# jinhan/tacotron2-vae

Measured on AMD Instinct MI355X. Metric: mel-frames/s (train step, batch=6, 80-mel), higher is better.
Workload: dtype f32; 1 GPU; configs[1]: Tacotron2-VAE fp32 train step (fwd+loss+bwd+clip+Adam), B=6/GPU fixed shape T_in=84 T_out=400, dropout on, random-init seed 1234; step_mode=hip-graph replay, decoder_forward=persistent, decoder_backward=persistent, startup_steps=43, global_batch=6, parallelism=dp1

## Files before the change

include/t2vae.h:

```cpp
#ifndef T2VAE_H
#define T2VAE_H
#include <stdint.h>
#ifdef __cplusplus
extern "C" {
#endif

#define T2V_OK 0
#define T2V_ERR_DIMS -1
#define T2V_ERR_ARG -2
#define T2V_ERR_LAUNCH -3

const char* t2v_version(void);
const char* t2v_last_error(void);

void t2v_set_phase_profile(unsigned long long* dev_buf32);
int t2v_stamp(unsigned long long* dev_buf, int slot, void* stream);
int t2v_debug_spin(int wgs, int microseconds, void* stream);

typedef struct t2v_step_params {
    uint64_t epoch;
    float lr;
    float bc1;
    float bc2s;
    float kl_weight;
// ... 51 lines not shown
    const float* bias_dec;
    const float* wq;
    const float* wcomb;
    const float* v;
} t2v_dec_train_persist_weights;
int t2v_decoder_train_persist_supported(int B, int T_in);
long t2v_decoder_train_persist_scratch_floats(int B, int T_in, int T_out);
int t2v_decoder_train_fwd_persistent(const t2v_dec_train_persist_weights* w, const t2v_dec_train_bufs* s, float* scratch,
                                     int B, int T_in, int T_out, float p_att, float p_dec, uint64_t seed, void* stream);

int t2v_decoder_train_persist16_supported(int B, int T_in);
long t2v_decoder_train_persist16_scratch_floats(int B, int T_in, int T_out);
int t2v_decoder_train_fwd_persistent16(const t2v_dec_train_persist_weights* w, const t2v_dec_train_bufs* s, float* scratch,
                                       int B, int T_in, int T_out, float p_att, float p_dec, uint64_t seed, void* stream);

int t2v_decoder_replay_fwd_kernels(const t2v_dec_weights* w, const t2v_dec_train_bufs* s,
                                   int B, int T_in, int T_out, float p_att, float p_dec,
                                   uint64_t seed, int kernel_mask, void* stream);

typedef struct t2v_dec_bwd_bufs {
    const float* dHC;
    float* DGA;
    float* DGD;
    float* DQ;
    float* DCTX;
    float* YD;
    float* YA;
    float* DCA;
    float* DCD;
    float* GPREV;
    float* GCUM;
    float* DV;
} t2v_dec_bwd_bufs;

int t2v_attn_bwd_slices(int T_in);

int t2v_decoder_train_bwd(const t2v_dec_weights* w, const t2v_dec_train_bufs* s,
                          const t2v_dec_bwd_bufs* g, int B, int T_in, int T_out,
                          float p_att, float p_dec, uint64_t seed, void* stream);

int t2v_decoder_replay_bwd_kernels(const t2v_dec_weights* w, const t2v_dec_train_bufs* s,
                                   const t2v_dec_bwd_bufs* g, int B, int T_in, int T_out,
                                   float p_att, float p_dec, uint64_t seed, int kernel_mask, void* stream);

int t2v_attn_wgrad_scratch_floats(void);
int t2v_attn_wgrad(const float* dpre, const float* al, const float* acum, const float* loc_conv,
                   const float* loc_dense, float* part_scratch, float* d_loc_dense, float* d_loc_conv,
                   int B, int T_in, int T, void* stream);


int t2v_decoder_bwd_persist_supported(int B, int T_in);
long t2v_decoder_bwd_achain_scratch_floats(int B, int T_in, int T_out);
int t2v_decoder_bwd_persist_slices(int T_in);
int t2v_decoder_bwd_achain(const t2v_dec_train_persist_weights* w, const float* reserved, const t2v_dec_train_bufs* s,
                           const float* dHC, float* DGA, float* DGD, float* DCTX, float* DV, float* DQP, float* scratch,
                           uint32_t* err_word, int B, int T_in, int T_out, float p_att, float p_dec, uint64_t seed,
                           void* stream);
int t2v_decoder_bwd_persist16_supported(int B, int T_in);
int t2v_decoder_bwd_persist16_slices(int T_in);
int t2v_decoder_bwd_persist16_fits(int B, int T_in, int T_out);
long t2v_decoder_bwd_persist16_scratch_floats(int B, int T_in, int T_out);
long t2v_decoder_bwd_persist16_dq_offset(int B, int T_in, int T_out);
int t2v_decoder_bwd_persistent16(const t2v_dec_train_persist_weights* w, const t2v_dec_train_bufs* s, const float* dHC,
                                 float* DGA, float* DGD, float* DCTX, float* DV, float* DQP, float* scratch,
                                 uint32_t* err_word, int B, int T_in, int T_out, float p_att, float p_dec, uint64_t seed,
                                 void* stream);
int t2v_decoder_bwd_persistent16_prepare(float* DQP, float* scratch, uint32_t* err_word, int B, int T_in, int T_out, void* stream);
int t2v_decoder_bwd_persistent16_prepared(const t2v_dec_train_persist_weights* w, const t2v_dec_train_bufs* s, const float* dHC,
                                          float* DGA, float* DGD, float* DCTX, float* DV, float* DQP, float* scratch,
                                          uint32_t* err_word, int B, int T_in, int T_out, float p_att, float p_dec, uint64_t seed,
                                          void* stream);

long t2v_decoder_bwd_achain_dq_offset(int B, int T_in, int T_out);
int t2v_decoder_bwd_achain_prepare(const t2v_dec_train_bufs* s, float* DQP, float* scratch, uint32_t* err_word, int B, int T_in,
                                   int T_out, float p_att, float p_dec, uint64_t seed, void* stream);
int t2v_decoder_bwd_achain_prepared(const t2v_dec_train_persist_weights* w, const float* reserved, const t2v_dec_train_bufs* s,
                           const float* dHC, float* DGA, float* DGD, float* DCTX, float* DV, float* DQP, float* scratch,
                           uint32_t* err_word, int B, int T_in, int T_out, float p_att, float p_dec, uint64_t seed,
                           void* stream);

typedef struct t2v_dec_infer_bufs {
    const float* memory;
    const float* pm;
    const int32_t* lengths;
    float* XS; float* CA; float* CD; float* QP; float* AL; float* ACUM;
    float* PRE;
    float* MEL;
    float* GATE;
    int32_t* stop_flag;
    const float* prenet_w1;
    const float* proj_w;
    const float* proj_b;
} t2v_dec_infer_bufs;

int t2v_decoder_infer_steps(const t2v_dec_weights* w, const t2v_dec_infer_bufs* s, int B, int T_in,
                            int t_begin, int t_end, float gate_threshold, float p_prenet,
                            int external_prenet, uint64_t seed, void* stream);

typedef struct t2v_dec_persist_weights {
    const float* w_ih_att; const float* w_hh_att;
    const float* w_ih_dec; const float* w_hh_dec;
    const float* bias_att; const float* bias_dec;
    const float* wq;
    const float* wcomb;
    const float* v;
    const float* proj_w;
    const float* proj_b;
    const float* prenet_w1;
} t2v_dec_persist_weights;
typedef struct t2v_dec_persist_bufs {
    const float* memory;
    const float* pm;
    const int32_t* lengths;
    const float* pre_first;
    float* MEL;
    float* GATE;
    float* AL;
    int32_t* stop_flag;
    void* exchange;
    uint32_t* err_word;
} t2v_dec_persist_bufs;
long t2v_decoder_persist_scratch_floats(int B, int t_end);
int t2v_decoder_persist_supported(int B, int T_in);
int t2v_decoder_infer_persistent(const t2v_dec_persist_weights* w, const t2v_dec_persist_bufs* s, int B, int T_in,
                                 int t_end, float gate_threshold, float p_prenet, uint64_t seed, void* stream);

typedef struct t2v_dec_items {
    int32_t* stop_item;
    const uint64_t* item_seeds;
// ... 32 lines not shown
                   float* dconv_bias, int B, int M, int T, int act, float p_drop, uint64_t seed,
                   uint32_t rng_stream, uint32_t rng_t, void* stream);
int t2v_bn_act_bwd_eval(const float* y, const float* dout, const float* mean, const float* rstd,
                   const float* gamma, const float* beta, float* dy, float* dgamma, float* dbeta,
                   float* dconv_bias, int B, int M, int T, int act, float p_drop, uint64_t seed,
                   uint32_t rng_stream, uint32_t rng_t, void* stream);

int t2v_embedding_fwd(const long long* ids, const float* W, float* out_bct, int B, int T, int C, int n_symbols, void* stream);
int t2v_embedding_bwd(const long long* ids, const float* dy_bct, float* dW, int B, int T, int C, int n_symbols, void* stream);

int t2v_gemm_epilogue_bwd(const float* dy, const float* y, float* out, size_t n, float scale, void* stream);

long t2v_colsum_scratch_floats(long M, long N);
int t2v_colsum(const float* A, long lda, long M, long N, float* scratch, float* out, void* stream);

int t2v_mask_outputs(float* mel, float* mel_post, float* gate, const int* lengths, int B, int C, int T, float gate_fill,
                     void* stream);
int t2v_mask_time(const float* x, float* out, const int32_t* lengths, int B, int C, int T, void* stream);
int t2v_reparam_fwd(const float* eps, const float* mu, const float* logvar, float* z, long n, void* stream);
int t2v_reparam_bwd(const float* dz, const float* eps, const float* logvar, float* dlogvar, long n, void* stream);
int t2v_gather_words(const void* const* src, void* const* dst, int n, void* stream);
int t2v_concat2_rows(const float* a, long lda, int na, const float* b, long ldb, int nb, float* out, long rows, void* stream);

int t2v_bilstm_fwd(const float* gx, const float* whh, const int32_t* lengths, float* y, float* gates,
                   float* cells, float* hx_scratch, uint32_t* sync3, int B, int T, void* stream);
int t2v_bilstm_bwd(const float* whh, const int32_t* lengths, const float* dy, const float* gates,
                   const float* cells, float* dg, float* dgx_scratch, uint32_t* sync3, int B, int T,
                   void* stream);

int t2v_gemm_f32(const float* A, long sAi, long sAk, const float* B, long sBj, long sBk, const float* bias,
                 float* C, int ldc, int M, int N, int K, int relu, int accumulate, float p_drop,
                 uint64_t seed, uint32_t rng_stream, uint32_t rng_t, void* stream);
long t2v_gemm_splitk_scratch_floats(int M, int N, int K);
int t2v_gemm_f32_splitk(const float* A, long sAi, long sAk, const float* B, long sBj, long sBk, const float* bias,
                        float* C, int ldc, int M, int N, int K, int relu, int accumulate, float p_drop,
                        uint64_t seed, uint32_t rng_stream, uint32_t rng_t, float* splitk_scratch, void* stream);

int t2v_gemm_f32_set_mode(int x3);

typedef struct t2v_gemm_group {
    const float* A;
    long sAi;
    long sAk;
    int nb;
    const float* B[3];
    long sBj[3];
    long sBk[3];
    int N[3];
    float* C[3];
    int ldc[3];
} t2v_gemm_group;
long t2v_gemm_f32_grouped_scratch_floats(const t2v_gemm_group* groups, int ngroups, int M, int K);
int t2v_gemm_f32_grouped(const t2v_gemm_group* groups, int ngroups, int M, int K, int accumulate, float* scratch, void* stream);
long t2v_gemm_bf16_grouped_scratch_floats(const t2v_gemm_group* groups, int ngroups, int M, int K);
int t2v_gemm_bf16_grouped(const t2v_gemm_group* groups, int ngroups, int M, int K, int accumulate, float* scratch, void* stream);

int t2v_conv1d_x3_set_mode(int mode);
int t2v_conv1d_takes_x3(int B, int Cin, int T, int Cout, int KS, int bf16);

int t2v_gemm_f32_batched(const float* A, long sAb, long sAi, long sAk, const float* B, long sBb, long sBj, long sBk,
                         float* C, long sCb, int ldc, int nbatch, int M, int N, int K, void* stream);
int t2v_gemm_bf16(const float* A, long sAi, long sAk, const float* B, long sBj, long sBk, const float* bias,
                  float* C, int ldc, int M, int N, int K, int relu, int accumulate, float p_drop,
                  uint64_t seed, uint32_t rng_stream, uint32_t rng_t, void* stream);
long t2v_gemm_bf16_splitk_scratch_floats(int M, int N, int K);
int t2v_gemm_bf16_splitk(const float* A, long sAi, long sAk, const float* B, long sBj, long sBk, const float* bias,
                         float* C, int ldc, int M, int N, int K, int relu, int accumulate, float p_drop,
                         uint64_t seed, uint32_t rng_stream, uint32_t rng_t, float* splitk_scratch, void* stream);


int t2v_conv2d_s2_fwd(const float* x, const float* w, const float* bias, float* y, int B, int Cx, int H, int W,
                      int Cout, int coord, void* stream);
int t2v_conv2d_s2_dw_scratch_floats(int B, int Cx, int H, int W, int Cout, int coord);
int t2v_conv2d_s2_bwd(const float* x, const float* w, const float* dy, float* dx, float* dw, float* dw_scratch,
                      int B, int Cx, int H, int W, int Cout, int coord, void* stream);

long t2v_conv2d_s2_gemm_scratch_floats(int B, int Cx, int H, int W, int Cout, int coord);
int t2v_conv2d_s2_fwd_gemm(const float* x, const float* w, const float* bias, float* y, float* scratch, int B, int Cx, int H, int W,
                           int Cout, int coord, void* stream);
int t2v_conv2d_s2_bwd_gemm(const float* x, const float* w, const float* dy, float* dx, float* dw, float* scratch, int B, int Cx, int H,
                           int W, int Cout, int coord, void* stream);
int t2v_gru_fwd(const float* gi, const float* whh, const float* bhh, float* hs, float* gsave, float* xchg,
                uint32_t* sync2, int B, int T, void* stream);
int t2v_gru_bwd(const float* whh, const float* hs, const float* gsave, const float* dh_last, float* dgi,
                float* dgh, float* xchg, uint32_t* sync2, int B, int T, void* stream);

int t2v_conv2d_s2_fwd_ragged(const float* x, const float* w, const float* bias, float* y, const int32_t* hlen, int B, int Cx,
                             int H, int W, int Cout, int coord, int x_tstride, void* stream);
long t2v_conv2d_s2_gemm_ragged_scratch_floats(int B, int Cx, int H, int W, int Cout, int coord);
int t2v_conv2d_s2_fwd_gemm_ragged(const float* x, const float* w, const float* bias, float* y, float* scratch,
                                  const int32_t* hlen, int B, int Cx, int H, int W, int Cout, int coord, int x_tstride,
                                  void* stream);
int t2v_gru_fwd_len(const float* gi, const float* whh, const float* bhh, float* hs, float* gsave, float* xchg,
                    uint32_t* sync2, const int32_t* steps, float* h_last, int B, int T, void* stream);
int t2v_loss_fwd_bwd(const float* mel, const float* post, const float* mel_t, const float* gate,
                     const float* gate_t, const float* mu, const float* logvar, float* dmel, float* dpost,
                     float* dgate, float* dmu, float* dlogvar, float* part192, float* out4, uint32_t* ticket,
                     uint64_t n_mel, int n_gate, int n_lat, float kl_weight, void* stream);

int t2v_clip_adam_step(float* params, float* grads, float* exp_avg, float* exp_avg_sq, uint64_t n,
                       float lr, float beta1, float beta2, float eps, float weight_decay,
                       float max_norm, float inv_world, float bc1, float bc2, float* partials,
                       float* norm_out, void* stream);
int t2v_clip_adam_step_guarded(float* params, float* grads, float* exp_avg, float* exp_avg_sq, uint64_t n,
                               float lr, float beta1, float beta2, float eps, float weight_decay,
                               float max_norm, float inv_world, float bc1, float bc2, float* partials,
// ... 32 lines not shown
```

tacotron2-vae_amd/csrc/decoder_train_bwd_persist.hip:

```cpp
#include "t2v_common.h"
#include "t2v_kernels.h"
#include "t2v_xchg.h"

#define PB_THREADS 512
#define PB_MAXB 6
#define PB_MAXT 224
#define PB_MAXT_LONG 576
#define PB_SPIN 400000
#define PB_KJ (T2V_G / PB_THREADS)

#define PB_ROW_BYTES(NB) ((NB) > 4 ? 98304u : 65536u)

#define PB_DROW_BYTES(NB) ((NB) > 4 ? 49152u : 32768u)
__device__ __forceinline__ void pb_dma4(const void* g, float* ldsbase, const int aux_sc1) {
    if (aux_sc1)
        __builtin_amdgcn_global_load_lds((const __attribute__((address_space(1))) void*)g, (__attribute__((address_space(3))) void*)ldsbase, 4, 0, T2V_SC1);
    else
        __builtin_amdgcn_global_load_lds((const __attribute__((address_space(1))) void*)g, (__attribute__((address_space(3))) void*)ldsbase, 4, 0, 0);
}

template <int NB>
__device__ __forceinline__ void pb_park_factors(float* ldsX, const float* Frow) {
    const int wave = threadIdx.x >> 6, lane = threadIdx.x & 63;
    constexpr int NCH = PB_ROW_BYTES(NB) / 1024;
#pragma unroll
    for (int i = 0; i < NCH / 8; ++i) {
        const int c = wave + 8 * i;
        __builtin_amdgcn_global_load_lds((const __attribute__((address_space(1))) void*)(Frow + 256 * c + 4 * lane),
                                         (__attribute__((address_space(3))) void*)(ldsX + 256 * c), 16, 0, 0);
    }
}
template <int NB>
__device__ __forceinline__ int pb_build_row(f32x4* X0, f32x2* X1, __amdgpu_buffer_rsrc_t r, unsigned row_off, int B,
                                            int nap, unsigned* err, int* flag) {
    const int tid = threadIdx.x;
    for (int i = 0; i < nap; i += 8) __builtin_amdgcn_s_sleep(8);
    f32x4 dc[2], dh[2], dx[2];
    int rounds = 0;
    const int nw0 = min(B, 4), nw1 = B - 4;
    for (;;) {
#pragma unroll
        for (int h = 0; h < 2; ++h) {
            const unsigned U = (unsigned)(tid + PB_THREADS * h);
            dc[h] = t2v_ld_f32x4(r, row_off + 32u * U);
            dh[h] = t2v_ld_f32x4(r, row_off + 32u * U + 16u);
            if (NB > 4) dx[h] = t2v_ld_f32x4(r, row_off + 32768u + 16u * U);
        }
        bool ok = true;
#pragma unroll
        for (int h = 0; h < 2; ++h) {
            ok = ok && t2v_ok(dc[h][0]) && (nw0 < 2 || t2v_ok(dc[h][1])) && (nw0 < 3 || t2v_ok(dc[h][2])) && (nw0 < 4 || t2v_ok(dc[h][3]));
            ok = ok && t2v_ok(dh[h][0]) && (nw0 < 2 || t2v_ok(dh[h][1])) && (nw0 < 3 || t2v_ok(dh[h][2])) && (nw0 < 4 || t2v_ok(dh[h][3]));
            if (NB > 4) ok = ok && t2v_ok(dx[h][0]) && t2v_ok(dx[h][2]) && (nw1 < 2 || (t2v_ok(dx[h][1]) && t2v_ok(dx[h][3])));
        }
        if (__all(ok)) break;
        __builtin_amdgcn_s_sleep(2);
        if (t2v_give_up(rounds, PB_SPIN, err, flag)) break;
    }
#pragma unroll
    for (int j = 0; j < PB_KJ; ++j) {
        const int h = j & 1;
        const f32x4 d = (j >> 1) == 3 ? dh[h] : dc[h];
// ... 82 lines not shown
                     "v_add_f32_dpp %0, %2, %2 row_half_mirror row_mask:0xf bank_mask:0xa" : "=&v"(t) : "v"(lo), "v"(hi));
    return t;
}
__device__ __forceinline__ void pb_reduce16(float (&v)[16], float* part) {
    const int tid = threadIdx.x, lane = tid & 63;
    const bool b1 = lane & 2, b0 = lane & 1;
    float w8[8], w4[4], w2[2];
#pragma unroll
    for (int i = 0; i < 8; ++i) w8[i] = pb_dpp_pair_add(v[i], v[8 + i], 0);
#pragma unroll
    for (int i = 0; i < 4; ++i) w4[i] = pb_dpp_pair_add(w8[i], w8[4 + i], 1);
#pragma unroll
    for (int i = 0; i < 2; ++i) {
        const float keep = b1 ? w4[2 + i] : w4[i], send = b1 ? w4[i] : w4[2 + i];
        w2[i] = keep + T2V_DPP_F(send, 0x4E);
    }
    const float keep = b0 ? w2[1] : w2[0], send = b0 ? w2[0] : w2[1];
    part[((tid >> 6) * 4 + (lane >> 4)) * 16 + (lane & 15)] = keep + T2V_DPP_F(send, 0xB1);
}
__device__ __forceinline__ float pb_sum16(const float* part, int idx) {
    float s[8];
#pragma unroll
    for (int i = 0; i < 8; ++i) s[i] = (part[(4 * i) * 16 + idx] + part[(4 * i + 1) * 16 + idx]) + (part[(4 * i + 2) * 16 + idx] + part[(4 * i + 3) * 16 + idx]);
    return ((s[0] + s[1]) + (s[2] + s[3])) + ((s[4] + s[5]) + (s[6] + s[7]));
}

static size_t pb_row_bytes(int B) { return B > 4 ? 98304u : 65536u; }

extern "C" int t2v_decoder_bwd_persist_supported(int B, int T_in) {
    if (!(B >= 1 && B <= PB_MAXB && T_in >= 1 && T_in <= PB_MAXT_LONG)) return 0;
    return t2v_persist_cus_ok();
}

struct PBAArgs {
    const float* w_ih_att; const float* w_hh_att; const float* w_ih_dec; const float* w_hh_dec;
    const float* wq;
    const float* wcomb;
    const float* v;
    const float* memory; const float* XS; const float* CA; const float* CD; const float* GA; const float* GD; const float* AL;
    float* S;
    const float* dHC;
    float* DGA; float* DGD; float* DCTX; float* DV;
    float* GXA; float* GXD; float* CX; float* DQX; float* GPX; float* EX;
    float* DQT;
    const float* CPA;
    const float* CPD;
    const float* FA; const float* FD;
    unsigned* err;
    int B, T_in, T, S_sl;
    float p_att, p_dec;
    uint64_t seed;
    const t2v_step_params* step;
    unsigned long long* prof;
};
#define PBA_STAMP(COND, I) do { if (a.prof && (COND) && threadIdx.x == 0) { const unsigned long long now_ = __builtin_readcyclecounter(); \
        lprof_[(I)] += now_ - tprev_; tprev_ = now_; } } while (0)
#define PBA_RT(SLOT) do { if (a.prof && t == a.T / 2 && threadIdx.x == 0) a.prof[64 + blockIdx.x * 8 + (SLOT)] = __builtin_amdgcn_s_memrealtime(); } while (0)
#define PBA_PROF_INIT(FLAGP) unsigned long long* lprof_ = (unsigned long long*)((FLAGP) + 4); \
    if (threadIdx.x < 16) lprof_[threadIdx.x] = 0ull
#define PBA_PROF_FLUSH(COND, I0, N) do { if (a.prof && (COND) && threadIdx.x < (N)) a.prof[(I0) + threadIdx.x] = lprof_[(I0) + threadIdx.x]; } while (0)

#define PB_CX_ROW_BYTES(NB) ((NB) > 4 ? 32768u : 16384u)

__host__ __device__ static inline int pba_na(int NL);
template <int JS, int NWV>
__device__ __forceinline__ void pba_attention_role(const PBAArgs& a, float* lds, const int b, const int s, const int NB) {
    constexpr int NJT = JS / 16;
    constexpr int PW = JS + 30;
    constexpr int GPW = PW <= 64 ? 64 : 128;
    constexpr int NRG = 2 * NWV;
    constexpr int DPS = JS == 96 ? JS + 17 : JS + 1;
    static_assert(JS % NRG == 0 && JS % NWV == 0 && PW <= GPW, "slice geometry");
    const int tid = threadIdx.x, lane = tid & 63, wave = tid >> 6;
    const bool act = tid < 64 * NWV;
    const int g = lane >> 4, c16 = lane & 15;
    const int B = a.B, Tp = a.T_in, T = a.T, S = a.S_sl, j0 = s * JS;
    const int Tcap = (Tp + 15) & ~15;
    const int nown = min(JS, Tp - j0);
    const int NAw = pba_na(T2V_NWG - B * S);
    float* gfull0 = lds;
    float* gfull1 = gfull0 + Tcap;
    float* alf = gfull1 + Tcap;
    float* gcum = alf + Tcap;
    float* dctx = gcum + Tcap;
    float* de = dctx + T2V_E;
    float* red = de + JS;
    float* dpT = red + (1 + JS / NWV) * 4 * NWV;
    float* Tl = dpT + T2V_A * DPS;
    float* rq = Tl + 64 * (JS + 1);
    float* rv = rq + NRG * T2V_A;
    int* flag = (int*)(rv + NRG * T2V_A);
    constexpr bool AREG_LDS = NWV == 8;
    float* wcs = (float*)(flag + 40);
    const __amdgpu_buffer_rsrc_t rC = t2v_rsrc(a.CX), rQ = t2v_rsrc(a.DQX), rP = t2v_rsrc(a.GPX), rQT = t2v_rsrc(a.DQT);
    const int d4 = tid & 31, rg = (tid >> 5) & (NRG - 1);
    float4 m0[JS / NWV], m1[JS / NWV];
    float areg[AREG_LDS ? 1 : 32];
    float4 vd4 = make_float4(0.f, 0.f, 0.f, 0.f);
    if (act) {
#pragma unroll
        for (int r = 0; r < JS / NWV; ++r) {
            const int jl = wave + NWV * r;
            const float* mrow = a.memory + ((size_t)b * Tp + j0 + (jl < nown ? jl : 0)) * T2V_E + lane * 4;
            m0[r] = *(const float4*)mrow;
            m1[r] = *(const float4*)(mrow + 256);
        }
// ... 261 lines not shown
        }
    }
#pragma unroll
    for (int i = 0; i < 16; ++i) v[i] = 0.f;
#pragma unroll
    for (int c = 0; c < NC; ++c)
#pragma unroll
        for (int i = 0; i < 3; ++i) { v[c * 8 + 2 * i] = acc[c][i][0]; v[c * 8 + 2 * i + 1] = acc[c][i][1]; }
}

template <int NCT, int C0, int N, int NB, int R = 0>
__device__ __forceinline__ void pba_rounds16(const f32x2 (&w)[NCT][PB_KJ / 2], const f32x4* X0, const f32x2* X1, float* part) {
    if constexpr (2 * R < N) {
        float v[16];
        pb_gemv_cols16<NCT, C0 + 2 * R, (N - 2 * R >= 2 ? 2 : 1), NB>(w, X0, X1, v);
        pb_reduce16(v, part + 512 * R);
        pba_rounds16<NCT, C0, N, NB, R + 1>(w, X0, X1, part);
    }
}

#define PBA_NUA 13
#define PBA_NCA 7
#define PBA_NUD 8
#define PBA_NCD 4
__host__ __device__ static inline int pba_na(int NL) {
    if (NL - 128 >= 86) return NL - 128;
    const int n = (3 * NL + 4) / 8;
    return n < 79 ? 79 : n;
}

__device__ __forceinline__ float pba_wait_word(__amdgpu_buffer_rsrc_t r, unsigned off, unsigned* err, int* flag) {
    unsigned x;
    int spins = 0;
    for (;;) {
        x = t2v_ld_b32(r, off);
        if (x != T2V_SENT) break;
        __builtin_amdgcn_s_sleep(1);
        if (t2v_give_up(spins, PB_SPIN, err, flag)) break;
    }
    return __uint_as_float(x);
}

template <int NB>
__device__ __forceinline__ void pba_publish_rows(__amdgpu_buffer_rsrc_t r, unsigned row_off, const float* stage, int u0, int nu) {
    const int tid = threadIdx.x;
    if (tid < 2 * nu) {
        const int u = tid >> 1, q = tid & 1;
        const float* sp = stage + (u * 2 + q) * 8;
        t2v_st(r, row_off + 32u * (unsigned)(u0 + u) + 16u * (unsigned)q, f32x4{sp[0], sp[1], sp[2], sp[3]});
        if (NB > 4) t2v_st(r, row_off + 32768u + 16u * (unsigned)(u0 + u) + 8u * (unsigned)q, f32x2{sp[4], sp[5]});
    }
}

template <int NB>
__device__ __forceinline__ void pba_decoder_role(const PBAArgs& a, float* lds, const int jd, const int ND) {
    const int B = a.B, T = a.T;
    f32x4* X0 = (f32x4*)lds;
    f32x2* X1 = (f32x2*)(lds + 4 * T2V_G);
    float* part = lds + (NB > 4 ? 6 : 4) * T2V_G;
    float* stage = part + 10 * 512;
    float* cpd = stage + 256;
    float* dhcs = cpd + 1024;
    int* flag = (int*)(dhcs + 128);
    const int u0 = (jd * T2V_H) / ND, nu = ((jd + 1) * T2V_H) / ND - u0;
    const int c0 = (jd * T2V_E) / ND, nc = ((jd + 1) * T2V_E) / ND - c0;
    const __amdgpu_buffer_rsrc_t rD = t2v_rsrc(a.GXD), rE = t2v_rsrc(a.EX), rDG = t2v_rsrc(a.DGD);
    f32x2 w[20][PB_KJ / 2];
    {
        const int tid = threadIdx.x;
#pragma unroll
        for (int jj = 0; jj < PB_KJ; ++jj) {
            const size_t k = (size_t)(tid + PB_THREADS * jj);
#pragma unroll
            for (int u = 0; u < PBA_NUD; ++u) {
                const bool on = u < nu;
                const int U = u0 + (on ? u : 0);
                w[u][jj / 2][jj & 1] = on ? a.w_hh_dec[k * T2V_H + U] : 0.f;
                w[8 + u][jj / 2][jj & 1] = on ? a.w_ih_dec[k * T2V_KATT + U] : 0.f;
            }
#pragma unroll
            for (int c = 0; c < PBA_NCD; ++c) {
                const bool on = c < nc;
                w[16 + c][jj / 2][jj & 1] = on ? a.w_ih_dec[k * T2V_KATT + T2V_H + c0 + (on ? c : 0)] : 0.f;
            }
        }
        if (tid == 0) flag[0] = 1;
    }
    float dcd = 0.f;
    int nap = 0;
    const int ncp4 = 2 * nu * NB;
    const float* cpd0 = a.CPD + (size_t)u0 * NB * 8;
    constexpr size_t CPSTEP = (size_t)T2V_H * NB * 8;
    {
        const int tid = threadIdx.x;
        if (tid < ncp4) *(float4*)(cpd + ((T - 1) & 1) * 512 + 4 * tid) = *(const float4*)(cpd0 + (size_t)(T - 1) * CPSTEP + 4 * tid);
        const int cu = tid >> 3, cb = tid & 7;
        if (tid < 64 && cu < nu && cb < B) dhcs[((T - 1) & 1) * 64 + tid] = a.dHC[((size_t)(T - 1) * B + cb) * (T2V_H + T2V_E) + u0 + cu];
    }
    pb_park_factors<NB>(lds, a.FD + (size_t)(T - 1) * (PB_ROW_BYTES(NB) / 4));
    __syncthreads();

    if (a.prof && jd == 0 && threadIdx.x == 0) a.prof[40] = __builtin_amdgcn_s_memrealtime();
    for (int t = T; t >= 0; --t) {
        int tid_op = threadIdx.x;
        asm volatile("" : "+v"(tid_op));
        const int tid = tid_op;
// ... 2 lines not shown
        const int U = u0 + (cu < nu ? cu : 0);
        if (t < T) {
            const int rounds = pb_build_row<NB>(X0, X1, rD, (unsigned)t * PB_DROW_BYTES(NB), B, nap, a.err, flag);
            nap = t2v_adapt_nap(nap, rounds);
            pba_rounds16<20, 0, 8, NB>(w, X0, X1, part);
        }
        if (t >= 2) {
            if (tid < ncp4)
                __builtin_amdgcn_global_load_lds((const __attribute__((address_space(1))) void*)(cpd0 + (size_t)(t - 2) * CPSTEP + 4 * tid),
                                                 (__attribute__((address_space(3))) void*)(cpd + ((t - 2) & 1) * 512 + 256 * (tid >> 6)), 16, 0, 0);
            if (cell_thr) pb_dma4(a.dHC + ((size_t)(t - 2) * B + cb) * (T2V_H + T2V_E) + U, dhcs + ((t - 2) & 1) * 64, 0);
        }
        __syncthreads();
        if (flag[0] != 1) return;
        f32x4 dg4 = {0.f, 0.f, 0.f, 0.f};
        if (t >= 1) {
            const int td = t - 1;
            if (cell_thr) {
                const float dh = dhcs[(td & 1) * 64 + tid] + (t < T ? pb_sum16(part + (cu >> 1) * 512, (cu & 1) * 8 + cb) : 0.f);
                const float* cp = cpd + (td & 1) * 512 + (cu * NB + cb) * 8;
                const float4 c0v = *(const float4*)cp, c1v = *(const float4*)(cp + 4);
                const float dht = dh * c0v.x;
                const float dct = dcd * c0v.y + dht * c0v.z;
                dg4 = f32x4{dct * c1v.x, dct * c1v.y, dct * c1v.z, dht * c1v.w};
                dcd = dct * c0v.w;
                float* sp = stage + (cu * 2) * 8 + cb;
                sp[0] = dct; sp[8] = dht;
            }
            if (tid < 64) pba_publish_rows<NB>(rD, (unsigned)td * PB_DROW_BYTES(NB), stage, u0, nu);
            if (cell_thr) {
                const unsigned o = (unsigned)((td * B + cb) * T2V_G + U) * 4u;
                __builtin_amdgcn_raw_buffer_store_b32(__float_as_uint(dg4[0]), rDG, (int)o, 0, 0);
                __builtin_amdgcn_raw_buffer_store_b32(__float_as_uint(dg4[1]), rDG, (int)(o + 4u * T2V_H), 0, 0);
                __builtin_amdgcn_raw_buffer_store_b32(__float_as_uint(dg4[2]), rDG, (int)(o + 8u * T2V_H), 0, 0);
                __builtin_amdgcn_raw_buffer_store_b32(__float_as_uint(dg4[3]), rDG, (int)(o + 12u * T2V_H), 0, 0);
            }
        }
        if (t < T) {
            pba_rounds16<20, 8, 12, NB>(w, X0, X1, part + 4 * 512);
            __syncthreads();
            if (t > 0) pb_park_factors<NB>(lds, a.FD + (size_t)(t - 1) * (PB_ROW_BYTES(NB) / 4));
            if (tid >= 64 && tid < 64 + 96) {
                const int i = tid - 64, col = i >> 3, b = i & 7;
                if (b < B) {
                    const float val = pb_sum16(part + (4 + (col >> 1)) * 512, (col & 1) * 8 + b);
                    if (col < 8) { if (col < nu) t2v_st(rE, (unsigned)(((t * B + b) * T2V_KATT) + u0 + col) * 4u, val); }
                    else if (col - 8 < nc) t2v_st(rE, (unsigned)(((t * B + b) * T2V_KATT) + T2V_H + c0 + col - 8) * 4u, val);
                }
            }
        }
        __syncthreads();
    }
    if (a.prof && jd == 0 && threadIdx.x == 0) a.prof[41] = __builtin_amdgcn_s_memrealtime();
}

struct PBACellIn { float gi, gf, gg, go, cac, cprev; };
__device__ __forceinline__ PBACellIn pba_cell_pre_load(const PBAArgs& a, bool cell_thr, int t, int cb, int U) {
    PBACellIn r = {0.f, 0.f, 0.f, 0.f, 0.f, 0.f};
    if (!cell_thr) return r;
    const int B = a.B;
    const float* gp = a.GA + ((size_t)t * B + cb) * T2V_G + U;
    r.gi = gp[0]; r.gf = gp[T2V_H]; r.gg = gp[2 * T2V_H]; r.go = gp[3 * T2V_H];
    r.cac = a.CA[((size_t)(t + 1) * B + cb) * T2V_H + U];
    r.cprev = a.CA[((size_t)t * B + cb) * T2V_H + U];
    return r;
}
__device__ __forceinline__ void pba_cell_pre_finish(const PBAArgs& a, float* cpre, uint64_t seed, bool cell_thr, int rowi, int t, uint32_t idx,
                                                    const PBACellIn& r) {
    if (!cell_thr) return;
    const float gi = r.gi, gf = r.gf, gg = r.gg, go = r.go;
    float cprev = r.cprev;
    const float fh = t2v_drop_scale(seed, T2V_RNG_ATT_H, t, idx, a.p_att);
    const float fc = t2v_drop_scale(seed, T2V_RNG_ATT_C, t, idx, a.p_att);
    if (t > 0) cprev *= t2v_drop_scale(seed, T2V_RNG_ATT_C, t - 1, idx, a.p_att);
    const float tc = tanhf_(r.cac);
    *(float4*)(cpre + rowi * 8) = make_float4(fh, fc, go * (1.0f - tc * tc), gf);
    *(float4*)(cpre + rowi * 8 + 4) = make_float4(gg * gi * (1.0f - gi), cprev * gf * (1.0f - gf), gi * (1.0f - gg * gg), tc * go * (1.0f - go));
}
__device__ __forceinline__ void pba_cell_pre(const PBAArgs& a, float* cpre, uint64_t seed, bool cell_thr, int rowi, int t, int cb, int U,
                                             uint32_t idx) {
    const PBACellIn r = pba_cell_pre_load(a, cell_thr, t, cb, U);
    pba_cell_pre_finish(a, cpre, seed, cell_thr, rowi, t, idx, r);
}

template <int NB, int NUA, int NCA>
__device__ __forceinline__ void pba_attention_rnn_role(const PBAArgs& a, float* lds, const int ja, const int NA) {
    constexpr int NCT = NUA + NCA;
    static_assert(NCA > 4 && NCA <= 8 && NUA > 8 && NUA <= 16, "two context rounds, three or four recurrent rounds");
    constexpr int NCR = (NCA + 1) / 2;
    const uint64_t seed = t2v_step_seed(a.seed, a.step);
    const int tid = threadIdx.x;
    const int B = a.B, T = a.T, S = a.S_sl;
    f32x4* X0 = (f32x4*)lds;
    f32x2* X1 = (f32x2*)(lds + 4 * T2V_G);
    float* part = lds + (NB > 4 ? 6 : 4) * T2V_G;
    float* ysum = part + 6 * 1024;
    float* dhA = ysum + 192;
    float* stage = dhA + 128;
    float* wqs = stage + 512;
    float* dqs = wqs + 16 * T2V_A;
    float* cpre = dqs + 8 * T2V_A;
    float* eps = cpre + 2048;
    int* flag = (int*)(eps + 256);
    float* dump = eps + 256 + 64;
    const int u0 = (ja * T2V_H) / NA, nu = ((ja + 1) * T2V_H) / NA - u0;
    const int c0 = (ja * T2V_E) / NA, nc = ((ja + 1) * T2V_E) / NA - c0;
// ... 187 lines not shown
        }
        __syncthreads();
        if (t > 0) pba_publish_rows<NB>(rA, (unsigned)t * PB_DROW_BYTES(NB), stage, u0, nu);
        if (cell_thr) {
            const unsigned o = (unsigned)((t * B + cb) * T2V_G + U) * 4u;
            __builtin_amdgcn_raw_buffer_store_b32(__float_as_uint(dg4[0]), rDG, (int)o, 0, 0);
            __builtin_amdgcn_raw_buffer_store_b32(__float_as_uint(dg4[1]), rDG, (int)(o + 4u * T2V_H), 0, 0);
            __builtin_amdgcn_raw_buffer_store_b32(__float_as_uint(dg4[2]), rDG, (int)(o + 8u * T2V_H), 0, 0);
            __builtin_amdgcn_raw_buffer_store_b32(__float_as_uint(dg4[3]), rDG, (int)(o + 12u * T2V_H), 0, 0);
        }
        PBA_STAMP(ja == 0, 6);
        PBA_RT(5);
        __syncthreads();
        PBA_STAMP(ja == 0, 7);
    }
    if (a.prof && ja == 0 && tid == 0) a.prof[43] = __builtin_amdgcn_s_memrealtime();
    PBA_PROF_FLUSH(ja == 0, 0, 8);
    PBA_PROF_FLUSH(ja == 0, 12, 4);
}

template <int NB, bool LONG>
__global__ __launch_bounds__(PB_THREADS) void k_achain_bwd(PBAArgs a) {
    extern __shared__ __attribute__((aligned(16))) float lds[];
    const int wg = blockIdx.x;
    const int S = a.S_sl, NT = a.B * S, NL = T2V_NWG - NT, NA = pba_na(NL), ND = NL - NA;
#if defined(PBA_ONLY) && PBA_ONLY == 1
    pba_attention_role<16, 4>(a, lds, wg / S, wg % S, NB);
#elif defined(PBA_ONLY) && PBA_ONLY == 2
    pba_attention_rnn_role<NB, 12, 6>(a, lds, wg - NT, NA);
#elif defined(PBA_ONLY) && PBA_ONLY == 3
    pba_attention_rnn_role<NB, PBA_NUA, PBA_NCA>(a, lds, wg - NT, NA);
#elif defined(PBA_ONLY) && PBA_ONLY == 4
    pba_decoder_role<NB>(a, lds, wg - NT - NA, ND);
#else
    if (wg < NT) {
        if (LONG) pba_attention_role<96, 8>(a, lds, wg / S, wg % S, NB);
        else if (a.T_in <= 128) pba_attention_role<16, 4>(a, lds, wg / S, wg % S, NB);
        else pba_attention_role<32, 4>(a, lds, wg / S, wg % S, NB);
    } else if (wg < NT + NA) {
        if (NA >= 114) pba_attention_rnn_role<NB, 9, 5>(a, lds, wg - NT, NA);
        else if (NA >= 86) pba_attention_rnn_role<NB, 12, 6>(a, lds, wg - NT, NA);
        else pba_attention_rnn_role<NB, PBA_NUA, PBA_NCA>(a, lds, wg - NT, NA);
    } else {
        pba_decoder_role<NB>(a, lds, wg - NT - NA, ND);
    }
#endif
}

static inline int pba_js(int T_in) { return T_in > PB_MAXT ? 96 : t2v_attn_bwd_js(T_in); }
static inline int pba_slices(int T_in) { const int js = pba_js(T_in); return (T_in + js - 1) / js; }
extern "C" int t2v_decoder_bwd_persist_slices(int T_in) { return T_in < 1 ? 0 : pba_slices(T_in); }

static size_t pba_lds_bytes(int B, int T_in) {
    const size_t lrole = (B > 4 ? 6 : 4) * T2V_G + 6 * 1024 + 192 + 128 + 512 + 16 * T2V_A + 8 * T2V_A + 2048 + 256 + 64 + 512;
    const size_t Tcap = (size_t)((T_in + 15) / 16) * 16, JS = (size_t)pba_js(T_in), NWV = JS == 96 ? 8 : 4;
    const size_t trole = 4 * Tcap + T2V_E + JS + (1 + JS / NWV) * 4 * NWV + T2V_A * (JS == 96 ? JS + 17 : JS + 1) + 64 * (JS + 1) +
                         2 * 2 * NWV * T2V_A + 40 + (NWV == 8 ? 64 * 132 : 0);
    return sizeof(float) * (lrole > trole ? lrole : trole);
}

struct PBALayout {
    size_t n_gx, n_cx, n_gp, n_ex, n_dqt, n_f, n_cp, n_dq;
    size_t dqt_off() const { return 2 * n_gx + n_cx + n_gp + n_ex; }
    size_t n_exchange() const { return dqt_off() + n_dqt; }
    size_t total() const { return n_exchange() + 2 * n_f + 2 * n_cp; }
};
static PBALayout pba_layout(int B, int T_in, int T_out) {
    const size_t T = (size_t)T_out, S = (size_t)pba_slices(T_in), gpw = pba_js(T_in) + 30 <= 64 ? 64 : 128;
    const size_t rowf = pb_row_bytes(B) / 4, cxf = (size_t)(B > 4 ? 32768 : 16384) / 4;
    PBALayout l;
    l.n_gx = T * rowf / 2;
    l.n_cx = T * cxf;
    l.n_gp = T * B * S * 2 * gpw;
    l.n_ex = T * B * T2V_KATT;
    l.n_dqt = T * 8 * T2V_A;
    l.n_f = T * rowf;
    l.n_cp = T * T2V_H * (B > 4 ? 6 : 4) * 8;
    l.n_dq = T * B * S * 128;
    return l;
}

extern "C" long t2v_decoder_bwd_achain_scratch_floats(int B, int T_in, int T_out) {
    if (B < 1 || B > PB_MAXB || T_in < 1 || T_in > PB_MAXT_LONG || T_out < 1) return 0;
    return (long)pba_layout(B, T_in, T_out).total();
}

extern "C" long t2v_decoder_bwd_achain_dq_offset(int B, int T_in, int T_out) {
    if (!t2v_decoder_bwd_persist_supported(B, T_in) || T_out < 1) return -1;
    return (long)pba_layout(B, T_in, T_out).dqt_off();
}

static int pba_launch(const t2v_dec_train_persist_weights* w, const t2v_dec_train_bufs* s,
                      const float* dHC, float* DGA, float* DGD, float* DCTX, float* DV, float* DQP, float* scratch,
                      uint32_t* err_word, int B, int T_in, int T_out, float p_att, float p_dec, uint64_t seed,
                      void* stream_, bool do_prepare, bool do_run) {
    hipStream_t stream = (hipStream_t)stream_;
    if (!s || !DQP || !scratch || !err_word) return T2V_ERR_ARG;
    if (do_run && (!w || !dHC || !DGA || !DGD || !DCTX || !DV)) return T2V_ERR_ARG;
    if (!t2v_decoder_bwd_persist_supported(B, T_in) || T_out < 1) return T2V_ERR_ARG;
    if (do_run && (!w->w_ih_att || !w->w_hh_att || !w->w_ih_dec || !w->w_hh_dec || !w->wq || !w->wcomb || !w->v)) return T2V_ERR_ARG;
    if (!s->memory || !s->XS || !s->CA || !s->CD || !s->GA || !s->GD || !s->AL || !s->S) return T2V_ERR_ARG;
    const PBALayout l = pba_layout(B, T_in, T_out);
    if (((uintptr_t)scratch & 15) || ((uintptr_t)DQP & 15) || l.n_gx * 4 >= 0x7fffffffull || l.n_dq * 4 >= 0x7fffffffull) return T2V_ERR_ARG;
    if (pba_lds_bytes(B, T_in) > T2V_LDS_MAX) return T2V_ERR_ARG;
    static bool raised = false;
    if (!t2v_persist_raise_lds({(const void*)k_achain_bwd<4, false>, (const void*)k_achain_bwd<6, false>,
                                (const void*)k_achain_bwd<4, true>, (const void*)k_achain_bwd<6, true>}, raised))
        return t2v_check_launch();
    if (do_prepare) {
        (void)hipMemsetAsync(err_word, 0, sizeof(uint32_t), stream);
        t2v_fill_sentinel(scratch, l.n_exchange() / 4, 1024, stream);
        t2v_fill_sentinel(DQP, l.n_dq / 4, 256, stream);
    }
    PBAArgs a;
    if (do_run) {
        a.w_ih_att = w->w_ih_att; a.w_hh_att = w->w_hh_att; a.w_ih_dec = w->w_ih_dec; a.w_hh_dec = w->w_hh_dec;
        a.wq = w->wq; a.wcomb = w->wcomb; a.v = w->v;
    }
    a.memory = s->memory; a.XS = s->XS; a.CA = s->CA; a.CD = s->CD; a.GA = s->GA; a.GD = s->GD; a.AL = s->AL; a.S = s->S;
    a.dHC = dHC; a.DGA = DGA; a.DGD = DGD; a.DCTX = DCTX; a.DV = DV; a.DQX = DQP;
    a.GXA = scratch;
    a.GXD = a.GXA + l.n_gx;
    a.CX = a.GXD + l.n_gx;
    a.GPX = a.CX + l.n_cx;
    a.EX = a.GPX + l.n_gp;
    a.DQT = a.EX + l.n_ex;
    float* FA = a.DQT + l.n_dqt;
    float* FD = FA + l.n_f;
    float* CPA = FD + l.n_f;
    float* CPD = CPA + l.n_cp;
    a.FA = FA; a.FD = FD; a.CPA = CPA; a.CPD = CPD;
    a.err = err_word;
    a.B = B; a.T_in = T_in; a.T = T_out; a.S_sl = pba_slices(T_in); a.p_att = p_att; a.p_dec = p_dec; a.seed = seed;
    a.step = t2v_step_for(stream);
    a.prof = g_t2v_prof;
    if (do_prepare) {
        const unsigned nblk = (unsigned)(((size_t)T_out * T2V_G + 255) / 256);
        k_pb_factors<<<nblk, 256, 0, stream>>>(s->GA, s->CA, FA, B, T_out, B, p_att, T2V_RNG_ATT_C, seed, a.step);
        k_pb_factors<<<nblk, 256, 0, stream>>>(s->GD, s->CD, FD, B, T_out, B, p_dec, T2V_RNG_DEC_C, seed, a.step);
        const int nbs = B > 4 ? 6 : 4;
        const unsigned ncp = (unsigned)(((size_t)T_out * T2V_H * nbs + 255) / 256);
        k_pb_cellpre<<<ncp, 256, 0, stream>>>(s->GA, s->CA, CPA, B, T_out, nbs, p_att, T2V_RNG_ATT_H, T2V_RNG_ATT_C, seed, a.step);
        k_pb_cellpre<<<ncp, 256, 0, stream>>>(s->GD, s->CD, CPD, B, T_out, nbs, p_dec, T2V_RNG_DEC_H, T2V_RNG_DEC_C, seed, a.step);
    }
    if (!do_run) return t2v_check_launch();
    const size_t lds = pba_lds_bytes(B, T_in);
    if (T_in > PB_MAXT) {
        if (B > 4) k_achain_bwd<6, true><<<T2V_NWG, PB_THREADS, lds, stream>>>(a);
        else k_achain_bwd<4, true><<<T2V_NWG, PB_THREADS, lds, stream>>>(a);
    } else {
        if (B > 4) k_achain_bwd<6, false><<<T2V_NWG, PB_THREADS, lds, stream>>>(a);
        else k_achain_bwd<4, false><<<T2V_NWG, PB_THREADS, lds, stream>>>(a);
    }
    return t2v_check_launch();
}

extern "C" int t2v_decoder_bwd_achain(const t2v_dec_train_persist_weights* w, const float* w_unused, const t2v_dec_train_bufs* s,
                                      const float* dHC, float* DGA, float* DGD, float* DCTX, float* DV, float* DQP, float* scratch,
                                      uint32_t* err_word, int B, int T_in, int T_out, float p_att, float p_dec, uint64_t seed,
                                      void* stream_) {
    (void)w_unused;
    return pba_launch(w, s, dHC, DGA, DGD, DCTX, DV, DQP, scratch, err_word, B, T_in, T_out, p_att, p_dec, seed, stream_, true, true);
}

extern "C" int t2v_decoder_bwd_achain_prepare(const t2v_dec_train_bufs* s, float* DQP, float* scratch, uint32_t* err_word, int B, int T_in,
                                              int T_out, float p_att, float p_dec, uint64_t seed, void* stream_) {
    return pba_launch(nullptr, s, nullptr, nullptr, nullptr, nullptr, nullptr, DQP, scratch, err_word, B, T_in, T_out, p_att, p_dec, seed,
                      stream_, true, false);
}
extern "C" int t2v_decoder_bwd_achain_prepared(const t2v_dec_train_persist_weights* w, const float* w_unused, const t2v_dec_train_bufs* s,
                                               const float* dHC, float* DGA, float* DGD, float* DCTX, float* DV, float* DQP, float* scratch,
                                               uint32_t* err_word, int B, int T_in, int T_out, float p_att, float p_dec, uint64_t seed,
                                               void* stream_) {
    (void)w_unused;
    return pba_launch(w, s, dHC, DGA, DGD, DCTX, DV, DQP, scratch, err_word, B, T_in, T_out, p_att, p_dec, seed, stream_, false, true);
}
```

tacotron2-vae_amd/csrc/gemm.hip:

```cpp
#include <stdlib.h>
#include <string.h>
#include "t2v_common.h"
#include "t2v_kernels.h"
#include "t2v_coop.h"
#include "t2v_x3.h"
#include "t2v_xchg.h"

#define GM_BM 64
#define GM_BN 64
#define GM_BK 32

struct GemmArgs {
    const float* A; const float* B; const float* bias; float* C;
    long sAi, sAk, sBj, sBk;
    int M, N, K, ldc;
    int relu, accumulate;
    float p_drop; uint64_t seed; uint32_t rng_stream, rng_t;
    const t2v_step_params* step;
    int kz_chunk;
    float* part;
    int nbatch;
    long sAb, sBb, sCb;
    int nsub;
    long sAs, sBs;
    int bias_row;
    unsigned* tile_ctr;
};

__device__ __forceinline__ void gemm64_epilogue(const GemmArgs& a, f32x16& acc, int i0, int j0, int wm, int wn, int lane, int tid) {
    const int j = j0 + 32 * wn + (lane & 31);
    if (a.part) {
        if (j < a.N) {
#pragma unroll
            for (int r = 0; r < 16; ++r) {
                const int i = i0 + 32 * wm + (r & 3) + 8 * (r >> 2) + 4 * (lane >> 5);
                if (i < a.M) st_sc1(a.part + ((size_t)blockIdx.z * a.M + i) * a.N + j, acc[r]);
            }
        }
        __shared__ unsigned last_;
        asm volatile("s_waitcnt vmcnt(0)" ::: "memory");
        __syncthreads();
        unsigned* ctr = a.tile_ctr + blockIdx.y * gridDim.x + blockIdx.x;
        if (tid == 0) last_ = __hip_atomic_fetch_add(ctr, 1u, __ATOMIC_RELAXED, __HIP_MEMORY_SCOPE_AGENT) == gridDim.z - 1 ? 1u : 0u;
        __syncthreads();
        if (!last_) return;
        if (tid == 0) __hip_atomic_store(ctr, 0u, __ATOMIC_RELAXED, __HIP_MEMORY_SCOPE_AGENT);
        const int nz = (int)gridDim.z;
#pragma unroll
        for (int r = 0; r < 16; ++r) acc[r] = 0.f;
        if (j < a.N) {
            for (int z0 = 0; z0 < nz; z0 += 4) {
                float v[4][16];
#pragma unroll
                for (int u = 0; u < 4; ++u) {
                    const int z = min(z0 + u, nz - 1);
#pragma unroll
                    for (int r = 0; r < 16; ++r) {
                        const int i = min(i0 + 32 * wm + (r & 3) + 8 * (r >> 2) + 4 * (lane >> 5), a.M - 1);
                        v[u][r] = ld_sc1(a.part + ((size_t)z * a.M + i) * a.N + j);
// ... 524 lines not shown
            if (j < a.N) {
                const float bvs = a.bias ? a.bias[j] : 0.f;
#pragma unroll
                for (int r = 0; r < 16; ++r) {
                    const int i = i0 + 64 * wm + 32 * x + (r & 3) + 8 * (r >> 2) + 4 * (lane >> 5);
                    if (i < a.M) {
                        const size_t idx = (size_t)i * a.ldc + j;
                        float v = acc[x][y][r] + bvs;
                        if (a.accumulate) v += a.C[idx];
                        a.C[idx] = v;
                    }
                }
            }
        }
}
static bool gemm_bf16_big_operand_ok(long s_row, long s_k, int K, bool* kc) {
    if (s_row == 1 && !(s_k & 3)) { *kc = false; return true; }
    if (s_k == 1 && !(s_row & 3) && !(K % GBB_BK)) { *kc = true; return true; }
    return false;
}
static bool gemm_bf16_big_ok(const GemmArgs& a, bool* akc, bool* bkc) {
    if (a.relu || a.p_drop > 0.f) return false;
    if (!gemm_bf16_big_operand_ok(a.sAi, a.sAk, a.K, akc) || !gemm_bf16_big_operand_ok(a.sBj, a.sBk, a.K, bkc)) return false;
    if (a.M < GBB_BM || a.N < GBB_BN || (a.M & 3) || (a.N & 3)) return false;
    if (((uintptr_t)a.A | (uintptr_t)a.B) & 15) return false;
    return (long)((a.M + GBB_BM - 1) / GBB_BM) * ((a.N + GBB_BN - 1) / GBB_BN) >= 64;
}
static int gemm_bf16_big_splits(int M, int N, int K) {
    const long tiles = (long)((M + GBB_BM - 1) / GBB_BM) * ((N + GBB_BN - 1) / GBB_BN);
    const int nkt = (K + GBB_BK - 1) / GBB_BK;
    if (tiles < 64 || tiles >= 512 || nkt < 32) return 1;
    static const int forced = getenv("T2V_GEMM_BF16_SPLITS") ? atoi(getenv("T2V_GEMM_BF16_SPLITS")) : 0;
    long ns = forced > 0 ? forced : (768 + tiles - 1) / tiles;
    if (ns > nkt / 16) ns = nkt / 16;
    if (ns > 8) ns = 8;
    return ns < 2 ? 1 : (int)ns;
}
static bool gemm_bf16_planes_ok(int M, int N, int K);
static long gemm_x3_scratch_floats(int M, int N, int K, int np);
extern "C" long t2v_gemm_bf16_splitk_scratch_floats(int M, int N, int K) {
    if (M < 1 || N < 1 || K < 1) return 0;
    if (gemm_bf16_planes_ok(M, N, K)) return gemm_x3_scratch_floats(M, N, K, 1);
    long big = 0;
    if (M >= GBB_BM && N >= GBB_BN && !(M & 3) && !(N & 3)) {
        const int ns = gemm_bf16_big_splits(M, N, K);
        const long tiles = (long)((M + GBB_BM - 1) / GBB_BM) * ((N + GBB_BN - 1) / GBB_BN);
        big = ns > 1 ? (long)ns * tiles * GBB_BM * GBB_BN : 0;
    }
    const int ns64 = gemm_splits(M, N, K);
    const long small = ns64 > 1 ? (long)ns64 * M * N : 0;
    return big > small ? big : small;
}

#define GX_BM 128
#define GX_BN 128
#define GX_SK 16
static inline long gx_rp(int rows) { return ((long)rows + 127) / 128 * 128; }
static inline long gx_groups(int K, int np = 3) { return np == 3 ? ((long)K + 31) / 32 * 4 : ((long)K + 63) / 64 * 8; }
static inline long gx_plane_slots(int rows, int K, int np = 3) { return np * gx_groups(K, np) * gx_rp(rows); }
template <bool KC, int NP>
__global__ __launch_bounds__(256) void k_x3_split(const float* __restrict__ src, long s_row, long s_k, int rows, int K, uint4* __restrict__ dst,
                                                  long Rp, long G) {
    __shared__ uint4 sm[NP][4][64];
    const int tid = threadIdx.x;
    const int row0 = blockIdx.x * 64, g0 = blockIdx.y * 4;
    const int r = KC ? tid >> 2 : tid & 63, g = KC ? tid & 3 : tid >> 6;
    const int row = row0 + r, k0 = 8 * (g0 + g);
    float v[8];
    const bool rin = row < rows;
    const float* base = src + (long)min(row, rows - 1) * s_row;
    if (KC && s_k == 1 && !(s_row & 3) && !((uintptr_t)src & 15) && k0 + 8 <= K) {
        const float4 lo = *(const float4*)(base + k0), hi = *(const float4*)(base + k0 + 4);
        v[0] = lo.x; v[1] = lo.y; v[2] = lo.z; v[3] = lo.w; v[4] = hi.x; v[5] = hi.y; v[6] = hi.z; v[7] = hi.w;
#pragma unroll
        for (int u = 0; u < 8; ++u) v[u] = rin ? v[u] : 0.f;
    } else {
#pragma unroll
        for (int u = 0; u < 8; ++u) {
            const float x = base[(long)min(k0 + u, K - 1) * s_k];
            v[u] = (rin && k0 + u < K) ? x : 0.f;
        }
    }
    if (NP == 3) {
        uint4 p0, p1, p2;
        t2v_split8(v, p0, p1, p2);
        sm[0][g][r] = p0; sm[NP > 1 ? 1 : 0][g][r] = p1; sm[NP > 2 ? 2 : 0][g][r] = p2;
    } else {
        sm[0][g][r] = make_uint4(t2v_pack_bf16x2(v[0], v[1]), t2v_pack_bf16x2(v[2], v[3]), t2v_pack_bf16x2(v[4], v[5]), t2v_pack_bf16x2(v[6], v[7]));
    }
    __syncthreads();
    const int g2 = tid >> 6, r2 = tid & 63;
    if (row0 + r2 < Rp && g0 + g2 < G) {
#pragma unroll
        for (int p = 0; p < NP; ++p) dst[(p * G + g0 + g2) * Rp + row0 + r2] = sm[p][g2][r2];
    }
}
struct GemmX3Prod {
    const uint4* Ap; const uint4* Bp;
    long RpA, RpB;
    int N, tiles_x, tile0, nseg;
    int seg_col[3]; float* segC[3]; int seg_ldc[3];
};
struct GemmX3Args {
    GemmX3Prod pr[2];
    int nprod, ntiles;
    long G;
    const float* bias;
    int M, relu, accumulate;
    float p_drop; uint64_t seed; uint32_t rng_stream, rng_t;
    const t2v_step_params* step;
    int st_chunk;
    float* part; unsigned* tile_ctr;
};
#ifndef GX_NB
#define GX_NB 2
#endif
#ifndef GX_LDS_PAD
#define GX_LDS_PAD 0
#endif
#ifndef GX_NG1
#define GX_NG1 4
#endif
template <int NP, int NG>
__global__ __launch_bounds__(256, 2) void k_gemm_x3p(GemmX3Args a) {
    __shared__ uint4 lds_[GX_NB * 2 * NP * NG * GX_BM + GX_LDS_PAD];
    uint4 (*Ls)[2][NP][NG][GX_BM] = (uint4 (*)[2][NP][NG][GX_BM])&lds_[0];
    const unsigned lds0 = (unsigned)(unsigned long)(__attribute__((address_space(3))) void*)&lds_[0];
    const int tid = threadIdx.x, wave = __builtin_amdgcn_readfirstlane(tid >> 6), lane = tid & 63;
    const int wm = wave >> 1, wn = wave & 1;
    int lin;
    {
        const int nb = a.ntiles, bid = blockIdx.x;
        const int q = nb >> 3, r = nb & 7, xcd = bid & 7, idx = bid >> 3;
        lin = (xcd < r ? xcd * (q + 1) : r * (q + 1) + (xcd - r) * q) + idx;
    }
    const GemmX3Prod& P = a.pr[(a.nprod > 1 && lin >= a.pr[1].tile0) ? 1 : 0];
    const int by_ = (lin - P.tile0) / P.tiles_x, bx_ = (lin - P.tile0) - by_ * P.tiles_x;
    const int i0 = by_ * GX_BM, j0 = bx_ * GX_BN;
    const int nst_all = (int)(a.G / NG);
    const int st0 = a.st_chunk ? blockIdx.z * a.st_chunk : 0, st1 = a.st_chunk ? min(nst_all, st0 + a.st_chunk) : nst_all;
    constexpr int NPIECE = NP * NG;
    auto stage_dma = [&](int st, int buf) {
        st = min(st, st1 - 1);
#pragma unroll
        for (int i = 0; i < NPIECE; ++i) {
            const int q = wave + 4 * i;
            const int op = q / (2 * NP * NG), rem = q - (2 * NP * NG) * op, p = rem / (2 * NG), g = (rem >> 1) % NG, half = rem & 1;
            const uint4* src = op ? P.Bp + (p * a.G + NG * st + g) * P.RpB + j0 + 64 * half + lane
                                  : P.Ap + (p * a.G + NG * st + g) * P.RpA + i0 + 64 * half + lane;
            t2v_dma16(src, lds0 + 16u * (unsigned)(((((buf * 2 + op) * NP + p) * NG + g) * GX_BM) + 64 * half));
        }
    };
    f32x16 acc[2][2];
#pragma unroll
    for (int x = 0; x < 2; ++x)
#pragma unroll
        for (int y = 0; y < 2; ++y)
#pragma unroll
            for (int r = 0; r < 16; ++r) acc[x][y][r] = 0.f;
    const int am = 64 * wm + (lane & 31), bn = 64 * wn + (lane & 31), kq = lane >> 5;
#define GX_MFMA(A_, B_, C_) C_ = __builtin_amdgcn_mfma_f32_32x32x16_bf16(*(const t2v_bf16x8*)&(A_), *(const t2v_bf16x8*)&(B_), C_, 0, 0, 0)
#pragma unroll
    for (int d = 0; d < GX_NB - 1; ++d) stage_dma(st0 + d, d);
    t2v_wait_vmcnt<NPIECE * (GX_NB - 2)>();
    __syncthreads();
    int buf = 0;
    for (int st = st0; st < st1; ++st) {
        const int nb2 = buf == 0 ? GX_NB - 1 : buf - 1;
        stage_dma(st + GX_NB - 1, nb2);
#define GX_ALL(PA, PB)                                      \
        GX_MFMA(av[PA][0], bv[PB][0], acc[0][0]); GX_MFMA(av[PA][0], bv[PB][1], acc[0][1]); \
        GX_MFMA(av[PA][1], bv[PB][0], acc[1][0]); GX_MFMA(av[PA][1], bv[PB][1], acc[1][1])
#pragma unroll
        for (int ks = 0; ks < NG / 2; ++ks) {
            uint4 av[NP][2], bv[NP][2];
#pragma unroll
            for (int p = 0; p < NP; ++p) {
                av[p][0] = Ls[buf][0][p][2 * ks + kq][am];
                av[p][1] = Ls[buf][0][p][2 * ks + kq][am + 32];
                bv[p][0] = Ls[buf][1][p][2 * ks + kq][bn];
                bv[p][1] = Ls[buf][1][p][2 * ks + kq][bn + 32];
            }
            if constexpr (NP == 3) {
                GX_ALL(2, 0); GX_ALL(0, 2); GX_ALL(1, 1); GX_ALL(1, 0); GX_ALL(0, 1); GX_ALL(0, 0);
            } else {
                GX_ALL(0, 0);
            }
        }
#undef GX_ALL
        t2v_wait_vmcnt<NPIECE * (GX_NB - 2)>();
        __syncthreads();
        buf = buf == GX_NB - 1 ? 0 : buf + 1;
    }
#undef GX_MFMA
    asm volatile("s_waitcnt vmcnt(0)" ::: "memory");
    if (a.part) {
        const size_t tiles = (size_t)a.ntiles, tile = (size_t)lin;
        {
            __amdgpu_buffer_rsrc_t rs = t2v_rsrc(a.part + (blockIdx.z * tiles + tile) * (GX_BM * GX_BN));
#pragma unroll
            for (int x = 0; x < 2; ++x)
#pragma unroll
                for (int y = 0; y < 2; ++y)
#pragma unroll
                    for (int q = 0; q < 4; ++q) {
                        u32x4 v;
                        v.x = __float_as_uint(acc[x][y][4 * q]); v.y = __float_as_uint(acc[x][y][4 * q + 1]);
                        v.z = __float_as_uint(acc[x][y][4 * q + 2]); v.w = __float_as_uint(acc[x][y][4 * q + 3]);
                        __builtin_amdgcn_raw_buffer_store_b128(v, rs, ((((x * 2 + y) * 4 + q) * 256) + tid) * 16, 0, 16);
                    }
        }
        __shared__ unsigned last_;
        asm volatile("s_waitcnt vmcnt(0)" ::: "memory");
        __syncthreads();
        unsigned* ctr = a.tile_ctr + tile;
        if (tid == 0) last_ = __hip_atomic_fetch_add(ctr, 1u, __ATOMIC_RELAXED, __HIP_MEMORY_SCOPE_AGENT) == gridDim.z - 1 ? 1u : 0u;
        __syncthreads();
        if (!last_) return;
        if (tid == 0) __hip_atomic_store(ctr, 0u, __ATOMIC_RELAXED, __HIP_MEMORY_SCOPE_AGENT);
        const int nz = (int)gridDim.z;
#pragma unroll
        for (int x = 0; x < 2; ++x)
#pragma unroll
            for (int y = 0; y < 2; ++y)
#pragma unroll
                for (int r = 0; r < 16; ++r) acc[x][y][r] = 0.f;
        for (int z0 = 0; z0 < nz; z0 += 2) {
            u32x4 v[2][16];
#pragma unroll
            for (int u = 0; u < 2; ++u) {
                const int z = min(z0 + u, nz - 1);
                __amdgpu_buffer_rsrc_t rs = t2v_rsrc(a.part + (z * tiles + tile) * (GX_BM * GX_BN));
#pragma unroll
                for (int g = 0; g < 16; ++g) v[u][g] = __builtin_amdgcn_raw_buffer_load_b128(rs, (g * 256 + tid) * 16, 0, 16);
            }
#pragma unroll
            for (int u = 0; u < 2; ++u)
                if (z0 + u < nz) {
#pragma unroll
                    for (int g = 0; g < 16; ++g) {
                        acc[g >> 3][(g >> 2) & 1][4 * (g & 3)] += __uint_as_float(v[u][g].x);
                        acc[g >> 3][(g >> 2) & 1][4 * (g & 3) + 1] += __uint_as_float(v[u][g].y);
                        acc[g >> 3][(g >> 2) & 1][4 * (g & 3) + 2] += __uint_as_float(v[u][g].z);
                        acc[g >> 3][(g >> 2) & 1][4 * (g & 3) + 3] += __uint_as_float(v[u][g].w);
                    }
                }
        }
    }
    const uint64_t seed = t2v_step_seed(a.seed, a.step);
    int sg = 0;
    if (P.nseg > 1 && j0 >= P.seg_col[1]) sg = 1;
    if (P.nseg > 2 && j0 >= P.seg_col[2]) sg = 2;
    float* const Cd = P.segC[sg];
    const int ldc = P.seg_ldc[sg], jc0 = j0 - P.seg_col[sg];
#pragma unroll
    for (int x = 0; x < 2; ++x)
#pragma unroll
        for (int y = 0; y < 2; ++y) {
            const int jl = 64 * wn + 32 * y + (lane & 31), j = j0 + jl;
            if (j < P.N) {
                const float bvs = a.bias ? a.bias[j] : 0.f;
#pragma unroll
                for (int r = 0; r < 16; ++r) {
                    const int i = i0 + 64 * wm + 32 * x + (r & 3) + 8 * (r >> 2) + 4 * (lane >> 5);
                    if (i < a.M) {
                        const size_t idx = (size_t)i * ldc + jc0 + jl;
                        float v = acc[x][y][r] + bvs;
                        if (a.accumulate) v += Cd[idx];
                        if (a.relu) v = fmaxf(v, 0.f);
                        if (a.p_drop > 0.f) v *= t2v_drop_scale(seed, a.rng_stream, a.rng_t, (uint32_t)idx, a.p_drop);
                        Cd[idx] = v;
                    }
                }
            }
        }
}
static int g_f32_gemm_x3 = -1;
static int gemm_x3_mode() {
    if (g_f32_gemm_x3 < 0) {
        const char* e = getenv("T2V_F32_GEMM");
        g_f32_gemm_x3 = (e && (!strcmp(e, "native") || !strcmp(e, "0"))) ? 0 : 1;
    }
    return g_f32_gemm_x3;
}
extern "C" int t2v_gemm_f32_set_mode(int x3) {
    const int prev = gemm_x3_mode();
    if (x3 >= 0) g_f32_gemm_x3 = x3 ? 1 : 0;
    return prev;
}
static bool gemm_x3_shape_ok(int M, int N, int K) {
    if (M < GX_BM || N < GX_BN || K < 32) return false;
    static const int min_tiles = getenv("T2V_X3_MIN_TILES") ? atoi(getenv("T2V_X3_MIN_TILES")) : 64;
    return (long)((M + GX_BM - 1) / GX_BM) * ((N + GX_BN - 1) / GX_BN) >= min_tiles;
}
static int gemm_x3_splits(int M, int N, int K, int np = 3) {
    const long tiles = (long)((M + GX_BM - 1) / GX_BM) * ((N + GX_BN - 1) / GX_BN);
    const int nst = (int)(gx_groups(K, np) / (np == 3 ? 2 : GX_NG1));
    static const int forced = getenv("T2V_GEMM_X3_SPLITS") ? atoi(getenv("T2V_GEMM_X3_SPLITS")) : 0;
    if (forced > 0) return forced > nst ? nst : forced;
    int best = 1;
    double best_w = 1e30;
    for (int ns = 1; ns <= 6 && (ns == 1 || nst / ns >= 16); ++ns) {
        const double rounds = (double)((tiles * ns + 767) / 768);
        const double w = rounds * (1.0 / ns + 0.08) + 0.03 * (ns - 1);
        if (w < best_w - 1e-9) { best_w = w; best = ns; }
    }
    return best;
}
static long gemm_x3_plane_floats(int M, int N, int K, int np = 3) { return 4 * (gx_plane_slots(M, K, np) + gx_plane_slots(N, K, np)); }
static long gemm_x3_scratch_floats(int M, int N, int K, int np) {
    const int ns = gemm_x3_splits(M, N, K, np);
    const long tiles = (long)((M + GX_BM - 1) / GX_BM) * ((N + GX_BN - 1) / GX_BN);
    return gemm_x3_plane_floats(M, N, K, np) + (ns > 1 ? (long)ns * tiles * GX_BM * GX_BN : 0);
}
static bool gemm_bf16_planes_ok(int M, int N, int K) {
    static const int on = getenv("T2V_BF16_GEMM_PLANES") ? atoi(getenv("T2V_BF16_GEMM_PLANES")) : 1;
    return on && K >= 64 && gemm_x3_shape_ok(M, N, K);
}
static void gx_split_launch(const float* src, long s_row, long s_k, int rows, int K, uint4* planes, long Rp, long G, long row_off, hipStream_t stream,
                            int np = 3) {
    const unsigned gx = (unsigned)((rows + 127) / 128 * 2);
    const dim3 grid(gx, (unsigned)(G / 4));
    if (np == 3) {
        if (s_k == 1) k_x3_split<true, 3><<<grid, 256, 0, stream>>>(src, s_row, s_k, rows, K, planes + row_off, Rp, G);
        else k_x3_split<false, 3><<<grid, 256, 0, stream>>>(src, s_row, s_k, rows, K, planes + row_off, Rp, G);
    } else {
        if (s_k == 1) k_x3_split<true, 1><<<grid, 256, 0, stream>>>(src, s_row, s_k, rows, K, planes + row_off, Rp, G);
        else k_x3_split<false, 1><<<grid, 256, 0, stream>>>(src, s_row, s_k, rows, K, planes + row_off, Rp, G);
    }
}
static int gemm_x3_run(const GemmArgs& g, float* scratch, hipStream_t stream, int np = 3) {
    const int M = g.M, N = g.N, K = g.K;
    uint4* Ap = (uint4*)scratch;
    uint4* Bp = Ap + gx_plane_slots(M, K, np);
    const long G = gx_groups(K, np), RpA = gx_rp(M), RpB = gx_rp(N);
    gx_split_launch(g.A, g.sAi, g.sAk, M, K, Ap, RpA, G, 0, stream, np);
    gx_split_launch(g.B, g.sBj, g.sBk, N, K, Bp, RpB, G, 0, stream, np);
    GemmX3Args a;
    a.nprod = 1;
    GemmX3Prod& P = a.pr[0];
    P.Ap = Ap; P.Bp = Bp; P.RpA = RpA; P.RpB = RpB; P.N = N; P.tiles_x = (N + GX_BN - 1) / GX_BN; P.tile0 = 0; P.nseg = 1;
    P.seg_col[0] = 0; P.segC[0] = g.C; P.seg_ldc[0] = g.ldc;
    a.pr[1] = a.pr[0];
    a.ntiles = P.tiles_x * ((M + GX_BM - 1) / GX_BM);
    a.G = G; a.bias = g.bias; a.M = M; a.relu = g.relu; a.accumulate = g.accumulate;
    a.p_drop = g.p_drop; a.seed = g.seed; a.rng_stream = g.rng_stream; a.rng_t = g.rng_t; a.step = g.step;
    a.st_chunk = 0; a.part = nullptr; a.tile_ctr = nullptr;
    dim3 gb(a.ntiles, 1, 1);
    const int ns = gemm_x3_splits(M, N, K, np);
    if (ns > 1) {
        const int nst = (int)(G / (np == 3 ? 2 : GX_NG1));
        a.st_chunk = (nst + ns - 1) / ns;
        gb.z = (unsigned)((nst + a.st_chunk - 1) / a.st_chunk);
        a.part = scratch + gemm_x3_plane_floats(M, N, K, np);
        a.tile_ctr = t2v_arrival_counters(a.ntiles);
        if (!a.tile_ctr) return T2V_ERR_LAUNCH;
        if (gb.z < 2) { a.st_chunk = 0; a.part = nullptr; a.tile_ctr = nullptr; gb.z = 1; }
    }
    if (np == 3) k_gemm_x3p<3, 2><<<gb, 256, 0, stream>>>(a);
    else k_gemm_x3p<1, GX_NG1><<<gb, 256, 0, stream>>>(a);
    return t2v_check_launch();
}

static long gemm_grouped_scratch(const t2v_gemm_group* gr, int ngroups, int M, int K, int np) {
    if (!gr || ngroups < 1 || ngroups > 2 || M < 1 || K < 1) return 0;
    long slots = 0;
    for (int g = 0; g < ngroups; ++g) {
        long n = 0;
        for (int p = 0; p < gr[g].nb; ++p) n += gx_rp(gr[g].N[p]);
        slots += gx_plane_slots(M, K, np) + np * gx_groups(K, np) * n;
    }
    return 4 * slots;
}
extern "C" long t2v_gemm_f32_grouped_scratch_floats(const t2v_gemm_group* gr, int ngroups, int M, int K) {
    return gemm_grouped_scratch(gr, ngroups, M, K, 3);
}
extern "C" long t2v_gemm_bf16_grouped_scratch_floats(const t2v_gemm_group* gr, int ngroups, int M, int K) {
    return gemm_grouped_scratch(gr, ngroups, M, K, 1);
}
static bool gemm_grouped_x3_ok(const t2v_gemm_group* gr, int ngroups, int M, int K, int np) {
    if ((np == 3 && !gemm_x3_mode()) || M < GX_BM || K < 32) return false;
    long tiles = 0;
    for (int g = 0; g < ngroups; ++g)
        for (int p = 0; p < gr[g].nb; ++p) {
            if (gr[g].N[p] < GX_BN || (gr[g].N[p] % GX_BN)) return false;
            tiles += (long)(gr[g].N[p] / GX_BN) * ((M + GX_BM - 1) / GX_BM);
        }
    return tiles >= 64;
}
static int gemm_grouped_impl(const t2v_gemm_group* gr, int ngroups, int M, int K, int accumulate, float* scratch, void* stream_, int np) {
    hipStream_t stream = (hipStream_t)stream_;
    if (!gr || ngroups < 1 || ngroups > 2 || M < 1 || K < 1) return T2V_ERR_ARG;
    for (int g = 0; g < ngroups; ++g) {
        if (!gr[g].A || gr[g].nb < 1 || gr[g].nb > 3) return T2V_ERR_ARG;
        for (int p = 0; p < gr[g].nb; ++p)
            if (!gr[g].B[p] || !gr[g].C[p] || gr[g].N[p] < 1 || gr[g].ldc[p] < gr[g].N[p]) return T2V_ERR_ARG;
    }
    if (!scratch || ((uintptr_t)scratch & 15) || !gemm_grouped_x3_ok(gr, ngroups, M, K, np)) {
        for (int g = 0; g < ngroups; ++g)
            for (int p = 0; p < gr[g].nb; ++p) {
                const int rc = (np == 3 ? t2v_gemm_f32 : t2v_gemm_bf16)(gr[g].A, gr[g].sAi, gr[g].sAk, gr[g].B[p], gr[g].sBj[p], gr[g].sBk[p], nullptr, gr[g].C[p], gr[g].ldc[p],
                                            M, gr[g].N[p], K, 0, accumulate, 0.f, 0, 0, 0, stream_);
                if (rc != T2V_OK) return rc;
            }
        return T2V_OK;
    }
    const long G = gx_groups(K, np), RpA = gx_rp(M);
    GemmX3Args a;
    a.nprod = ngroups;
    uint4* at = (uint4*)scratch;
    int tile0 = 0;
    for (int g = 0; g < ngroups; ++g) {
        GemmX3Prod& P = a.pr[g];
        long n = 0;
        for (int p = 0; p < gr[g].nb; ++p) n += gr[g].N[p];
        P.Ap = at; at += gx_plane_slots(M, K, np);
        P.Bp = at; at += np * G * n;
        P.RpA = RpA; P.RpB = n; P.N = (int)n; P.tiles_x = (int)(n / GX_BN); P.tile0 = tile0; P.nseg = gr[g].nb;
        gx_split_launch(gr[g].A, gr[g].sAi, gr[g].sAk, M, K, (uint4*)P.Ap, RpA, G, 0, stream, np);
        long col = 0;
        for (int p = 0; p < 3; ++p) {
            const int q = p < gr[g].nb ? p : gr[g].nb - 1;
            P.seg_col[p] = p < gr[g].nb ? (int)col : 0x7fffffff; P.segC[p] = gr[g].C[q]; P.seg_ldc[p] = gr[g].ldc[q];
            if (p < gr[g].nb) {
                gx_split_launch(gr[g].B[p], gr[g].sBj[p], gr[g].sBk[p], gr[g].N[p], K, (uint4*)P.Bp, n, G, col, stream, np);
                col += gr[g].N[p];
            }
        }
        tile0 += P.tiles_x * (int)((M + GX_BM - 1) / GX_BM);
    }
    if (ngroups == 1) a.pr[1] = a.pr[0];
    a.ntiles = tile0;
    a.G = G; a.bias = nullptr; a.M = M; a.relu = 0; a.accumulate = accumulate;
    a.p_drop = 0.f; a.seed = 0; a.rng_stream = 0; a.rng_t = 0; a.step = t2v_step_for(stream);
    a.st_chunk = 0; a.part = nullptr; a.tile_ctr = nullptr;
    if (np == 3) k_gemm_x3p<3, 2><<<dim3(a.ntiles, 1, 1), 256, 0, stream>>>(a);
    else k_gemm_x3p<1, GX_NG1><<<dim3(a.ntiles, 1, 1), 256, 0, stream>>>(a);
    return t2v_check_launch();
}
extern "C" int t2v_gemm_f32_grouped(const t2v_gemm_group* gr, int ngroups, int M, int K, int accumulate, float* scratch, void* stream_) {
    return gemm_grouped_impl(gr, ngroups, M, K, accumulate, scratch, stream_, 3);
}
extern "C" int t2v_gemm_bf16_grouped(const t2v_gemm_group* gr, int ngroups, int M, int K, int accumulate, float* scratch, void* stream_) {
    return gemm_grouped_impl(gr, ngroups, M, K, accumulate, scratch, stream_, 1);
}

__global__ __launch_bounds__(256) void k_epilogue_bwd(const float4* __restrict__ dy, const float4* __restrict__ y,
                                                      float4* __restrict__ out, size_t n4, float scale) {
    const size_t i = (size_t)blockIdx.x * 256 + threadIdx.x;
    if (i >= n4) return;
    const float4 g = dy[i], v = y[i];
    float4 o;
    o.x = v.x != 0.f ? g.x * scale : 0.f; o.y = v.y != 0.f ? g.y * scale : 0.f;
    o.z = v.z != 0.f ? g.z * scale : 0.f; o.w = v.w != 0.f ? g.w * scale : 0.f;
    out[i] = o;
}
__global__ __launch_bounds__(256) void k_epilogue_bwd_tail(const float* __restrict__ dy, const float* __restrict__ y,
                                                           float* __restrict__ out, size_t lo, size_t n, float scale) {
    const size_t i = lo + threadIdx.x;
    if (i < n) out[i] = y[i] != 0.f ? dy[i] * scale : 0.f;
}

extern "C" int t2v_gemm_epilogue_bwd(const float* dy, const float* y, float* out, size_t n, float scale, void* stream_) {
    hipStream_t stream = (hipStream_t)stream_;
    if (!dy || !y || !out || n < 1) return T2V_ERR_ARG;
    if (((uintptr_t)dy | (uintptr_t)y | (uintptr_t)out) & 15) return T2V_ERR_ARG;
    const size_t n4 = n / 4;
    if (n4) k_epilogue_bwd<<<(unsigned)((n4 + 255) / 256), 256, 0, stream>>>((const float4*)dy, (const float4*)y, (float4*)out, n4, scale);
    if (n & 3) k_epilogue_bwd_tail<<<1, 256, 0, stream>>>(dy, y, out, 4 * n4, n, scale);
    return t2v_check_launch();
}

extern "C" int t2v_gemm_f32(const float* A, long sAi, long sAk, const float* B, long sBj, long sBk, const float* bias,
                            float* C, int ldc, int M, int N, int K, int relu, int accumulate, float p_drop,
                            uint64_t seed, uint32_t rng_stream, uint32_t rng_t, void* stream_);
static int gemm_bf16_impl(const float* A, long sAi, long sAk, const float* B, long sBj, long sBk, const float* bias,
                          float* C, int ldc, int M, int N, int K, int relu, int accumulate, float p_drop,
                          uint64_t seed, uint32_t rng_stream, uint32_t rng_t, float* splitk_scratch, void* stream_);
extern "C" int t2v_gemm_bf16(const float* A, long sAi, long sAk, const float* B, long sBj, long sBk, const float* bias,
                             float* C, int ldc, int M, int N, int K, int relu, int accumulate, float p_drop,
                             uint64_t seed, uint32_t rng_stream, uint32_t rng_t, void* stream_) {
    return gemm_bf16_impl(A, sAi, sAk, B, sBj, sBk, bias, C, ldc, M, N, K, relu, accumulate, p_drop, seed, rng_stream, rng_t, nullptr, stream_);
}
extern "C" int t2v_gemm_bf16_splitk(const float* A, long sAi, long sAk, const float* B, long sBj, long sBk, const float* bias,
                                    float* C, int ldc, int M, int N, int K, int relu, int accumulate, float p_drop,
                                    uint64_t seed, uint32_t rng_stream, uint32_t rng_t, float* splitk_scratch, void* stream_) {
    return gemm_bf16_impl(A, sAi, sAk, B, sBj, sBk, bias, C, ldc, M, N, K, relu, accumulate, p_drop, seed, rng_stream, rng_t, splitk_scratch, stream_);
}
static int gemm_bf16_impl(const float* A, long sAi, long sAk, const float* B, long sBj, long sBk, const float* bias,
                          float* C, int ldc, int M, int N, int K, int relu, int accumulate, float p_drop,
                          uint64_t seed, uint32_t rng_stream, uint32_t rng_t, float* splitk_scratch, void* stream_) {
    hipStream_t stream = (hipStream_t)stream_;
    if (!A || !B || !C || M < 1 || N < 1 || K < 1 || ldc < N) return T2V_ERR_ARG;
    GemmArgs a;
// ... 127 lines not shown
```

tacotron2-vae_amd/t2v_hip.py:

```python
import collections
import ctypes as C
import os

import torch

_HERE = os.path.dirname(os.path.abspath(__file__))
_LIB_PATH = os.environ.get('T2V_LIB') or os.path.join(_HERE, 'libt2vae_hip.so')
_lib = None

H, E, PRE, A, F_LOC, KS, XW, KATT, KATT_INF, G4 = 1024, 512, 256, 128, 32, 31, 2560, 1536, 1792, 4096


class T2VHipError(RuntimeError):
    pass


class _DecWeights(C.Structure):
    _fields_ = [(n, C.c_void_p) for n in (
        'packF_att', 'packF_dec', 'packB_att', 'packB_dec', 'bias_att', 'bias_dec', 'wqT', 'wcomb', 'v')] + [
        ('packs_bf16', C.c_int32)]


class _DecTrainBufs(C.Structure):
    _fields_ = [(n, C.c_void_p) for n in (
        'gpre', 'memory', 'pm', 'lengths', 'XS', 'CA', 'CD', 'GA', 'GD', 'QP', 'AL', 'ACUM', 'S')]


class _DecBwdBufs(C.Structure):
    _fields_ = [(n, C.c_void_p) for n in (
        'dHC', 'DGA', 'DGD', 'DQ', 'DCTX', 'YD', 'YA', 'DCA', 'DCD', 'GPREV', 'GCUM', 'DV')]


class _DecPersistWeights(C.Structure):
    _fields_ = [(n, C.c_void_p) for n in (
        'w_ih_att', 'w_hh_att', 'w_ih_dec', 'w_hh_dec', 'bias_att', 'bias_dec', 'wq', 'wcomb', 'v', 'proj_w', 'proj_b',
        'prenet_w1')]


class _DecPersistBufs(C.Structure):
    _fields_ = [(n, C.c_void_p) for n in (
        'memory', 'pm', 'lengths', 'pre_first', 'MEL', 'GATE', 'AL', 'stop_flag', 'exchange', 'err_word')]


class _DecTrainPersistWeights(C.Structure):
    C_NAME = 't2v_dec_train_persist_weights'
    _fields_ = [(n, C.c_void_p) for n in (
        'w_ih_att', 'w_hh_att', 'w_ih_dec', 'w_hh_dec', 'bias_dec', 'wq', 'wcomb', 'v')]


class _GemmGroup(C.Structure):
    C_NAME = 't2v_gemm_group'
    _fields_ = [('A', C.c_void_p), ('sAi', C.c_long), ('sAk', C.c_long), ('nb', C.c_int), ('B', C.c_void_p * 3), ('sBj', C.c_long * 3),
                ('sBk', C.c_long * 3), ('N', C.c_int * 3), ('C', C.c_void_p * 3), ('ldc', C.c_int * 3)]


class _DecInferBufs(C.Structure):
    _fields_ = [(n, C.c_void_p) for n in (
        'memory', 'pm', 'lengths', 'XS', 'CA', 'CD', 'QP', 'AL', 'ACUM', 'PRE', 'MEL', 'GATE', 'stop_flag',
        'prenet_w1', 'proj_w', 'proj_b')]


class _DecItems(C.Structure):
    C_NAME = 't2v_dec_items'
    _fields_ = [(n, C.c_void_p) for n in ('stop_item', 'item_seeds')]


EXPORTS = ('t2v_version', 't2v_last_error', 't2v_stamp', 't2v_debug_spin', 't2v_pack_lstm_weights', 't2v_pack_lstm_weights_bf16', 't2v_decoder_train_fwd',
           't2v_decoder_train_bwd', 't2v_clip_adam_step', 't2v_clip_adam_step_guarded', 't2v_decoder_replay_fwd_kernels', 't2v_mel_frontend', 't2v_set_phase_profile', 't2v_decoder_infer_steps', 't2v_conv1d_stat_blocks', 't2v_conv1d_stat_blocks_bf16', 't2v_conv1d_fwd', 't2v_conv1d_bwd', 't2v_conv1d_fwd_bf16', 't2v_conv1d_bwd_bf16', 't2v_conv1d_dw_scratch_floats', 't2v_conv1d_flip_weights', 't2v_gemm_bf16', 't2v_gemm_bf16_splitk', 't2v_gemm_bf16_splitk_scratch_floats', 't2v_attn_wgrad', 't2v_attn_wgrad_scratch_floats',
           't2v_bn_act_fwd', 't2v_bn_act_bwd', 't2v_bn_act_bwd_eval', 't2v_bilstm_fwd', 't2v_bilstm_bwd', 't2v_gemm_f32', 't2v_conv2d_s2_fwd', 't2v_conv2d_s2_bwd', 't2v_conv2d_s2_dw_scratch_floats', 't2v_conv2d_s2_fwd_gemm', 't2v_conv2d_s2_bwd_gemm',
           't2v_conv2d_s2_gemm_scratch_floats',
           't2v_gru_fwd', 't2v_gru_bwd', 't2v_loss_fwd_bwd', 't2v_fuse_location_weights', 't2v_decoder_qp_floats',
           't2v_set_step_params', 't2v_set_step_params_stream', 't2v_decoder_replay_bwd_kernels', 't2v_embedding_fwd', 't2v_embedding_bwd', 't2v_gemm_f32_splitk', 't2v_gemm_splitk_scratch_floats', 't2v_gemm_f32_batched',
           't2v_decoder_infer_persistent', 't2v_decoder_persist_supported', 't2v_decoder_persist_scratch_floats',
           't2v_attn_bwd_slices', 't2v_colsum', 't2v_colsum_scratch_floats', 't2v_gemm_epilogue_bwd',
           't2v_decoder_train_fwd_persistent', 't2v_decoder_train_persist_supported',
           't2v_decoder_train_persist_scratch_floats', 't2v_decoder_bwd_persist_supported',
           't2v_decoder_bwd_achain_scratch_floats', 't2v_decoder_bwd_achain', 't2v_decoder_bwd_achain_prepare',
           't2v_decoder_bwd_achain_prepared', 't2v_decoder_bwd_persist_slices', 't2v_decoder_bwd_achain_dq_offset', 't2v_mask_outputs', 't2v_reparam_fwd',
           't2v_reparam_bwd', 't2v_gather_words', 't2v_concat2_rows',
           't2v_decoder_train_fwd_persistent16', 't2v_decoder_train_persist16_supported',
           't2v_decoder_train_persist16_scratch_floats', 't2v_decoder_bwd_persistent16', 't2v_decoder_bwd_persist16_supported',
           't2v_decoder_bwd_persist16_scratch_floats', 't2v_decoder_bwd_persist16_dq_offset', 't2v_decoder_bwd_persist16_slices',
           't2v_decoder_bwd_persist16_fits', 't2v_gemm_f32_set_mode', 't2v_conv1d_x3_set_mode', 't2v_gemm_f32_grouped',
           't2v_gemm_f32_grouped_scratch_floats', 't2v_gemm_bf16_grouped', 't2v_gemm_bf16_grouped_scratch_floats',
           't2v_decoder_bwd_persistent16_prepare', 't2v_decoder_bwd_persistent16_prepared',
           't2v_stft_polar', 't2v_istft', 't2v_istft_scratch_bytes', 't2v_griffin_lim', 't2v_griffin_lim_scratch_bytes',
           't2v_mel_to_magnitude', 't2v_decoder_infer_steps_items', 't2v_decoder_infer_persistent_items', 't2v_bn_act_fwd_len',
           't2v_mask_time', 't2v_conv2d_s2_fwd_ragged', 't2v_conv2d_s2_fwd_gemm_ragged', 't2v_conv2d_s2_gemm_ragged_scratch_floats',
           't2v_gru_fwd_len', 't2v_mel_dtw', 't2v_mel_dtw_scratch_bytes')


def lib_path():
    return _LIB_PATH


def load_library():
    global _lib
    if _lib is not None:
        return _lib
    if not os.path.isfile(_LIB_PATH):
        raise T2VHipError("libt2vae_hip.so not built: run `python -c 'import __graft_entry__ as g; g.build()'` "
                          "(or make -C tacotron2-vae_amd/csrc)")
    lib = C.CDLL(_LIB_PATH)
    lib.t2v_version.restype = C.c_char_p
    lib.t2v_last_error.restype = C.c_char_p
    lib.t2v_pack_lstm_weights.argtypes = [C.c_void_p, C.c_void_p, C.c_void_p, C.c_void_p, C.c_int, C.c_void_p,
                                          C.c_void_p, C.c_void_p, C.c_void_p, C.c_void_p]
    lib.t2v_pack_lstm_weights_bf16.argtypes = [C.c_void_p, C.c_void_p, C.c_void_p, C.c_void_p, C.c_int, C.c_void_p,
                                          C.c_void_p, C.c_void_p, C.c_void_p, C.c_void_p]
    lib.t2v_fuse_location_weights.argtypes = [C.c_void_p, C.c_void_p, C.c_void_p, C.c_void_p]
    lib.t2v_decoder_qp_floats.argtypes = [C.c_int, C.c_int]
    lib.t2v_decoder_qp_floats.restype = C.c_long
    lib.t2v_attn_bwd_slices.argtypes = [C.c_int]
    lib.t2v_decoder_train_fwd.argtypes = [C.POINTER(_DecWeights), C.POINTER(_DecTrainBufs), C.c_int, C.c_int,
                                          C.c_int, C.c_float, C.c_float, C.c_uint64, C.c_void_p]
    lib.t2v_decoder_train_bwd.argtypes = [C.POINTER(_DecWeights), C.POINTER(_DecTrainBufs),
                                          C.POINTER(_DecBwdBufs), C.c_int, C.c_int, C.c_int, C.c_float,
                                          C.c_float, C.c_uint64, C.c_void_p]
    lib.t2v_decoder_train_fwd_persistent.argtypes = [C.POINTER(_DecTrainPersistWeights), C.POINTER(_DecTrainBufs), C.c_void_p,
                                                     C.c_int, C.c_int, C.c_int, C.c_float, C.c_float, C.c_uint64, C.c_void_p]
    lib.t2v_decoder_train_persist_supported.argtypes = [C.c_int, C.c_int]
    lib.t2v_decoder_train_fwd_persistent16.argtypes = lib.t2v_decoder_train_fwd_persistent.argtypes
    lib.t2v_decoder_train_persist16_supported.argtypes = [C.c_int, C.c_int]
    lib.t2v_decoder_train_persist16_scratch_floats.argtypes = [C.c_int, C.c_int, C.c_int]
    lib.t2v_decoder_train_persist16_scratch_floats.restype = C.c_long
    lib.t2v_decoder_bwd_persistent16.argtypes = [C.POINTER(_DecTrainPersistWeights), C.POINTER(_DecTrainBufs)] + [C.c_void_p] * 8 + [
        C.c_int, C.c_int, C.c_int, C.c_float, C.c_float, C.c_uint64, C.c_void_p]
    lib.t2v_decoder_bwd_persistent16_prepared.argtypes = lib.t2v_decoder_bwd_persistent16.argtypes
    lib.t2v_decoder_bwd_persistent16_prepare.argtypes = [C.c_void_p, C.c_void_p, C.c_void_p, C.c_int, C.c_int, C.c_int, C.c_void_p]
    lib.t2v_decoder_bwd_persist16_supported.argtypes = [C.c_int, C.c_int]
    lib.t2v_decoder_bwd_persist16_scratch_floats.argtypes = [C.c_int, C.c_int, C.c_int]
    lib.t2v_decoder_bwd_persist16_scratch_floats.restype = C.c_long
    lib.t2v_decoder_bwd_persist16_dq_offset.argtypes = [C.c_int, C.c_int, C.c_int]
    lib.t2v_decoder_bwd_persist16_dq_offset.restype = C.c_long
    lib.t2v_decoder_bwd_persist16_slices.argtypes = [C.c_int]
    lib.t2v_decoder_bwd_persist16_fits.argtypes = [C.c_int, C.c_int, C.c_int]
    lib.t2v_gemm_f32_set_mode.argtypes = [C.c_int]
    lib.t2v_conv1d_x3_set_mode.argtypes = [C.c_int]
    lib.t2v_gemm_f32_grouped_scratch_floats.argtypes = [C.POINTER(_GemmGroup), C.c_int, C.c_int, C.c_int]
    lib.t2v_gemm_f32_grouped_scratch_floats.restype = C.c_long
    lib.t2v_gemm_f32_grouped.argtypes = [C.POINTER(_GemmGroup), C.c_int, C.c_int, C.c_int, C.c_int, C.c_void_p, C.c_void_p]
    lib.t2v_gemm_bf16_grouped_scratch_floats.argtypes = lib.t2v_gemm_f32_grouped_scratch_floats.argtypes
    lib.t2v_gemm_bf16_grouped_scratch_floats.restype = C.c_long
    lib.t2v_gemm_bf16_grouped.argtypes = lib.t2v_gemm_f32_grouped.argtypes
    lib.t2v_decoder_train_persist_scratch_floats.argtypes = [C.c_int, C.c_int, C.c_int]
    lib.t2v_decoder_train_persist_scratch_floats.restype = C.c_long
    lib.t2v_decoder_bwd_persist_supported.argtypes = [C.c_int, C.c_int]
    lib.t2v_decoder_bwd_achain_scratch_floats.argtypes = [C.c_int, C.c_int, C.c_int]
    lib.t2v_decoder_bwd_achain_scratch_floats.restype = C.c_long
    lib.t2v_decoder_bwd_achain.argtypes = [C.POINTER(_DecTrainPersistWeights), C.c_void_p, C.POINTER(_DecTrainBufs)] + [C.c_void_p] * 8 + [
        C.c_int, C.c_int, C.c_int, C.c_float, C.c_float, C.c_uint64, C.c_void_p]
    lib.t2v_decoder_bwd_persist_slices.argtypes = [C.c_int]
    lib.t2v_decoder_bwd_achain_dq_offset.argtypes = [C.c_int, C.c_int, C.c_int]
    lib.t2v_decoder_bwd_achain_dq_offset.restype = C.c_long
    lib.t2v_decoder_bwd_achain_prepared.argtypes = lib.t2v_decoder_bwd_achain.argtypes
    lib.t2v_decoder_bwd_achain_prepare.argtypes = [C.POINTER(_DecTrainBufs), C.c_void_p, C.c_void_p, C.c_void_p, C.c_int, C.c_int, C.c_int,
                                                   C.c_float, C.c_float, C.c_uint64, C.c_void_p]
    lib.t2v_decoder_replay_fwd_kernels.argtypes = [C.POINTER(_DecWeights), C.POINTER(_DecTrainBufs), C.c_int,
                                                   C.c_int, C.c_int, C.c_float, C.c_float, C.c_uint64, C.c_int,
                                                   C.c_void_p]
    lib.t2v_decoder_replay_bwd_kernels.argtypes = [C.POINTER(_DecWeights), C.POINTER(_DecTrainBufs),
                                                   C.POINTER(_DecBwdBufs), C.c_int, C.c_int, C.c_int, C.c_float,
                                                   C.c_float, C.c_uint64, C.c_int, C.c_void_p]
    lib.t2v_clip_adam_step.argtypes = [C.c_void_p, C.c_void_p, C.c_void_p, C.c_void_p, C.c_uint64, C.c_float,
                                       C.c_float, C.c_float, C.c_float, C.c_float, C.c_float, C.c_float,
                                       C.c_float, C.c_float, C.c_void_p, C.c_void_p, C.c_void_p]
    lib.t2v_clip_adam_step_guarded.argtypes = lib.t2v_clip_adam_step.argtypes[:-1] + [C.c_void_p, C.c_int, C.c_void_p]
    lib.t2v_mask_outputs.argtypes = [C.c_void_p] * 4 + [C.c_int, C.c_int, C.c_int, C.c_float, C.c_void_p]
    lib.t2v_reparam_fwd.argtypes = [C.c_void_p] * 4 + [C.c_long, C.c_void_p]
    lib.t2v_reparam_bwd.argtypes = [C.c_void_p] * 4 + [C.c_long, C.c_void_p]
    lib.t2v_concat2_rows.argtypes = [C.c_void_p, C.c_long, C.c_int, C.c_void_p, C.c_long, C.c_int, C.c_void_p, C.c_long, C.c_void_p]
    lib.t2v_gather_words.argtypes = [C.POINTER(C.c_void_p), C.POINTER(C.c_void_p), C.c_int, C.c_void_p]
    lib.t2v_embedding_fwd.argtypes = [C.c_void_p, C.c_void_p, C.c_void_p, C.c_int, C.c_int, C.c_int, C.c_int, C.c_void_p]
    lib.t2v_embedding_bwd.argtypes = [C.c_void_p, C.c_void_p, C.c_void_p, C.c_int, C.c_int, C.c_int, C.c_int, C.c_void_p]
    lib.t2v_gemm_epilogue_bwd.argtypes = [C.c_void_p, C.c_void_p, C.c_void_p, C.c_size_t, C.c_float, C.c_void_p]
    lib.t2v_colsum.argtypes = [C.c_void_p, C.c_long, C.c_long, C.c_long, C.c_void_p, C.c_void_p, C.c_void_p]
    lib.t2v_colsum_scratch_floats.argtypes = [C.c_long, C.c_long]
    lib.t2v_colsum_scratch_floats.restype = C.c_long
    lib.t2v_set_step_params.argtypes = [C.c_void_p]
    lib.t2v_set_step_params.restype = None
    lib.t2v_set_step_params_stream.argtypes = [C.c_void_p, C.c_void_p]
    lib.t2v_mel_frontend.argtypes = [C.c_void_p, C.c_void_p, C.c_void_p, C.c_int, C.c_int, C.c_float, C.c_int,
                                     C.c_int, C.c_int, C.c_void_p, C.c_void_p, C.c_void_p, C.c_void_p, C.c_void_p,
                                     C.c_void_p, C.c_int, C.c_void_p, C.c_int, C.c_void_p]
    lib.t2v_set_phase_profile.argtypes = [C.c_void_p]
    lib.t2v_stamp.argtypes = [C.c_void_p, C.c_int, C.c_void_p]
    lib.t2v_debug_spin.argtypes = [C.c_int, C.c_int, C.c_void_p]
    lib.t2v_decoder_infer_persistent.argtypes = [C.POINTER(_DecPersistWeights), C.POINTER(_DecPersistBufs), C.c_int, C.c_int,
                                                 C.c_int, C.c_float, C.c_float, C.c_uint64, C.c_void_p]
    lib.t2v_decoder_infer_persistent_items.argtypes = lib.t2v_decoder_infer_persistent.argtypes[:-1] + [C.POINTER(_DecItems),
                                                                                                        C.c_void_p]
    lib.t2v_decoder_persist_supported.argtypes = [C.c_int, C.c_int]
    lib.t2v_decoder_persist_scratch_floats.argtypes = [C.c_int, C.c_int]
    lib.t2v_decoder_persist_scratch_floats.restype = C.c_long
    lib.t2v_decoder_infer_steps.argtypes = [C.POINTER(_DecWeights), C.POINTER(_DecInferBufs), C.c_int, C.c_int, C.c_int,
                                            C.c_int, C.c_float, C.c_float, C.c_int, C.c_uint64, C.c_void_p]
    lib.t2v_decoder_infer_steps_items.argtypes = lib.t2v_decoder_infer_steps.argtypes[:-1] + [C.POINTER(_DecItems), C.c_void_p]
    vp = C.c_void_p
    lib.t2v_stft_polar.argtypes = [vp, vp, C.c_int, C.c_int, C.c_int, C.c_int, vp, vp, vp, vp, vp, C.c_int, vp]
    lib.t2v_istft_scratch_bytes.argtypes = [C.c_int, C.c_int]
    lib.t2v_istft_scratch_bytes.restype = C.c_size_t
    lib.t2v_istft.argtypes = [vp, vp, vp, C.c_int, C.c_int, C.c_int, C.c_int, vp, vp, vp, vp, vp, C.c_int, vp]
    lib.t2v_griffin_lim_scratch_bytes.argtypes = [C.c_int, C.c_int]
# ... 503 lines not shown
    if bad:
        e = T2VHipError("cooperative kernel barrier timed out (results of that step are invalid): %s"
                        % ", ".join(sorted(set(bad))))
        e.labels = sorted(set(bad))
        raise e


def _require_gpu(*tensors):
    lib = load_library()
    for t in tensors:
        if t is not None and not t.is_cuda:
            raise T2VHipError("HIP op called with a CPU tensor; this path has no CPU fallback")
    return lib


def _check(rc, what):
    if rc != 0:
        raise T2VHipError("%s failed: rc=%d (%s)" % (what, rc, load_library().t2v_last_error().decode()))


def _p(t):
    return None if t is None else C.c_void_p(t.data_ptr())


def _stream():
    return C.c_void_p(torch.cuda.current_stream().cuda_stream)


def _f32c(t):
    assert t.dtype == torch.float32
    return t.contiguous()


MAX_DEC_B = 16

_FwdEngine = collections.namedtuple('_FwdEngine', 'kernel scratch run')
_FWD_ENGINES = {
    'persist': _FwdEngine('k_dec_train_persist', 't2v_decoder_train_persist_scratch_floats', 't2v_decoder_train_fwd_persistent'),
    'persist16': _FwdEngine('k_dec_train_persist16', 't2v_decoder_train_persist16_scratch_floats',
                            't2v_decoder_train_fwd_persistent16'),
}
_BwdEngine = collections.namedtuple('_BwdEngine', 'kernel slices scratch dq_offset dq_rows prepare prepared run arena_prepare '
                                                  'reserved keep')
_BWD_ENGINES = {
    'achain': _BwdEngine('k_achain_bwd', 't2v_decoder_bwd_persist_slices', 't2v_decoder_bwd_achain_scratch_floats',
                         't2v_decoder_bwd_achain_dq_offset', None, 't2v_decoder_bwd_achain_prepare',
                         't2v_decoder_bwd_achain_prepared', 't2v_decoder_bwd_achain', True, True, ('XS', 'CA', 'CD', 'GA', 'GD')),
    'persist16': _BwdEngine('k_bwd_persist16', 't2v_decoder_bwd_persist16_slices', 't2v_decoder_bwd_persist16_scratch_floats',
                            't2v_decoder_bwd_persist16_dq_offset', 16, 't2v_decoder_bwd_persistent16_prepare',
                            't2v_decoder_bwd_persistent16_prepared', 't2v_decoder_bwd_persistent16', False, False, ('XS',)),
}
_STEPS_KERNELS = {'fwd': 'k_lstm_fwd256 + k_attn_fwd', 'bwd': 'k_lstm_bwd256 + k_attn_cell_bwd'}
_ARENA = tuple(n for n, _ in _DecTrainBufs._fields_)
ChunkPlan = collections.namedtuple('ChunkPlan', 'b0 b1 fwd bwd prepare')


def _chunk_seed(seed, b0):
    return (int(seed) + 7919 * b0) & 0x7FFFFFFFFFFFFFFF


def _persist_weights(raw, bias_dec, wcomb, vv):
    w_ih_att, w_hh_att, w_ih_dec, w_hh_dec, wq = raw
    return _DecTrainPersistWeights(_p(w_ih_att), _p(w_hh_att), _p(w_ih_dec), _p(w_hh_dec), _p(bias_dec), _p(wq), _p(wcomb), _p(vv))


def _bwd_launch(lib, eng, prepared, PW, Sb, bufs, dims):
    name = eng.prepared if prepared else eng.run
    head = (C.byref(PW), None, C.byref(Sb)) if eng.reserved else (C.byref(PW), C.byref(Sb))
    _check(getattr(lib, name)(*(head + tuple(_p(t) for t in bufs) + tuple(dims) + (_stream(),))), name)


def replay_fwd_kernels(kernel_mask):
    if DecoderCore.last_call is None:
        raise T2VHipError("replay_fwd_kernels: set DecoderCore.keep_last = True before the forward pass")
    W, Sb, (B, T_in, T, p_att, p_dec, seed), _keep = DecoderCore.last_call
    _check(load_library().t2v_decoder_replay_fwd_kernels(C.byref(W), C.byref(Sb), B, T_in, T, p_att, p_dec,
                                                         seed, int(kernel_mask), _stream()),
           't2v_decoder_replay_fwd_kernels')
    return T + 1 if kernel_mask == 1 else T


def replay_persistent_forward():
    if DecoderCore.last_persist is None:
        raise T2VHipError("replay_persistent_forward: the last forward pass did not run on the persistent kernel (or "
                          "DecoderCore.keep_last was off)")
    PW, Sb, scratch, dims, _keep = DecoderCore.last_persist
    eng = _FWD_ENGINES['persist16' if DecoderCore.last_kernel == _FWD_ENGINES['persist16'].kernel else 'persist']
    _check(getattr(load_library(), eng.run)(C.byref(PW), C.byref(Sb), _p(scratch), *(tuple(dims) + (_stream(),))), eng.run)
    return 1


def replay_persistent_backward():
    if DecoderCore.last_bwd_persist is None:
        raise T2VHipError("replay_persistent_backward: the last backward pass did not run on the persistent kernel (or "
                          "DecoderCore.keep_last was off)")
    PW, Sb, bufs, dims, _keep = DecoderCore.last_bwd_persist
    eng = _BWD_ENGINES['persist16' if DecoderCore.last_bwd_kernel == _BWD_ENGINES['persist16'].kernel else 'achain']
    _bwd_launch(load_library(), eng, False, PW, Sb, bufs, dims)
    return 1


def replay_bwd_kernels(kernel_mask):
    if DecoderCore.last_bwd is None:
        raise T2VHipError("replay_bwd_kernels: no backward pass was kept (DecoderCore.keep_last = True before the step)")
    W, Sb, Gb, (B, T_in, T, p_att, p_dec, seed), _keep = DecoderCore.last_bwd
    _check(load_library().t2v_decoder_replay_bwd_kernels(C.byref(W), C.byref(Sb), C.byref(Gb), B, T_in, T, p_att, p_dec,
                                                         seed, int(kernel_mask), _stream()),
           't2v_decoder_replay_bwd_kernels')
    return T if kernel_mask == 1 else T + 1


def pack_decoder_weights(w_ih_att, w_hh_att, w_ih_dec, w_hh_dec, k_att, need_bwd, bf16=False, need_fwd=True):
    lib = load_library()
    dev = w_ih_att.device
    f32 = dict(device=dev, dtype=torch.float32)
    w_ih_att, w_hh_att, w_ih_dec, w_hh_dec = (_f32c(t.detach()) for t in (w_ih_att, w_hh_att, w_ih_dec, w_hh_dec))
    need_fwd = need_fwd or not need_bwd
    packF_att = torch.empty(G4 * k_att, **f32) if need_fwd else None
    packF_dec = torch.empty(G4 * XW, **f32) if need_fwd else None
    packB_att = torch.empty(G4 * KATT, **f32) if need_bwd else None
    packB_dec = torch.empty(G4 * XW, **f32) if need_bwd else None
    fn = lib.t2v_pack_lstm_weights_bf16 if bf16 else lib.t2v_pack_lstm_weights
    _check(fn(_p(w_ih_att), _p(w_hh_att), _p(w_ih_dec), _p(w_hh_dec), int(k_att),
              _p(packF_att), _p(packF_dec), _p(packB_att), _p(packB_dec), _stream()), 't2v_pack_lstm_weights')
    return packF_att, packF_dec, packB_att, packB_dec


def fuse_location_weights(loc_conv, loc_dense):
    lib = load_library()
    wcomb = torch.empty(2, A, 64, device=loc_conv.device, dtype=torch.float32)
    _check(lib.t2v_fuse_location_weights(_p(loc_conv), _p(loc_dense), _p(wcomb), _stream()), 't2v_fuse_location_weights')
    return wcomb


class DecoderCore(torch.autograd.Function):
    persistent = None
    persistent_bwd = None
    persistent16 = None
    keep_last = False
    last_call = None
    last_persist = None
    last_bwd = None
    last_bwd_persist = None
    last_mode = None
    last_bwd_mode = None
    last_kernel = None
    last_bwd_kernel = None
    chunk_kernels = []
    chunk_bwd_kernels = []

    @staticmethod
    def plan(lib, B, T_in, T, need_grad):
        D = DecoderCore
        env = os.environ.get
        fwd_on = D.persistent if D.persistent is not None else env('T2V_TRAIN_PERSISTENT', '1') != '0'
        bwd_on = D.persistent_bwd if D.persistent_bwd is not None else env('T2V_BWD_PERSISTENT', env('T2V_TRAIN_PERSISTENT', '1')) != '0'
        on16 = D.persistent16 if D.persistent16 is not None else env('T2V_PERSIST16', '1') != '0'
        force = on16 == 'force'
        on16 = bool(on16) and bool(_BF16)
        small = lambda floats: 4 * floats < 2 ** 31 - 1
        chunks = [(b0, min(B, b0 + MAX_DEC_B)) for b0 in range(0, B, MAX_DEC_B)]
        fwd, bwd = [], []
        for b0, b1 in chunks:
            b = b1 - b0
            p32 = bool(fwd_on) and bool(lib.t2v_decoder_train_persist_supported(b, T_in)) and \
                small(lib.t2v_decoder_train_persist_scratch_floats(b, T_in, T))
            f16 = on16 and bool(fwd_on) and bool(lib.t2v_decoder_train_persist16_supported(b, T_in)) and (force or not p32) and \
                small(lib.t2v_decoder_train_persist16_scratch_floats(b, T_in, T))
            fwd.append('persist16' if f16 else 'persist' if p32 else 'steps')
            if need_grad:
                r32 = bool(bwd_on) and bool(lib.t2v_decoder_bwd_persist_supported(b, T_in)) and \
                    small(lib.t2v_decoder_bwd_achain_scratch_floats(b, T_in, T))
                r16 = on16 and env('T2V_PERSIST16_BWD', '1') != '0' and bool(bwd_on) and \
                    bool(lib.t2v_decoder_bwd_persist16_fits(b, T_in, T)) and (force or not r32)
                bwd.append('persist16' if r16 else 'achain' if r32 else 'steps')
            else:
                bwd.append(None)
        if 'steps' in bwd:
            bwd = ['steps'] * len(bwd)
        return [ChunkPlan(b0, b1, f, r, f != 'steps' and r in _BWD_ENGINES) for (b0, b1), f, r in zip(chunks, fwd, bwd)]

    @staticmethod
    def _note(fwd=None, bwd=None, **kept):
        D = DecoderCore
        if fwd is not None:
            D.last_mode = 'launch-per-step' if fwd == 'steps' else 'persistent'
            D.last_kernel = _STEPS_KERNELS['fwd'] if fwd == 'steps' else _FWD_ENGINES[fwd].kernel
            D.chunk_kernels.append(D.last_kernel)
        if bwd is not None:
            D.last_bwd_mode = 'launch-per-step' if bwd == 'steps' else 'persistent'
            D.last_bwd_kernel = _STEPS_KERNELS['bwd'] if bwd == 'steps' else _BWD_ENGINES[bwd].kernel
            D.chunk_bwd_kernels.append(D.last_bwd_kernel)
        for name, value in kept.items():
            setattr(D, name, value)

    @staticmethod
    def _bwd_buffers(lib, eng, B, T_in, T, dev):
        f32 = dict(device=dev, dtype=torch.float32)
        DQP = torch.empty(T, B, getattr(lib, eng.slices)(T_in), A, **f32)
        scratch = torch.empty(getattr(lib, eng.scratch)(B, T_in, T), **f32)
        return DQP, scratch, torch.zeros(1, device=dev, dtype=torch.int32)

    @staticmethod
    def _fwd_chunk(lib, plan, gpre, memory, pm, lengths, packs, bias_dec, wqT, wcomb, vv, need_grad, p_att, p_dec, seed, wbf, raw):
        T, B, _ = gpre.shape
        T_in = memory.shape[1]
        f32 = dict(device=gpre.device, dtype=torch.float32)
        XS = torch.empty(T + 2, B, XW, **f32)
        CA = torch.empty(T + 1, B, H, **f32)
        CD = torch.empty(T + 1, B, H, **f32)
        GA = torch.empty(T, B, G4, **f32) if need_grad else None
        GD = torch.empty(T, B, G4, **f32) if need_grad else None
        QP = torch.empty(lib.t2v_decoder_qp_floats(B, T_in), **f32)
        AL = torch.empty(T + 1, B, T_in, **f32)
        ACUM = torch.empty(T + 1, B, T_in, **f32)
        S = torch.empty(T, B, T_in, A, **f32) if need_grad else None
        keep = (gpre, memory, pm, lengths, XS, CA, CD, GA, GD, QP, AL, ACUM, S)
        packF_att, packF_dec, packB_att, packB_dec = packs
        W = _DecWeights(_p(packF_att), _p(packF_dec), _p(packB_att), _p(packB_dec), None, _p(bias_dec),
                        _p(wqT), _p(wcomb), _p(vv), int(bool(wbf)))
        Sb = _DecTrainBufs(*(_p(t) for t in keep))
        dims = (B, T_in, T, float(p_att), float(p_dec), int(seed))
        if plan.fwd == 'steps':
            _check(lib.t2v_decoder_train_fwd(C.byref(W), C.byref(Sb), *(dims + (_stream(),))), 't2v_decoder_train_fwd')
            _err_note('decoder forward (attention exchange)', QP.view(torch.int32)[B * 256 * A + 31:][:1])
            DecoderCore._note(fwd='steps')
            return W, Sb, keep, None
        eng = _FWD_ENGINES[plan.fwd]
        scratch = torch.empty(getattr(lib, eng.scratch)(B, T_in, T), **f32)
        PW = _persist_weights(raw, bias_dec, wcomb, vv)
        _check(getattr(lib, eng.run)(C.byref(PW), C.byref(Sb), _p(scratch), *(dims + (_stream(),))), eng.run)
        _err_note('decoder forward (persistent kernel hand-off)', QP.view(torch.int32)[B * 256 * A + 31:][:1])
        DecoderCore._note(fwd=plan.fwd)
        if DecoderCore.keep_last:
            DecoderCore._note(last_persist=(PW, Sb, scratch, dims, raw))
        if not plan.prepare:
            return W, Sb, keep, None
        beng = _BWD_ENGINES[plan.bwd]
        DQP, bscr, errw = DecoderCore._bwd_buffers(lib, beng, B, T_in, T, gpre.device)
        with side('w', keep=tuple(keep[_ARENA.index(n)] for n in beng.keep)):
            args = (_p(DQP), _p(bscr), _p(errw), B, T_in, T)
            if beng.arena_prepare:
                args = (C.byref(Sb),) + args + dims[3:]
            _check(getattr(lib, beng.prepare)(*(args + (_stream(),))), beng.prepare)
            ev = torch.cuda.Event()
            ev.record()
        return W, Sb, keep, (DQP, bscr, errw, ev)
# ... 31 lines not shown
        wcomb = fuse_location_weights(loc_conv, loc_dense)
        chunks = []
        DecoderCore._note(chunk_kernels=[])
        for p in plans:
            if p.b0 == 0 and p.b1 == B:
                g_c, m_c, pm_c, l_c = gpre, memory, pm, lengths
            else:
                g_c, m_c, pm_c = gpre[:, p.b0:p.b1].contiguous(), memory[p.b0:p.b1].contiguous(), pm[p.b0:p.b1].contiguous()
                l_c = None if lengths is None else lengths[p.b0:p.b1].contiguous()
            chunks.append(DecoderCore._fwd_chunk(lib, p, g_c, m_c, pm_c, l_c, packs, bias_dec, wqT, wcomb, vv, need_grad,
                                                 p_att, p_dec, _chunk_seed(seed, p.b0), wbf, raw))
        hcs = []
        for _w, _s, k, _prep in chunks:
            XSc = k[4]
            Bc, XWc = XSc.size(1), XSc.size(2)
            hc_c = torch.empty(T, Bc, XWc - H, device=XSc.device, dtype=torch.float32)
            _check(lib.t2v_concat2_rows(_p(XSc[2:, :, KATT:]), XWc, XWc - KATT, _p(XSc[1:, :, H:KATT]), XWc, KATT - H, _p(hc_c),
                                        T * Bc, _stream()), 't2v_concat2_rows')
            hcs.append(hc_c)
        als = [k[10][1:].permute(1, 0, 2) for _, _, k, _ in chunks]
        HC = hcs[0] if len(hcs) == 1 else torch.cat(hcs, 1)
        align = als[0] if len(als) == 1 else torch.cat(als, 0)
        ctx.dims = (B, T_in, T, float(p_att), float(p_dec), int(seed))
        ctx.consts = (packs, bias_dec, wqT, wcomb, vv, loc_conv, loc_dense)
        ctx.wbf = wbf
        ctx.wrefs = (w_ih_att, w_hh_att, w_ih_dec, w_hh_dec)
        ctx.raw = raw
        ctx.pre2 = pre2
        ctx.pre_on_side = gpre_ready is not None
        ctx.plans = plans
        ctx.chunks = [k for _, _, k, _ in chunks] if need_grad else None
        ctx.prepared = [pr for _, _, _, pr in chunks] if need_grad else None
        ctx.mark_non_differentiable(align)
        if DecoderCore.keep_last:
            W0, S0, k0, _ = chunks[0]
            DecoderCore._note(last_call=(W0, S0, (k0[0].shape[1], T_in, T, float(p_att), float(p_dec), int(seed)),
                                         k0 + (packs, bias_dec, wqT, wcomb, vv)))
        return HC, align

    @staticmethod
    def backward(ctx, dHC, _dalign):
        lib = load_library()
        Bt, T_in, T, p_att, p_dec, seed = ctx.dims
        packs, bias_dec, wqT, wcomb, vv, loc_conv, loc_dense = ctx.consts
        packF_att, packF_dec, packB_att, packB_dec = packs
        if ctx.chunks is None:
            raise T2VHipError("DecoderCore.backward without a saved arena (forward ran under no_grad)")
        dev = dHC.device
        f32 = dict(device=dev, dtype=torch.float32)
        dHC = _f32c(dHC)
        tcap = (T_in + 15) // 16 * 16
        acc = bacc = None
        wg = None
        dga_l, dmem_l, dpm_l, dpre_l = [], [], [], []
        DecoderCore._note(chunk_bwd_kernels=[])
        for ci, (plan, keep) in enumerate(zip(ctx.plans, ctx.chunks)):
            gpre, memory, pm, lengths, XS, CA, CD, GA, GD, QP, AL, ACUM, S = keep
            b0, B = plan.b0, plan.b1 - plan.b0
            kept = DecoderCore.keep_last and b0 == 0
            dhc_c = dHC if B == Bt else dHC[:, b0:b0 + B].contiguous()
            DGA = torch.empty(T, B, G4, **f32)
            DGD = torch.empty(T, B, G4, **f32)
            DCTX = torch.empty(T, B, E, **f32)
            eng = _BWD_ENGINES.get(plan.bwd)
            NS = lib.t2v_attn_bwd_slices(T_in) if eng is None else getattr(lib, eng.slices)(T_in)
            DV = torch.empty(B, NS, A, **f32)
            Sb = _DecTrainBufs(*(_p(t) for t in keep))
            if eng is not None:
                PW = _persist_weights(ctx.raw, bias_dec, wcomb, vv)
                prep, ctx.prepared[ci] = ctx.prepared[ci], None
                if prep is not None:
                    DQP, scratch, errw, pev = prep
                    torch.cuda.current_stream().wait_event(pev)
                else:
                    DQP, scratch, errw = DecoderCore._bwd_buffers(lib, eng, B, T_in, T, dev)
                stamp('dec_bwd_begin')
                bufs = (dhc_c, DGA, DGD, DCTX, DV, DQP, scratch, errw)
                _bwd_launch(lib, eng, prep is not None, PW, Sb, bufs, (B, T_in, T, p_att, p_dec, _chunk_seed(seed, b0)))
                _err_note('decoder backward (persistent kernel hand-off)', errw)
                dq_off = getattr(lib, eng.dq_offset)(B, T_in, T)
                rows = eng.dq_rows or B
                dq_sum = scratch[dq_off:dq_off + T * rows * A].view(T, rows, A)[:, :B].reshape(T * B, A)
                DecoderCore._note(bwd=plan.bwd)
                if kept:
                    DecoderCore._note(last_bwd_persist=(PW, Sb, bufs, (B, T_in, T, p_att, p_dec, seed), keep + (ctx.raw, wcomb, vv, bias_dec)))
            else:
                W = _DecWeights(_p(packF_att), _p(packF_dec), _p(packB_att), _p(packB_dec), None, _p(bias_dec),
                                _p(wqT), _p(wcomb), _p(vv), int(bool(ctx.wbf)))
                DQ = torch.empty(T, B, NS, A, 2, **f32)
                YD = torch.empty(B, XW, **f32); YA = torch.empty(B, KATT, **f32)
                DCA = torch.empty(B, H, **f32); DCD = torch.empty(B, H, **f32)
                GPREV = torch.empty(2, B, NS, 2, 64, **f32); GCUM = torch.empty(B * NS * tcap + 64, **f32)
                Gb = _DecBwdBufs(_p(dhc_c), _p(DGA), _p(DGD), _p(DQ), _p(DCTX), _p(YD), _p(YA), _p(DCA),
                                 _p(DCD), _p(GPREV), _p(GCUM), _p(DV))
                _check(lib.t2v_decoder_train_bwd(C.byref(W), C.byref(Sb), C.byref(Gb), B, T_in, T, p_att, p_dec,
                                                 _chunk_seed(seed, b0), _stream()), 't2v_decoder_train_bwd')
                _err_note('decoder backward (dq hand-off)', GCUM.view(torch.int32)[B * NS * tcap + 1:][:1])
                dq_sum = DQ[..., 0].sum(2).view(T * B, A)
                DecoderCore._note(bwd='steps')
                if kept:
                    DecoderCore._note(last_bwd=(W, Sb, Gb, (B, T_in, T, p_att, p_dec, seed),
                                                keep + (dhc_c, DGA, DGD, DQ, DCTX, YD, YA, DCA, DCD, GPREV, GCUM, DV, packs, bias_dec,
                                                        wqT, wcomb, vv)))
            TB = T * B
            stamp('dec_bwd_end')
            fork = mark()
            d_memory = torch.empty(B, T_in, E, **f32)
            _check(lib.t2v_gemm_f32_batched(_p(AL[1:]), T_in, 1, B * T_in, _p(DCTX), E, 1, B * E, _p(d_memory), T_in * E, E, B,
                                            T_in, E, T, _stream()), 't2v_gemm_f32_batched')
            dpre = S
            d_pm = colsum(dpre.view(T, B * T_in * A)).view(B, T_in, A)
            dmem_l.append(d_memory); dpm_l.append(d_pm)
            if ctx.pre2 is not None and ctx.needs_input_grad[17] and not ctx.pre_on_side:
                dpre_l.append(gemm(DGA.view(TB, G4), ctx.wrefs[0].detach()[:, :PRE].t()).view(T, B, PRE))
            with side('w', keep=(DGA, DGD, DCTX, DV, dq_sum, dhc_c) + tuple(keep), after=fork):
                dga2, dgd2 = DGA.view(TB, G4), DGD.view(TB, G4)
                x_prev = XS[0:T].reshape(TB, XW)
                x_cur = XS[1:T + 1].reshape(TB, XW)
                first = wg is None
                if first:
                    wg = [grad_slot(w) for w in ctx.wrefs]
                    wg = [torch.empty(w.shape, **f32) if g is None else g for g, w in zip(wg, ctx.wrefs)]
                    if ctx.pre2 is None:
                        wg[0][:, :PRE].zero_()
                d_w_ih_att, d_w_hh_att, d_w_ih_dec, d_w_hh_dec = wg
                grouped = os.environ.get('T2V_DW_GROUPED', '1') != '0'
                if ctx.pre2 is not None:
                    pre_c = ctx.pre2 if B == Bt else ctx.pre2.view(T, Bt, PRE)[:, b0:b0 + B].reshape(TB, PRE)
                    if ctx.needs_input_grad[17] and ctx.pre_on_side:
                        dpre_l.append(gemm(dga2, ctx.wrefs[0].detach()[:, :PRE].t()).view(T, B, PRE))
                    if not grouped:
                        gemm(dga2.t(), pre_c.t(), out=d_w_ih_att[:, :PRE], accumulate=not first)
                with side('g', after=fork):
                    if grouped:
                        att = [(x_prev[:, :H].t(), d_w_hh_att), (x_prev[:, H:KATT].t(), d_w_ih_att[:, PRE:])]
                        if ctx.pre2 is not None:
                            att.insert(0, (pre_c.t(), d_w_ih_att[:, :PRE]))
                        gemm_grouped([(dga2.t(), att),
                                      (dgd2.t(), [(x_cur[:, :KATT].t(), d_w_ih_dec), (x_cur[:, KATT:].t(), d_w_hh_dec)])], accumulate=not first)
                    else:
                        gemm(dga2.t(), x_prev[:, :H].t(), out=d_w_hh_att, accumulate=not first)
                        gemm(dga2.t(), x_prev[:, H:KATT].t(), out=d_w_ih_att[:, PRE:], accumulate=not first)
                        gemm(dgd2.t(), x_cur[:, :KATT].t(), out=d_w_ih_dec, accumulate=not first)
                        gemm(dgd2.t(), x_cur[:, KATT:].t(), out=d_w_hh_dec, accumulate=not first)
                d_wq = gemm(dq_sum.t(), x_cur[:, :H].t())
                d_v = DV.sum((0, 1)).view(1, A)
                d_loc_dense, d_loc_conv = attn_wgrad(dpre, AL, ACUM, loc_conv, loc_dense, B, T_in, T)
                parts = [d_wq, d_loc_conv, d_loc_dense, d_v]
                acc = parts if acc is None else [x + y for x, y in zip(acc, parts)]
            bparts = [colsum(DGD.view(TB, G4))] + ([colsum(DGA.view(TB, G4))] if ctx.pre2 is not None else [])
            bacc = bparts if bacc is None else [x + y for x, y in zip(bacc, bparts)]
            dga_l.append(DGA)
        ctx.chunks = ctx.prepared = None
        d_wq, d_loc_conv, d_loc_dense, d_v = acc
        d_bias_dec = bacc[0]
        d_w_ih_att, d_w_hh_att, d_w_ih_dec, d_w_hh_dec = wg
        d_memory = dmem_l[0] if len(dmem_l) == 1 else torch.cat(dmem_l, 0)
        d_pm = dpm_l[0] if len(dpm_l) == 1 else torch.cat(dpm_l, 0)
        d_pre = d_b_att = None
        if ctx.pre2 is not None:
            DGA = None
            d_b_att = bacc[1]
            if dpre_l and ctx.pre_on_side:
                with side('w'):
                    d_pre = dpre_l[0] if len(dpre_l) == 1 else torch.cat(dpre_l, 1)
            elif dpre_l:
                d_pre = dpre_l[0] if len(dpre_l) == 1 else torch.cat(dpre_l, 1)
        else:
            DGA = dga_l[0] if len(dga_l) == 1 else torch.cat(dga_l, 1)
        return (DGA, d_memory, d_pm, None, d_w_ih_att, d_w_hh_att, d_w_ih_dec, d_w_hh_dec, d_bias_dec,
                d_wq, d_loc_conv, d_loc_dense, d_v, None, None, None, None, d_pre, d_b_att, d_b_att, None)


def attn_wgrad(dpre, AL, ACUM, loc_conv, loc_dense, B, T_in, T):
    lib = _require_gpu(dpre, AL, ACUM, loc_conv, loc_dense)
    f32 = dict(device=dpre.device, dtype=torch.float32)
    part = torch.empty(lib.t2v_attn_wgrad_scratch_floats(), **f32)
    d_dense, d_conv = torch.empty(A, F_LOC, **f32), torch.empty(F_LOC, 2, KS, **f32)
    _check(lib.t2v_attn_wgrad(_p(dpre), _p(AL), _p(ACUM), _p(_f32c(loc_conv)), _p(_f32c(loc_dense)), _p(part),
                              _p(d_dense), _p(d_conv), B, T_in, T, _stream()), 't2v_attn_wgrad')
    return d_dense, d_conv


def mel_frontend(wav, n_samples, tables, scale=1.0, t_stride=None):
    lib = _require_gpu(wav)
    B, N = wav.shape
    wav = wav.contiguous()
# ... 528 lines not shown
            hp0 = torch.cat((z, y[:, :-1, :256]), 1).reshape(BT, 256)
            hp1 = torch.cat((y[:, 1:, 256:], z), 1).reshape(BT, 256)
            g = (gemm(d0.t(), x2.t(), out=grad_slot(w_ih)), gemm(d0.t(), hp0.t()),
                 gemm(d1.t(), x2.t(), out=grad_slot(w_ih_r)), gemm(d1.t(), hp1.t()))
        return (dx, None, g[0], g[1], db0, db0, g[2], g[3], db1, db1, None)


def bilstm_check(sync):
    if int(sync[2].item()) != 0:
        raise T2VHipError("BiLSTM cooperative kernel timed out on its inter-workgroup barrier")


def colsum(x):
    lib = _require_gpu(x)
    assert x.dim() == 2 and x.dtype == torch.float32
    if x.stride(1) != 1 and x.shape[1] > 1:
        x = x.contiguous()
    M, N = x.shape
    out = torch.empty(N, device=x.device, dtype=torch.float32)
    nscr = lib.t2v_colsum_scratch_floats(M, N)
    scr = torch.empty(nscr, device=x.device, dtype=torch.float32) if nscr else None
    _check(lib.t2v_colsum(_p(x), x.stride(0) if M > 1 else N, M, N, _p(scr), _p(out), _stream()), 't2v_colsum')
    return out


_GRAD_SLOTS = {}


def register_grad_slots(slots):
    _GRAD_SLOTS.clear()
    _GRAD_SLOTS.update(slots)


def grad_slot(weight):
    if not weight.is_leaf or weight.grad is not None:
        return None
    ent = _GRAD_SLOTS.get(weight.data_ptr())
    if ent is None:
        return None
    flat, off, shape = ent
    if tuple(shape) != tuple(weight.shape) or flat.device != weight.device:
        return None
    return flat[off:off + weight.numel()].view(shape)


def _small_grads(params, n, f32):
    out = []
    for p in params:
        g = grad_slot(p) if p is not None else None
        out.append(torch.empty(n, **f32) if g is None else g)
    return out


def gemm_grouped(groups, accumulate=False):
    lib = _require_gpu(groups[0][0])
    M, K = groups[0][0].shape
    ok = 1 <= len(groups) <= 2
    for A, parts in groups:
        ok = ok and A.shape == (M, K) and A.dtype == torch.float32 and 1 <= len(parts) <= 3
        for Bp, out in parts:
            ok = ok and Bp.shape[1] == K and Bp.dtype == torch.float32 and out.shape == (M, Bp.shape[0]) and out.stride(1) == 1 and Bp.shape[0] % 128 == 0
    if not ok:
        for A, parts in groups:
            for Bp, out in parts:
                gemm(A, Bp, out=out, accumulate=accumulate)
        return
    arr = (_GemmGroup * len(groups))()
    for g, (A, parts) in zip(arr, groups):
        g.A, g.sAi, g.sAk, g.nb = A.data_ptr(), A.stride(0), A.stride(1), len(parts)
        for p, (Bp, out) in enumerate(parts):
            g.B[p], g.sBj[p], g.sBk[p], g.N[p] = Bp.data_ptr(), Bp.stride(0), Bp.stride(1), Bp.shape[0]
            g.C[p], g.ldc[p] = out.data_ptr(), out.stride(0)
    size_fn, run_fn = ((lib.t2v_gemm_bf16_grouped_scratch_floats, lib.t2v_gemm_bf16_grouped) if _BF16 else
                       (lib.t2v_gemm_f32_grouped_scratch_floats, lib.t2v_gemm_f32_grouped))
    nscr = size_fn(arr, len(groups), M, K)
    scr = torch.empty(max(nscr, 4), device=groups[0][0].device, dtype=torch.float32)
    _check(run_fn(arr, len(groups), M, K, int(bool(accumulate)), _p(scr), _stream()), 't2v_gemm_grouped')


def set_f32_gemm_mode(x3):
    return bool(load_library().t2v_gemm_f32_set_mode(-1 if x3 is None else int(bool(x3))))


def gemm(A, B, bias=None, out=None, relu=False, accumulate=False, p_drop=0.0, seed=0, rng_stream=0, rng_t=0):
    lib = _require_gpu(A, B)
    M, K = A.shape
    N, K2 = B.shape
    assert K == K2 and A.dtype == torch.float32 and B.dtype == torch.float32
    if out is None:
        out = torch.empty(M, N, device=A.device, dtype=torch.float32)
    assert out.shape == (M, N) and out.dtype == torch.float32 and (N == 1 or out.stride(1) == 1)
    ldc = out.stride(0) if M > 1 else max(N, out.stride(0))
    assert ldc >= N and (ldc == N or p_drop == 0.0)
    if True:
        nscr = lib.t2v_gemm_splitk_scratch_floats(M, N, K)
        if nscr and _BF16 and ((M + 63) // 64) * ((N + 63) // 64) >= 64:
            nscr = 0
        if nscr:
            scr = torch.empty(nscr, device=A.device, dtype=torch.float32)
            _check(lib.t2v_gemm_f32_splitk(_p(A), A.stride(0), A.stride(1), _p(B), B.stride(0), B.stride(1), _p(bias), _p(out),
                                           ldc, M, N, K, int(relu), int(accumulate), float(p_drop), int(seed), int(rng_stream),
                                           int(rng_t), _p(scr), _stream()), 't2v_gemm_f32_splitk')
            return out
    if _BF16:
        nscr = lib.t2v_gemm_bf16_splitk_scratch_floats(M, N, K)
        if nscr:
            scr = torch.empty(nscr, device=A.device, dtype=torch.float32)
            _check(lib.t2v_gemm_bf16_splitk(_p(A), A.stride(0), A.stride(1), _p(B), B.stride(0), B.stride(1), _p(bias), _p(out),
                                            ldc, M, N, K, int(relu), int(accumulate), float(p_drop), int(seed), int(rng_stream),
                                            int(rng_t), _p(scr), _stream()), 't2v_gemm_bf16_splitk')
            return out
    fn = lib.t2v_gemm_bf16 if _BF16 else lib.t2v_gemm_f32
    _check(fn(_p(A), A.stride(0), A.stride(1), _p(B), B.stride(0), B.stride(1), _p(bias), _p(out), ldc,
              M, N, K, int(relu), int(accumulate), float(p_drop), int(seed), int(rng_stream),
              int(rng_t), _stream()), 't2v_gemm_bf16' if _BF16 else 't2v_gemm_f32')
    return out


class LinearHIP(torch.autograd.Function):

    @staticmethod
    def forward(ctx, x, weight, bias, relu, p_drop, seed, rng_stream, rng_t):
        _require_gpu(x, weight)
        x2 = x.reshape(-1, x.shape[-1])
        x2 = x2 if x2.dtype == torch.float32 else x2.float()
# ... 220 lines not shown
```

Measured before the change: 222,000 mel-frames/s.

## Fuse decoder-LSTM weight-gradient GEMM into the persistent backward kernel epilogue

```diff
diff --git a/include/t2vae.h b/include/t2vae.h
--- a/include/t2vae.h
+++ b/include/t2vae.h
@@ -127,7 +127,15 @@
 int t2v_decoder_bwd_persist_supported(int B, int T_in);
 long t2v_decoder_bwd_achain_scratch_floats(int B, int T_in, int T_out);
 int t2v_decoder_bwd_persist_slices(int T_in);
-int t2v_decoder_bwd_achain(const t2v_dec_train_persist_weights* w, const float* reserved, const t2v_dec_train_bufs* s,
+typedef struct t2v_achain_dw {
+    float* planes;
+    float* d_w_ih; int ld_ih;
+    float* d_w_hh; int ld_hh;
+    int accumulate;
+    int tile_cap;
+} t2v_achain_dw;
+long t2v_decoder_bwd_achain_dw_offset(int B, int T_in, int T_out);
+int t2v_decoder_bwd_achain(const t2v_dec_train_persist_weights* w, const t2v_achain_dw* dw, const t2v_dec_train_bufs* s,
                            const float* dHC, float* DGA, float* DGD, float* DCTX, float* DV, float* DQP, float* scratch,
                            uint32_t* err_word, int B, int T_in, int T_out, float p_att, float p_dec, uint64_t seed,
                            void* stream);
@@ -149,7 +157,7 @@
 long t2v_decoder_bwd_achain_dq_offset(int B, int T_in, int T_out);
 int t2v_decoder_bwd_achain_prepare(const t2v_dec_train_bufs* s, float* DQP, float* scratch, uint32_t* err_word, int B, int T_in,
                                    int T_out, float p_att, float p_dec, uint64_t seed, void* stream);
-int t2v_decoder_bwd_achain_prepared(const t2v_dec_train_persist_weights* w, const float* reserved, const t2v_dec_train_bufs* s,
+int t2v_decoder_bwd_achain_prepared(const t2v_dec_train_persist_weights* w, const t2v_achain_dw* dw, const t2v_dec_train_bufs* s,
                            const float* dHC, float* DGA, float* DGD, float* DCTX, float* DV, float* DQP, float* scratch,
                            uint32_t* err_word, int B, int T_in, int T_out, float p_att, float p_dec, uint64_t seed,
                            void* stream);
@@ -288,6 +296,9 @@
 } t2v_gemm_group;
 long t2v_gemm_f32_grouped_scratch_floats(const t2v_gemm_group* groups, int ngroups, int M, int K);
 int t2v_gemm_f32_grouped(const t2v_gemm_group* groups, int ngroups, int M, int K, int accumulate, float* scratch, void* stream);
+long t2v_gemm_f32_grouped_group_offset(const t2v_gemm_group* groups, int ngroups, int M, int K, int g);
+int t2v_gemm_f32_grouped_handed(const t2v_gemm_group* groups, int ngroups, int M, int K, int accumulate, float* scratch, int handed,
+                                const uint32_t* done_ctr, int done_cap, void* stream);
 long t2v_gemm_bf16_grouped_scratch_floats(const t2v_gemm_group* groups, int ngroups, int M, int K);
 int t2v_gemm_bf16_grouped(const t2v_gemm_group* groups, int ngroups, int M, int K, int accumulate, float* scratch, void* stream);
 
diff --git a/tacotron2-vae_amd/csrc/decoder_train_bwd_persist.hip b/tacotron2-vae_amd/csrc/decoder_train_bwd_persist.hip
--- a/tacotron2-vae_amd/csrc/decoder_train_bwd_persist.hip
+++ b/tacotron2-vae_amd/csrc/decoder_train_bwd_persist.hip
@@ -1,6 +1,7 @@
 #include "t2v_common.h"
 #include "t2v_kernels.h"
 #include "t2v_xchg.h"
+#include "gemm_x3_tile.h"
 
 #define PB_THREADS 512
 #define PB_MAXB 6
@@ -8,6 +9,7 @@
 #define PB_MAXT_LONG 576
 #define PB_SPIN 400000
 #define PB_KJ (T2V_G / PB_THREADS)
+#define PBA_LROLE_FLOATS(NBS) ((NBS) * T2V_G + 6 * 1024 + 192 + 128 + 512 + 16 * T2V_A + 8 * T2V_A + 2048 + 256 + 64 + 512)
 
 #define PB_ROW_BYTES(NB) ((NB) > 4 ? 98304u : 65536u)
 
@@ -196,6 +198,8 @@
     uint64_t seed;
     const t2v_step_params* step;
     unsigned long long* prof;
+    uint4* dw_planes; float* dw_ih; float* dw_hh; unsigned* dw_ctr;
+    int dw_ld_ih, dw_ld_hh, dw_accumulate, dw_cap, dw_margin;
 };
 #define PBA_STAMP(COND, I) do { if (a.prof && (COND) && threadIdx.x == 0) { const unsigned long long now_ = __builtin_readcyclecounter(); \
         lprof_[(I)] += now_ - tprev_; tprev_ = now_; } } while (0)
@@ -563,6 +567,94 @@
     }
 }
 
+
+struct PBADw {
+    const float* DGD; const float* XC; uint4* planes; float* c_ih; float* c_hh; unsigned* ctr; const float* GXA; unsigned* err;
+    unsigned long long* prof;
+    int K, ld_ih, ld_hh, accumulate, cap, margin_off, jd, ND;
+};
+#define PBA_DW_CTL_SLOT (2 * GX_TILE_SLOTS(3, 2))
+static_assert(16 * (PBA_DW_CTL_SLOT + 1) <= 4 * PBA_LROLE_FLOATS(4), "the epilogue's LDS fits the LSTM roles' allocation");
+
+__device__ __forceinline__ bool pba_dw_barrier(unsigned* ctr, int n, unsigned* err, int* flag) {
+    asm volatile("s_waitcnt vmcnt(0)" ::: "memory");
+    __syncthreads();
+    if (threadIdx.x == 0) {
+        __hip_atomic_fetch_add(ctr, 1u, __ATOMIC_RELEASE, __HIP_MEMORY_SCOPE_AGENT);
+        int rounds = 0;
+        while (__hip_atomic_load(ctr, __ATOMIC_RELAXED, __HIP_MEMORY_SCOPE_AGENT) < (unsigned)n) {
+            __builtin_amdgcn_s_sleep(8);
+            if (t2v_give_up(rounds, PB_SPIN, err, flag)) break;
+        }
+        __builtin_amdgcn_fence(__ATOMIC_ACQUIRE, "agent");
+    }
+    __syncthreads();
+    return flag[0] == 1;
+}
+
+__device__ __noinline__ void pba_dw_epilogue(const PBADw d, float* lds) {
+    const int tid = threadIdx.x, half = tid >> 8, t2 = tid & 255;
+    uint4* const slots = (uint4*)lds;
+    int* const flag = (int*)(slots + PBA_DW_CTL_SLOT);
+    const bool prof = d.prof && d.jd == 0 && tid == 0;
+    if (prof) d.prof[44] = __builtin_amdgcn_s_memrealtime();
+    __syncthreads();
+    if (tid == 0) flag[0] = 1;
+    if (!pba_dw_barrier(d.ctr + 1, d.ND, d.err, flag)) return;
+    if (prof) d.prof[45] = __builtin_amdgcn_s_memrealtime();
+    const long G = gx_groups(d.K);
+    uint4* const Ap = d.planes;
+    uint4* const Bp = Ap + gx_plane_slots(T2V_G, d.K);
+    {
+        uint4 (*sm)[4][64] = (uint4 (*)[4][64])(slots + half * (3 * 4 * 64));
+        const int gy = (int)(G / 4), nA = (T2V_G / 64) * gy, total = nA + (T2V_XW / 64) * gy;
+        const int W = 2 * d.ND, w = 2 * d.jd + half;
+        for (int i0 = 0; i0 < total; i0 += W) {
+            const bool on = i0 + w < total;
+            const int i = on ? i0 + w : 0;
+            const bool isA = i < nA;
+            const int rows = isA ? T2V_G : T2V_XW, j = isA ? i : i - nA, nbx = rows / 64;
+            gx_split_block<false, 3>(isA ? d.DGD : d.XC, 1, rows, rows, d.K, isA ? Ap : Bp, rows, G, j % nbx, j / nbx, t2, sm, on);
+            __syncthreads();
+        }
+    }
+    if (!pba_dw_barrier(d.ctr + 2, d.ND, d.err, flag)) return;
+    if (prof) d.prof[46] = __builtin_amdgcn_s_memrealtime();
+    GemmX3Args ga;
+    {
+        GemmX3Prod& P = ga.pr[0];
+        P.Ap = Ap; P.Bp = Bp; P.RpA = T2V_G; P.RpB = T2V_XW; P.N = T2V_XW; P.tiles_x = T2V_XW / GX_BN; P.tile0 = 0; P.nseg = 2;
+        P.seg_col[0] = 0; P.seg_col[1] = T2V_KATT; P.seg_col[2] = 0x7fffffff;
+        P.segC[0] = d.c_ih; P.segC[1] = d.c_hh; P.segC[2] = d.c_hh;
+        P.seg_ldc[0] = d.ld_ih; P.seg_ldc[1] = d.ld_hh; P.seg_ldc[2] = d.ld_hh;
+        ga.pr[1] = P;
+        ga.nprod = 1; ga.ntiles = (T2V_G / GX_BM) * (T2V_XW / GX_BN); ga.G = G; ga.bias = nullptr; ga.M = T2V_G; ga.relu = 0;
+        ga.accumulate = d.accumulate; ga.p_drop = 0.f; ga.seed = 0; ga.rng_stream = 0; ga.rng_t = 0; ga.step = nullptr;
+        ga.st_chunk = 0; ga.part = nullptr; ga.tile_ctr = nullptr; ga.done_ctr = nullptr; ga.done_prod = 0; ga.done_cap = 0;
+    }
+    const int limit = min(ga.ntiles, d.cap);
+    const __amdgpu_buffer_rsrc_t rA = t2v_rsrc(d.GXA);
+    unsigned npair = 0;
+    for (;;) {
+        if (tid == 0) {
+            int take = -1;
+            if (limit > 0 && d.margin_off >= 0 && t2v_ld_b32(rA, (unsigned)d.margin_off) == T2V_SENT) {
+                const unsigned t = __hip_atomic_fetch_add(d.ctr, 2u, __ATOMIC_RELAXED, __HIP_MEMORY_SCOPE_AGENT);
+                if (t < (unsigned)limit) take = (int)t;
+            }
+            flag[1] = take;
+        }
+        __syncthreads();
+        const int take = flag[1];
+        __syncthreads();
+        if (take < 0) break;
+        const int lin = take + half;
+        gx_tile<3, 2, false>(ga, ga.pr[0], min(lin, limit - 1), t2, slots + half * GX_TILE_SLOTS(3, 2), 0, 1, lin < limit);
+        ++npair;
+    }
+    if (prof) { d.prof[47] = __builtin_amdgcn_s_memrealtime(); d.prof[48] = npair; }
+}
+
 template <int NB>
 __device__ __forceinline__ void pba_decoder_role(const PBAArgs& a, float* lds, const int jd, const int ND) {
     const int B = a.B, T = a.T;
@@ -671,6 +763,15 @@
         __syncthreads();
     }
     if (a.prof && jd == 0 && threadIdx.x == 0) a.prof[41] = __builtin_amdgcn_s_memrealtime();
+    if (a.dw_planes) {
+        PBADw d;
+        d.DGD = a.DGD; d.XC = a.XS + (size_t)B * T2V_XW; d.planes = a.dw_planes; d.c_ih = a.dw_ih; d.c_hh = a.dw_hh; d.ctr = a.dw_ctr;
+        d.GXA = a.GXA; d.err = a.err; d.prof = a.prof;
+        d.K = T * B; d.ld_ih = a.dw_ld_ih; d.ld_hh = a.dw_ld_hh; d.accumulate = a.dw_accumulate; d.cap = a.dw_cap;
+        d.margin_off = a.dw_margin >= 1 && a.dw_margin < T ? (int)((unsigned)a.dw_margin * PB_DROW_BYTES(NB)) : -1;
+        d.jd = jd; d.ND = ND;
+        pba_dw_epilogue(d, lds);
+    }
 }
 
 struct PBACellIn { float gi, gf, gg, go, cac, cprev; };
@@ -964,7 +1065,7 @@
 extern "C" int t2v_decoder_bwd_persist_slices(int T_in) { return T_in < 1 ? 0 : pba_slices(T_in); }
 
 static size_t pba_lds_bytes(int B, int T_in) {
-    const size_t lrole = (B > 4 ? 6 : 4) * T2V_G + 6 * 1024 + 192 + 128 + 512 + 16 * T2V_A + 8 * T2V_A + 2048 + 256 + 64 + 512;
+    const size_t lrole = PBA_LROLE_FLOATS(B > 4 ? 6 : 4);
     const size_t Tcap = (size_t)((T_in + 15) / 16) * 16, JS = (size_t)pba_js(T_in), NWV = JS == 96 ? 8 : 4;
     const size_t trole = 4 * Tcap + T2V_E + JS + (1 + JS / NWV) * 4 * NWV + T2V_A * (JS == 96 ? JS + 17 : JS + 1) + 64 * (JS + 1) +
                          2 * 2 * NWV * T2V_A + 40 + (NWV == 8 ? 64 * 132 : 0);
@@ -972,10 +1073,11 @@
 }
 
 struct PBALayout {
-    size_t n_gx, n_cx, n_gp, n_ex, n_dqt, n_f, n_cp, n_dq;
+    size_t n_gx, n_cx, n_gp, n_ex, n_dqt, n_f, n_cp, n_dwc, n_dq;
     size_t dqt_off() const { return 2 * n_gx + n_cx + n_gp + n_ex; }
     size_t n_exchange() const { return dqt_off() + n_dqt; }
-    size_t total() const { return n_exchange() + 2 * n_f + 2 * n_cp; }
+    size_t dwc_off() const { return n_exchange() + 2 * n_f + 2 * n_cp; }
+    size_t total() const { return dwc_off() + n_dwc; }
 };
 static PBALayout pba_layout(int B, int T_in, int T_out) {
     const size_t T = (size_t)T_out, S = (size_t)pba_slices(T_in), gpw = pba_js(T_in) + 30 <= 64 ? 64 : 128;
@@ -988,6 +1090,7 @@
     l.n_dqt = T * 8 * T2V_A;
     l.n_f = T * rowf;
     l.n_cp = T * T2V_H * (B > 4 ? 6 : 4) * 8;
+    l.n_dwc = 16;
     l.n_dq = T * B * S * 128;
     return l;
 }
@@ -1002,10 +1105,20 @@
     return (long)pba_layout(B, T_in, T_out).dqt_off();
 }
 
+extern "C" long t2v_decoder_bwd_achain_dw_offset(int B, int T_in, int T_out) {
+    if (!t2v_decoder_bwd_persist_supported(B, T_in) || T_out < 1) return -1;
+    return (long)pba_layout(B, T_in, T_out).dwc_off();
+}
+
+static int pba_dw_margin(int B, int T_out) {
+    const double pair_us = 20.0 + 0.09 * (double)T_out * B;
+    return (int)(1.25 * pair_us / 10.58) + 1;
+}
+
 static int pba_launch(const t2v_dec_train_persist_weights* w, const t2v_dec_train_bufs* s,
                       const float* dHC, float* DGA, float* DGD, float* DCTX, float* DV, float* DQP, float* scratch,
                       uint32_t* err_word, int B, int T_in, int T_out, float p_att, float p_dec, uint64_t seed,
-                      void* stream_, bool do_prepare, bool do_run) {
+                      void* stream_, bool do_prepare, bool do_run, const t2v_achain_dw* dw = nullptr) {
     hipStream_t stream = (hipStream_t)stream_;
     if (!s || !DQP || !scratch || !err_word) return T2V_ERR_ARG;
     if (do_run && (!w || !dHC || !DGA || !DGD || !DCTX || !DV)) return T2V_ERR_ARG;
@@ -1015,6 +1128,9 @@
     const PBALayout l = pba_layout(B, T_in, T_out);
     if (((uintptr_t)scratch & 15) || ((uintptr_t)DQP & 15) || l.n_gx * 4 >= 0x7fffffffull || l.n_dq * 4 >= 0x7fffffffull) return T2V_ERR_ARG;
     if (pba_lds_bytes(B, T_in) > T2V_LDS_MAX) return T2V_ERR_ARG;
+    if (do_run && dw && (!dw->planes || ((uintptr_t)dw->planes & 15) || !dw->d_w_ih || !dw->d_w_hh || dw->ld_ih < T2V_KATT || dw->ld_hh < T2V_H ||
+                         (long)T_out * B < 32))
+        return T2V_ERR_ARG;
     static bool raised = false;
     if (!t2v_persist_raise_lds({(const void*)k_achain_bwd<4, false>, (const void*)k_achain_bwd<6, false>,
                                 (const void*)k_achain_bwd<4, true>, (const void*)k_achain_bwd<6, true>}, raised))
@@ -1023,6 +1139,7 @@
         (void)hipMemsetAsync(err_word, 0, sizeof(uint32_t), stream);
         t2v_fill_sentinel(scratch, l.n_exchange() / 4, 1024, stream);
         t2v_fill_sentinel(DQP, l.n_dq / 4, 256, stream);
+        (void)hipMemsetAsync(scratch + l.dwc_off(), 0, l.n_dwc * sizeof(float), stream);
     }
     PBAArgs a;
     if (do_run) {
@@ -1046,6 +1163,14 @@
     a.B = B; a.T_in = T_in; a.T = T_out; a.S_sl = pba_slices(T_in); a.p_att = p_att; a.p_dec = p_dec; a.seed = seed;
     a.step = t2v_step_for(stream);
     a.prof = g_t2v_prof;
+    a.dw_planes = nullptr; a.dw_ih = a.dw_hh = nullptr; a.dw_ctr = (unsigned*)(scratch + l.dwc_off());
+    a.dw_ld_ih = a.dw_ld_hh = a.dw_accumulate = a.dw_cap = a.dw_margin = 0;
+    if (do_run && dw) {
+        a.dw_planes = (uint4*)dw->planes; a.dw_ih = dw->d_w_ih; a.dw_hh = dw->d_w_hh; a.dw_ld_ih = dw->ld_ih; a.dw_ld_hh = dw->ld_hh;
+        a.dw_accumulate = dw->accumulate ? 1 : 0;
+        a.dw_cap = dw->tile_cap < 0 ? 0x7fffffff : dw->tile_cap;
+        a.dw_margin = pba_dw_margin(B, T_out);
+    }
     if (do_prepare) {
         const unsigned nblk = (unsigned)(((size_t)T_out * T2V_G + 255) / 256);
         k_pb_factors<<<nblk, 256, 0, stream>>>(s->GA, s->CA, FA, B, T_out, B, p_att, T2V_RNG_ATT_C, seed, a.step);
@@ -1067,12 +1192,11 @@
     return t2v_check_launch();
 }
 
-extern "C" int t2v_decoder_bwd_achain(const t2v_dec_train_persist_weights* w, const float* w_unused, const t2v_dec_train_bufs* s,
+extern "C" int t2v_decoder_bwd_achain(const t2v_dec_train_persist_weights* w, const t2v_achain_dw* dw, const t2v_dec_train_bufs* s,
                                       const float* dHC, float* DGA, float* DGD, float* DCTX, float* DV, float* DQP, float* scratch,
                                       uint32_t* err_word, int B, int T_in, int T_out, float p_att, float p_dec, uint64_t seed,
                                       void* stream_) {
-    (void)w_unused;
-    return pba_launch(w, s, dHC, DGA, DGD, DCTX, DV, DQP, scratch, err_word, B, T_in, T_out, p_att, p_dec, seed, stream_, true, true);
+    return pba_launch(w, s, dHC, DGA, DGD, DCTX, DV, DQP, scratch, err_word, B, T_in, T_out, p_att, p_dec, seed, stream_, true, true, dw);
 }
 
 extern "C" int t2v_decoder_bwd_achain_prepare(const t2v_dec_train_bufs* s, float* DQP, float* scratch, uint32_t* err_word, int B, int T_in,
@@ -1080,10 +1204,9 @@
     return pba_launch(nullptr, s, nullptr, nullptr, nullptr, nullptr, nullptr, DQP, scratch, err_word, B, T_in, T_out, p_att, p_dec, seed,
                       stream_, true, false);
 }
-extern "C" int t2v_decoder_bwd_achain_prepared(const t2v_dec_train_persist_weights* w, const float* w_unused, const t2v_dec_train_bufs* s,
+extern "C" int t2v_decoder_bwd_achain_prepared(const t2v_dec_train_persist_weights* w, const t2v_achain_dw* dw, const t2v_dec_train_bufs* s,
                                                const float* dHC, float* DGA, float* DGD, float* DCTX, float* DV, float* DQP, float* scratch,
                                                uint32_t* err_word, int B, int T_in, int T_out, float p_att, float p_dec, uint64_t seed,
                                                void* stream_) {
-    (void)w_unused;
-    return pba_launch(w, s, dHC, DGA, DGD, DCTX, DV, DQP, scratch, err_word, B, T_in, T_out, p_att, p_dec, seed, stream_, false, true);
-}
+    return pba_launch(w, s, dHC, DGA, DGD, DCTX, DV, DQP, scratch, err_word, B, T_in, T_out, p_att, p_dec, seed, stream_, false, true, dw);
+}
diff --git a/tacotron2-vae_amd/csrc/gemm.hip b/tacotron2-vae_amd/csrc/gemm.hip
--- a/tacotron2-vae_amd/csrc/gemm.hip
+++ b/tacotron2-vae_amd/csrc/gemm.hip
@@ -5,6 +5,7 @@
 #include "t2v_coop.h"
 #include "t2v_x3.h"
 #include "t2v_xchg.h"
+#include "gemm_x3_tile.h"
 
 #define GM_BM 64
 #define GM_BN 64
@@ -635,228 +636,31 @@
     return big > small ? big : small;
 }
 
-#define GX_BM 128
-#define GX_BN 128
-#define GX_SK 16
-static inline long gx_rp(int rows) { return ((long)rows + 127) / 128 * 128; }
-static inline long gx_groups(int K, int np = 3) { return np == 3 ? ((long)K + 31) / 32 * 4 : ((long)K + 63) / 64 * 8; }
-static inline long gx_plane_slots(int rows, int K, int np = 3) { return np * gx_groups(K, np) * gx_rp(rows); }
 template <bool KC, int NP>
 __global__ __launch_bounds__(256) void k_x3_split(const float* __restrict__ src, long s_row, long s_k, int rows, int K, uint4* __restrict__ dst,
                                                   long Rp, long G) {
     __shared__ uint4 sm[NP][4][64];
-    const int tid = threadIdx.x;
-    const int row0 = blockIdx.x * 64, g0 = blockIdx.y * 4;
-    const int r = KC ? tid >> 2 : tid & 63, g = KC ? tid & 3 : tid >> 6;
-    const int row = row0 + r, k0 = 8 * (g0 + g);
-    float v[8];
-    const bool rin = row < rows;
-    const float* base = src + (long)min(row, rows - 1) * s_row;
-    if (KC && s_k == 1 && !(s_row & 3) && !((uintptr_t)src & 15) && k0 + 8 <= K) {
-        const float4 lo = *(const float4*)(base + k0), hi = *(const float4*)(base + k0 + 4);
-        v[0] = lo.x; v[1] = lo.y; v[2] = lo.z; v[3] = lo.w; v[4] = hi.x; v[5] = hi.y; v[6] = hi.z; v[7] = hi.w;
-#pragma unroll
-        for (int u = 0; u < 8; ++u) v[u] = rin ? v[u] : 0.f;
-    } else {
-#pragma unroll
-        for (int u = 0; u < 8; ++u) {
-            const float x = base[(long)min(k0 + u, K - 1) * s_k];
-            v[u] = (rin && k0 + u < K) ? x : 0.f;
-        }
-    }
-    if (NP == 3) {
-        uint4 p0, p1, p2;
-        t2v_split8(v, p0, p1, p2);
-        sm[0][g][r] = p0; sm[NP > 1 ? 1 : 0][g][r] = p1; sm[NP > 2 ? 2 : 0][g][r] = p2;
-    } else {
-        sm[0][g][r] = make_uint4(t2v_pack_bf16x2(v[0], v[1]), t2v_pack_bf16x2(v[2], v[3]), t2v_pack_bf16x2(v[4], v[5]), t2v_pack_bf16x2(v[6], v[7]));
-    }
-    __syncthreads();
-    const int g2 = tid >> 6, r2 = tid & 63;
-    if (row0 + r2 < Rp && g0 + g2 < G) {
-#pragma unroll
-        for (int p = 0; p < NP; ++p) dst[(p * G + g0 + g2) * Rp + row0 + r2] = sm[p][g2][r2];
-    }
-}
-struct GemmX3Prod {
-    const uint4* Ap; const uint4* Bp;
-    long RpA, RpB;
-    int N, tiles_x, tile0, nseg;
-    int seg_col[3]; float* segC[3]; int seg_ldc[3];
-};
-struct GemmX3Args {
-    GemmX3Prod pr[2];
-    int nprod, ntiles;
-    long G;
-    const float* bias;
-    int M, relu, accumulate;
-    float p_drop; uint64_t seed; uint32_t rng_stream, rng_t;
-    const t2v_step_params* step;
-    int st_chunk;
-    float* part; unsigned* tile_ctr;
-};
-#ifndef GX_NB
-#define GX_NB 2
-#endif
-#ifndef GX_LDS_PAD
-#define GX_LDS_PAD 0
-#endif
-#ifndef GX_NG1
-#define GX_NG1 4
-#endif
+    gx_split_block<KC, NP>(src, s_row, s_k, rows, K, dst, Rp, G, blockIdx.x, blockIdx.y, threadIdx.x, sm);
+}
 template <int NP, int NG>
 __global__ __launch_bounds__(256, 2) void k_gemm_x3p(GemmX3Args a) {
-    __shared__ uint4 lds_[GX_NB * 2 * NP * NG * GX_BM + GX_LDS_PAD];
-    uint4 (*Ls)[2][NP][NG][GX_BM] = (uint4 (*)[2][NP][NG][GX_BM])&lds_[0];
-    const unsigned lds0 = (unsigned)(unsigned long)(__attribute__((address_space(3))) void*)&lds_[0];
-    const int tid = threadIdx.x, wave = __builtin_amdgcn_readfirstlane(tid >> 6), lane = tid & 63;
-    const int wm = wave >> 1, wn = wave & 1;
+    __shared__ uint4 lds_[GX_TILE_SLOTS(NP, NG)];
+    int nb = a.ntiles, d0 = 0, ndone = 0;
+    if (a.done_ctr) {
+        const GemmX3Prod& D = a.pr[a.done_prod];
+        ndone = (int)min(min(*a.done_ctr, a.done_cap), (unsigned)(D.tiles_x * ((a.M + GX_BM - 1) / GX_BM)));
+        nb -= ndone; d0 = D.tile0;
+        if ((int)blockIdx.x >= nb) return;
+    }
     int lin;
     {
-        const int nb = a.ntiles, bid = blockIdx.x;
+        const int bid = blockIdx.x;
         const int q = nb >> 3, r = nb & 7, xcd = bid & 7, idx = bid >> 3;
         lin = (xcd < r ? xcd * (q + 1) : r * (q + 1) + (xcd - r) * q) + idx;
+        if (lin >= d0) lin += ndone;
     }
     const GemmX3Prod& P = a.pr[(a.nprod > 1 && lin >= a.pr[1].tile0) ? 1 : 0];
-    const int by_ = (lin - P.tile0) / P.tiles_x, bx_ = (lin - P.tile0) - by_ * P.tiles_x;
-    const int i0 = by_ * GX_BM, j0 = bx_ * GX_BN;
-    const int nst_all = (int)(a.G / NG);
-    const int st0 = a.st_chunk ? blockIdx.z * a.st_chunk : 0, st1 = a.st_chunk ? min(nst_all, st0 + a.st_chunk) : nst_all;
-    constexpr int NPIECE = NP * NG;
-    auto stage_dma = [&](int st, int buf) {
-        st = min(st, st1 - 1);
-#pragma unroll
-        for (int i = 0; i < NPIECE; ++i) {
-            const int q = wave + 4 * i;
-            const int op = q / (2 * NP * NG), rem = q - (2 * NP * NG) * op, p = rem / (2 * NG), g = (rem >> 1) % NG, half = rem & 1;
-            const uint4* src = op ? P.Bp + (p * a.G + NG * st + g) * P.RpB + j0 + 64 * half + lane
-                                  : P.Ap + (p * a.G + NG * st + g) * P.RpA + i0 + 64 * half + lane;
-            t2v_dma16(src, lds0 + 16u * (unsigned)(((((buf * 2 + op) * NP + p) * NG + g) * GX_BM) + 64 * half));
-        }
-    };
-    f32x16 acc[2][2];
-#pragma unroll
-    for (int x = 0; x < 2; ++x)
-#pragma unroll
-        for (int y = 0; y < 2; ++y)
-#pragma unroll
-            for (int r = 0; r < 16; ++r) acc[x][y][r] = 0.f;
-    const int am = 64 * wm + (lane & 31), bn = 64 * wn + (lane & 31), kq = lane >> 5;
-#define GX_MFMA(A_, B_, C_) C_ = __builtin_amdgcn_mfma_f32_32x32x16_bf16(*(const t2v_bf16x8*)&(A_), *(const t2v_bf16x8*)&(B_), C_, 0, 0, 0)
-#pragma unroll
-    for (int d = 0; d < GX_NB - 1; ++d) stage_dma(st0 + d, d);
-    t2v_wait_vmcnt<NPIECE * (GX_NB - 2)>();
-    __syncthreads();
-    int buf = 0;
-    for (int st = st0; st < st1; ++st) {
-        const int nb2 = buf == 0 ? GX_NB - 1 : buf - 1;
-        stage_dma(st + GX_NB - 1, nb2);
-#define GX_ALL(PA, PB)                                      \
-        GX_MFMA(av[PA][0], bv[PB][0], acc[0][0]); GX_MFMA(av[PA][0], bv[PB][1], acc[0][1]); \
-        GX_MFMA(av[PA][1], bv[PB][0], acc[1][0]); GX_MFMA(av[PA][1], bv[PB][1], acc[1][1])
-#pragma unroll
-        for (int ks = 0; ks < NG / 2; ++ks) {
-            uint4 av[NP][2], bv[NP][2];
-#pragma unroll
-            for (int p = 0; p < NP; ++p) {
-                av[p][0] = Ls[buf][0][p][2 * ks + kq][am];
-                av[p][1] = Ls[buf][0][p][2 * ks + kq][am + 32];
-                bv[p][0] = Ls[buf][1][p][2 * ks + kq][bn];
-                bv[p][1] = Ls[buf][1][p][2 * ks + kq][bn + 32];
-            }
-            if constexpr (NP == 3) {
-                GX_ALL(2, 0); GX_ALL(0, 2); GX_ALL(1, 1); GX_ALL(1, 0); GX_ALL(0, 1); GX_ALL(0, 0);
-            } else {
-                GX_ALL(0, 0);
-            }
-        }
-#undef GX_ALL
-        t2v_wait_vmcnt<NPIECE * (GX_NB - 2)>();
-        __syncthreads();
-        buf = buf == GX_NB - 1 ? 0 : buf + 1;
-    }
-#undef GX_MFMA
-    asm volatile("s_waitcnt vmcnt(0)" ::: "memory");
-    if (a.part) {
-        const size_t tiles = (size_t)a.ntiles, tile = (size_t)lin;
-        {
-            __amdgpu_buffer_rsrc_t rs = t2v_rsrc(a.part + (blockIdx.z * tiles + tile) * (GX_BM * GX_BN));
-#pragma unroll
-            for (int x = 0; x < 2; ++x)
-#pragma unroll
-                for (int y = 0; y < 2; ++y)
-#pragma unroll
-                    for (int q = 0; q < 4; ++q) {
-                        u32x4 v;
-                        v.x = __float_as_uint(acc[x][y][4 * q]); v.y = __float_as_uint(acc[x][y][4 * q + 1]);
-                        v.z = __float_as_uint(acc[x][y][4 * q + 2]); v.w = __float_as_uint(acc[x][y][4 * q + 3]);
-                        __builtin_amdgcn_raw_buffer_store_b128(v, rs, ((((x * 2 + y) * 4 + q) * 256) + tid) * 16, 0, 16);
-                    }
-        }
-        __shared__ unsigned last_;
-        asm volatile("s_waitcnt vmcnt(0)" ::: "memory");
-        __syncthreads();
-        unsigned* ctr = a.tile_ctr + tile;
-        if (tid == 0) last_ = __hip_atomic_fetch_add(ctr, 1u, __ATOMIC_RELAXED, __HIP_MEMORY_SCOPE_AGENT) == gridDim.z - 1 ? 1u : 0u;
-        __syncthreads();
-        if (!last_) return;
-        if (tid == 0) __hip_atomic_store(ctr, 0u, __ATOMIC_RELAXED, __HIP_MEMORY_SCOPE_AGENT);
-        const int nz = (int)gridDim.z;
-#pragma unroll
-        for (int x = 0; x < 2; ++x)
-#pragma unroll
-            for (int y = 0; y < 2; ++y)
-#pragma unroll
-                for (int r = 0; r < 16; ++r) acc[x][y][r] = 0.f;
-        for (int z0 = 0; z0 < nz; z0 += 2) {
-            u32x4 v[2][16];
-#pragma unroll
-            for (int u = 0; u < 2; ++u) {
-                const int z = min(z0 + u, nz - 1);
-                __amdgpu_buffer_rsrc_t rs = t2v_rsrc(a.part + (z * tiles + tile) * (GX_BM * GX_BN));
-#pragma unroll
-                for (int g = 0; g < 16; ++g) v[u][g] = __builtin_amdgcn_raw_buffer_load_b128(rs, (g * 256 + tid) * 16, 0, 16);
-            }
-#pragma unroll
-            for (int u = 0; u < 2; ++u)
-                if (z0 + u < nz) {
-#pragma unroll
-                    for (int g = 0; g < 16; ++g) {
-                        acc[g >> 3][(g >> 2) & 1][4 * (g & 3)] += __uint_as_float(v[u][g].x);
-                        acc[g >> 3][(g >> 2) & 1][4 * (g & 3) + 1] += __uint_as_float(v[u][g].y);
-                        acc[g >> 3][(g >> 2) & 1][4 * (g & 3) + 2] += __uint_as_float(v[u][g].z);
-                        acc[g >> 3][(g >> 2) & 1][4 * (g & 3) + 3] += __uint_as_float(v[u][g].w);
-                    }
-                }
-        }
-    }
-    const uint64_t seed = t2v_step_seed(a.seed, a.step);
-    int sg = 0;
-    if (P.nseg > 1 && j0 >= P.seg_col[1]) sg = 1;
-    if (P.nseg > 2 && j0 >= P.seg_col[2]) sg = 2;
-    float* const Cd = P.segC[sg];
-    const int ldc = P.seg_ldc[sg], jc0 = j0 - P.seg_col[sg];
-#pragma unroll
-    for (int x = 0; x < 2; ++x)
-#pragma unroll
-        for (int y = 0; y < 2; ++y) {
-            const int jl = 64 * wn + 32 * y + (lane & 31), j = j0 + jl;
-            if (j < P.N) {
-                const float bvs = a.bias ? a.bias[j] : 0.f;
-#pragma unroll
-                for (int r = 0; r < 16; ++r) {
-                    const int i = i0 + 64 * wm + 32 * x + (r & 3) + 8 * (r >> 2) + 4 * (lane >> 5);
-                    if (i < a.M) {
-                        const size_t idx = (size_t)i * ldc + jc0 + jl;
-                        float v = acc[x][y][r] + bvs;
-                        if (a.accumulate) v += Cd[idx];
-                        if (a.relu) v = fmaxf(v, 0.f);
-                        if (a.p_drop > 0.f) v *= t2v_drop_scale(seed, a.rng_stream, a.rng_t, (uint32_t)idx, a.p_drop);
-                        Cd[idx] = v;
-                    }
-                }
-            }
-        }
+    gx_tile<NP, NG, true>(a, P, lin, threadIdx.x, lds_, blockIdx.z, gridDim.z);
 }
 static int g_f32_gemm_x3 = -1;
 static int gemm_x3_mode() {
@@ -929,6 +733,7 @@
     a.G = G; a.bias = g.bias; a.M = M; a.relu = g.relu; a.accumulate = g.accumulate;
     a.p_drop = g.p_drop; a.seed = g.seed; a.rng_stream = g.rng_stream; a.rng_t = g.rng_t; a.step = g.step;
     a.st_chunk = 0; a.part = nullptr; a.tile_ctr = nullptr;
+    a.done_ctr = nullptr; a.done_prod = 0; a.done_cap = 0;
     dim3 gb(a.ntiles, 1, 1);
     const int ns = gemm_x3_splits(M, N, K, np);
     if (ns > 1) {
@@ -971,7 +776,8 @@
         }
     return tiles >= 64;
 }
-static int gemm_grouped_impl(const t2v_gemm_group* gr, int ngroups, int M, int K, int accumulate, float* scratch, void* stream_, int np) {
+static int gemm_grouped_impl(const t2v_gemm_group* gr, int ngroups, int M, int K, int accumulate, float* scratch, void* stream_, int np,
+                             int handed = -1, const uint32_t* done_ctr = nullptr, int done_cap = 0) {
     hipStream_t stream = (hipStream_t)stream_;
     if (!gr || ngroups < 1 || ngroups > 2 || M < 1 || K < 1) return T2V_ERR_ARG;
     for (int g = 0; g < ngroups; ++g) {
@@ -979,6 +785,9 @@
         for (int p = 0; p < gr[g].nb; ++p)
             if (!gr[g].B[p] || !gr[g].C[p] || gr[g].N[p] < 1 || gr[g].ldc[p] < gr[g].N[p]) return T2V_ERR_ARG;
     }
+    if (handed >= 0 && (handed >= ngroups || !done_ctr || done_cap < 0 || np != 3 || !scratch || ((uintptr_t)scratch & 15) ||
+                        !gemm_grouped_x3_ok(gr, ngroups, M, K, np)))
+        return T2V_ERR_ARG;
     if (!scratch || ((uintptr_t)scratch & 15) || !gemm_grouped_x3_ok(gr, ngroups, M, K, np)) {
         for (int g = 0; g < ngroups; ++g)
             for (int p = 0; p < gr[g].nb; ++p) {
@@ -1000,13 +809,13 @@
         P.Ap = at; at += gx_plane_slots(M, K, np);
         P.Bp = at; at += np * G * n;
         P.RpA = RpA; P.RpB = n; P.N = (int)n; P.tiles_x = (int)(n / GX_BN); P.tile0 = tile0; P.nseg = gr[g].nb;
-        gx_split_launch(gr[g].A, gr[g].sAi, gr[g].sAk, M, K, (uint4*)P.Ap, RpA, G, 0, stream, np);
+        if (g != handed) gx_split_launch(gr[g].A, gr[g].sAi, gr[g].sAk, M, K, (uint4*)P.Ap, RpA, G, 0, stream, np);
         long col = 0;
         for (int p = 0; p < 3; ++p) {
             const int q = p < gr[g].nb ? p : gr[g].nb - 1;
             P.seg_col[p] = p < gr[g].nb ? (int)col : 0x7fffffff; P.segC[p] = gr[g].C[q]; P.seg_ldc[p] = gr[g].ldc[q];
             if (p < gr[g].nb) {
-                gx_split_launch(gr[g].B[p], gr[g].sBj[p], gr[g].sBk[p], gr[g].N[p], K, (uint4*)P.Bp, n, G, col, stream, np);
+                if (g != handed) gx_split_launch(gr[g].B[p], gr[g].sBj[p], gr[g].sBk[p], gr[g].N[p], K, (uint4*)P.Bp, n, G, col, stream, np);
                 col += gr[g].N[p];
             }
         }
@@ -1017,12 +826,22 @@
     a.G = G; a.bias = nullptr; a.M = M; a.relu = 0; a.accumulate = accumulate;
     a.p_drop = 0.f; a.seed = 0; a.rng_stream = 0; a.rng_t = 0; a.step = t2v_step_for(stream);
     a.st_chunk = 0; a.part = nullptr; a.tile_ctr = nullptr;
+    a.done_ctr = handed >= 0 ? done_ctr : nullptr; a.done_prod = handed >= 0 ? handed : 0; a.done_cap = (unsigned)done_cap;
     if (np == 3) k_gemm_x3p<3, 2><<<dim3(a.ntiles, 1, 1), 256, 0, stream>>>(a);
     else k_gemm_x3p<1, GX_NG1><<<dim3(a.ntiles, 1, 1), 256, 0, stream>>>(a);
     return t2v_check_launch();
 }
 extern "C" int t2v_gemm_f32_grouped(const t2v_gemm_group* gr, int ngroups, int M, int K, int accumulate, float* scratch, void* stream_) {
     return gemm_grouped_impl(gr, ngroups, M, K, accumulate, scratch, stream_, 3);
+}
+extern "C" int t2v_gemm_f32_grouped_handed(const t2v_gemm_group* gr, int ngroups, int M, int K, int accumulate, float* scratch, int handed,
+                                           const uint32_t* done_ctr, int done_cap, void* stream_) {
+    if (handed < 0) return T2V_ERR_ARG;
+    return gemm_grouped_impl(gr, ngroups, M, K, accumulate, scratch, stream_, 3, handed, done_ctr, done_cap);
+}
+extern "C" long t2v_gemm_f32_grouped_group_offset(const t2v_gemm_group* gr, int ngroups, int M, int K, int g) {
+    if (!gr || ngroups < 1 || ngroups > 2 || g < 0 || g >= ngroups || M < 1 || K < 1 || !gemm_grouped_x3_ok(gr, ngroups, M, K, 3)) return -1;
+    return g == 0 ? 0 : gemm_grouped_scratch(gr, 1, M, K, 3);
 }
 extern "C" int t2v_gemm_bf16_grouped(const t2v_gemm_group* gr, int ngroups, int M, int K, int accumulate, float* scratch, void* stream_) {
     return gemm_grouped_impl(gr, ngroups, M, K, accumulate, scratch, stream_, 1);
diff --git a/tacotron2-vae_amd/csrc/gemm_x3_tile.h b/tacotron2-vae_amd/csrc/gemm_x3_tile.h
--- /dev/null
+++ b/tacotron2-vae_amd/csrc/gemm_x3_tile.h
@@ -0,0 +1,228 @@
+#pragma once
+#include "t2v_common.h"
+#include "t2v_x3.h"
+#include "t2v_xchg.h"
+
+#define GX_BM 128
+#define GX_BN 128
+#define GX_SK 16
+__host__ __device__ static inline long gx_rp(int rows) { return ((long)rows + 127) / 128 * 128; }
+__host__ __device__ static inline long gx_groups(int K, int np = 3) { return np == 3 ? ((long)K + 31) / 32 * 4 : ((long)K + 63) / 64 * 8; }
+__host__ __device__ static inline long gx_plane_slots(int rows, int K, int np = 3) { return np * gx_groups(K, np) * gx_rp(rows); }
+
+template <bool KC, int NP>
+__device__ __forceinline__ void gx_split_block(const float* __restrict__ src, long s_row, long s_k, int rows, int K, uint4* __restrict__ dst,
+                                               long Rp, long G, int bx, int by, int tid, uint4 (*sm)[4][64], bool on = true) {
+    const int row0 = bx * 64, g0 = by * 4;
+    const int r = KC ? tid >> 2 : tid & 63, g = KC ? tid & 3 : tid >> 6;
+    const int row = row0 + r, k0 = 8 * (g0 + g);
+    if (on) {
+        float v[8];
+        const bool rin = row < rows;
+        const float* base = src + (long)min(row, rows - 1) * s_row;
+        if (KC && s_k == 1 && !(s_row & 3) && !((uintptr_t)src & 15) && k0 + 8 <= K) {
+            const float4 lo = *(const float4*)(base + k0), hi = *(const float4*)(base + k0 + 4);
+            v[0] = lo.x; v[1] = lo.y; v[2] = lo.z; v[3] = lo.w; v[4] = hi.x; v[5] = hi.y; v[6] = hi.z; v[7] = hi.w;
+#pragma unroll
+            for (int u = 0; u < 8; ++u) v[u] = rin ? v[u] : 0.f;
+        } else {
+#pragma unroll
+            for (int u = 0; u < 8; ++u) {
+                const float x = base[(long)min(k0 + u, K - 1) * s_k];
+                v[u] = (rin && k0 + u < K) ? x : 0.f;
+            }
+        }
+        if (NP == 3) {
+            uint4 p0, p1, p2;
+            t2v_split8(v, p0, p1, p2);
+            sm[0][g][r] = p0; sm[NP > 1 ? 1 : 0][g][r] = p1; sm[NP > 2 ? 2 : 0][g][r] = p2;
+        } else {
+            sm[0][g][r] = make_uint4(t2v_pack_bf16x2(v[0], v[1]), t2v_pack_bf16x2(v[2], v[3]), t2v_pack_bf16x2(v[4], v[5]), t2v_pack_bf16x2(v[6], v[7]));
+        }
+    }
+    __syncthreads();
+    const int g2 = tid >> 6, r2 = tid & 63;
+    if (on && row0 + r2 < Rp && g0 + g2 < G) {
+#pragma unroll
+        for (int p = 0; p < NP; ++p) dst[(p * G + g0 + g2) * Rp + row0 + r2] = sm[p][g2][r2];
+    }
+}
+
+struct GemmX3Prod {
+    const uint4* Ap; const uint4* Bp;
+    long RpA, RpB;
+    int N, tiles_x, tile0, nseg;
+    int seg_col[3]; float* segC[3]; int seg_ldc[3];
+};
+struct GemmX3Args {
+    GemmX3Prod pr[2];
+    int nprod, ntiles;
+    long G;
+    const float* bias;
+    int M, relu, accumulate;
+    float p_drop; uint64_t seed; uint32_t rng_stream, rng_t;
+    const t2v_step_params* step;
+    int st_chunk;
+    float* part; unsigned* tile_ctr;
+    const unsigned* done_ctr; int done_prod; unsigned done_cap;
+};
+#ifndef GX_NB
+#define GX_NB 2
+#endif
+#ifndef GX_LDS_PAD
+#define GX_LDS_PAD 0
+#endif
+#ifndef GX_NG1
+#define GX_NG1 4
+#endif
+#define GX_TILE_SLOTS(NP, NG) (GX_NB * 2 * (NP) * (NG) * GX_BM + GX_LDS_PAD)
+
+template <int NP, int NG, bool SPLITK>
+__device__ __forceinline__ void gx_tile(const GemmX3Args& a, const GemmX3Prod& P, const int lin, const int tid, uint4* lds_, const int zi,
+                                        const int nz, const bool store = true) {
+    uint4 (*Ls)[2][NP][NG][GX_BM] = (uint4 (*)[2][NP][NG][GX_BM])lds_;
+    const unsigned lds0 = __builtin_amdgcn_readfirstlane((unsigned)(unsigned long)(__attribute__((address_space(3))) void*)lds_);
+    const int wave = __builtin_amdgcn_readfirstlane(tid >> 6), lane = tid & 63;
+    const int wm = wave >> 1, wn = wave & 1;
+    const int by_ = (lin - P.tile0) / P.tiles_x, bx_ = (lin - P.tile0) - by_ * P.tiles_x;
+    const int i0 = by_ * GX_BM, j0 = bx_ * GX_BN;
+    const int nst_all = (int)(a.G / NG);
+    const int st0 = a.st_chunk ? zi * a.st_chunk : 0, st1 = a.st_chunk ? min(nst_all, st0 + a.st_chunk) : nst_all;
+    constexpr int NPIECE = NP * NG;
+    auto stage_dma = [&](int st, int buf) {
+        st = min(st, st1 - 1);
+#pragma unroll
+        for (int i = 0; i < NPIECE; ++i) {
+            const int q = wave + 4 * i;
+            const int op = q / (2 * NP * NG), rem = q - (2 * NP * NG) * op, p = rem / (2 * NG), g = (rem >> 1) % NG, half = rem & 1;
+            const uint4* src = op ? P.Bp + (p * a.G + NG * st + g) * P.RpB + j0 + 64 * half + lane
+                                  : P.Ap + (p * a.G + NG * st + g) * P.RpA + i0 + 64 * half + lane;
+            t2v_dma16(src, lds0 + 16u * (unsigned)(((((buf * 2 + op) * NP + p) * NG + g) * GX_BM) + 64 * half));
+        }
+    };
+    f32x16 acc[2][2];
+#pragma unroll
+    for (int x = 0; x < 2; ++x)
+#pragma unroll
+        for (int y = 0; y < 2; ++y)
+#pragma unroll
+            for (int r = 0; r < 16; ++r) acc[x][y][r] = 0.f;
+    const int am = 64 * wm + (lane & 31), bn = 64 * wn + (lane & 31), kq = lane >> 5;
+#define GX_MFMA(A_, B_, C_) C_ = __builtin_amdgcn_mfma_f32_32x32x16_bf16(*(const t2v_bf16x8*)&(A_), *(const t2v_bf16x8*)&(B_), C_, 0, 0, 0)
+#pragma unroll
+    for (int d = 0; d < GX_NB - 1; ++d) stage_dma(st0 + d, d);
+    t2v_wait_vmcnt<NPIECE * (GX_NB - 2)>();
+    __syncthreads();
+    int buf = 0;
+    for (int st = st0; st < st1; ++st) {
+        const int nb2 = buf == 0 ? GX_NB - 1 : buf - 1;
+        stage_dma(st + GX_NB - 1, nb2);
+#define GX_ALL(PA, PB)                                      \
+        GX_MFMA(av[PA][0], bv[PB][0], acc[0][0]); GX_MFMA(av[PA][0], bv[PB][1], acc[0][1]); \
+        GX_MFMA(av[PA][1], bv[PB][0], acc[1][0]); GX_MFMA(av[PA][1], bv[PB][1], acc[1][1])
+#pragma unroll
+        for (int ks = 0; ks < NG / 2; ++ks) {
+            uint4 av[NP][2], bv[NP][2];
+#pragma unroll
+            for (int p = 0; p < NP; ++p) {
+                av[p][0] = Ls[buf][0][p][2 * ks + kq][am];
+                av[p][1] = Ls[buf][0][p][2 * ks + kq][am + 32];
+                bv[p][0] = Ls[buf][1][p][2 * ks + kq][bn];
+                bv[p][1] = Ls[buf][1][p][2 * ks + kq][bn + 32];
+            }
+            if constexpr (NP == 3) {
+                GX_ALL(2, 0); GX_ALL(0, 2); GX_ALL(1, 1); GX_ALL(1, 0); GX_ALL(0, 1); GX_ALL(0, 0);
+            } else {
+                GX_ALL(0, 0);
+            }
+        }
+#undef GX_ALL
+        t2v_wait_vmcnt<NPIECE * (GX_NB - 2)>();
+        __syncthreads();
+        buf = buf == GX_NB - 1 ? 0 : buf + 1;
+    }
+#undef GX_MFMA
+    asm volatile("s_waitcnt vmcnt(0)" ::: "memory");
+    if constexpr (SPLITK) {
+        if (a.part) {
+            const size_t tiles = (size_t)a.ntiles, tile = (size_t)lin;
+            {
+                __amdgpu_buffer_rsrc_t rs = t2v_rsrc(a.part + (zi * tiles + tile) * (GX_BM * GX_BN));
+#pragma unroll
+                for (int x = 0; x < 2; ++x)
+#pragma unroll
+                    for (int y = 0; y < 2; ++y)
+#pragma unroll
+                        for (int q = 0; q < 4; ++q) {
+                            u32x4 v;
+                            v.x = __float_as_uint(acc[x][y][4 * q]); v.y = __float_as_uint(acc[x][y][4 * q + 1]);
+                            v.z = __float_as_uint(acc[x][y][4 * q + 2]); v.w = __float_as_uint(acc[x][y][4 * q + 3]);
+                            __builtin_amdgcn_raw_buffer_store_b128(v, rs, ((((x * 2 + y) * 4 + q) * 256) + tid) * 16, 0, 16);
+                        }
+            }
+            __shared__ unsigned last_;
+            asm volatile("s_waitcnt vmcnt(0)" ::: "memory");
+            __syncthreads();
+            unsigned* ctr = a.tile_ctr + tile;
+            if (tid == 0) last_ = __hip_atomic_fetch_add(ctr, 1u, __ATOMIC_RELAXED, __HIP_MEMORY_SCOPE_AGENT) == (unsigned)nz - 1 ? 1u : 0u;
+            __syncthreads();
+            if (!last_) return;
+            if (tid == 0) __hip_atomic_store(ctr, 0u, __ATOMIC_RELAXED, __HIP_MEMORY_SCOPE_AGENT);
+#pragma unroll
+            for (int x = 0; x < 2; ++x)
+#pragma unroll
+                for (int y = 0; y < 2; ++y)
+#pragma unroll
+                    for (int r = 0; r < 16; ++r) acc[x][y][r] = 0.f;
+            for (int z0 = 0; z0 < nz; z0 += 2) {
+                u32x4 v[2][16];
+#pragma unroll
+                for (int u = 0; u < 2; ++u) {
+                    const int z = min(z0 + u, nz - 1);
+                    __amdgpu_buffer_rsrc_t rs = t2v_rsrc(a.part + (z * tiles + tile) * (GX_BM * GX_BN));
+#pragma unroll
+                    for (int g = 0; g < 16; ++g) v[u][g] = __builtin_amdgcn_raw_buffer_load_b128(rs, (g * 256 + tid) * 16, 0, 16);
+                }
+#pragma unroll
+                for (int u = 0; u < 2; ++u)
+                    if (z0 + u < nz) {
+#pragma unroll
+                        for (int g = 0; g < 16; ++g) {
+                            acc[g >> 3][(g >> 2) & 1][4 * (g & 3)] += __uint_as_float(v[u][g].x);
+                            acc[g >> 3][(g >> 2) & 1][4 * (g & 3) + 1] += __uint_as_float(v[u][g].y);
+                            acc[g >> 3][(g >> 2) & 1][4 * (g & 3) + 2] += __uint_as_float(v[u][g].z);
+                            acc[g >> 3][(g >> 2) & 1][4 * (g & 3) + 3] += __uint_as_float(v[u][g].w);
+                        }
+                    }
+            }
+        }
+    }
+    if (!store) return;
+    const uint64_t seed = t2v_step_seed(a.seed, a.step);
+    int sg = 0;
+    if (P.nseg > 1 && j0 >= P.seg_col[1]) sg = 1;
+    if (P.nseg > 2 && j0 >= P.seg_col[2]) sg = 2;
+    float* const Cd = P.segC[sg];
+    const int ldc = P.seg_ldc[sg], jc0 = j0 - P.seg_col[sg];
+#pragma unroll
+    for (int x = 0; x < 2; ++x)
+#pragma unroll
+        for (int y = 0; y < 2; ++y) {
+            const int jl = 64 * wn + 32 * y + (lane & 31), j = j0 + jl;
+            if (j < P.N) {
+                const float bvs = a.bias ? a.bias[j] : 0.f;
+#pragma unroll
+                for (int r = 0; r < 16; ++r) {
+                    const int i = i0 + 64 * wm + 32 * x + (r & 3) + 8 * (r >> 2) + 4 * (lane >> 5);
+                    if (i < a.M) {
+                        const size_t idx = (size_t)i * ldc + jc0 + jl;
+                        float v = acc[x][y][r] + bvs;
+                        if (a.accumulate) v += Cd[idx];
+                        if (a.relu) v = fmaxf(v, 0.f);
+                        if (a.p_drop > 0.f) v *= t2v_drop_scale(seed, a.rng_stream, a.rng_t, (uint32_t)idx, a.p_drop);
+                        Cd[idx] = v;
+                    }
+                }
+            }
+        }
+}
diff --git a/tacotron2-vae_amd/t2v_hip.py b/tacotron2-vae_amd/t2v_hip.py
--- a/tacotron2-vae_amd/t2v_hip.py
+++ b/tacotron2-vae_amd/t2v_hip.py
@@ -52,6 +52,12 @@
     C_NAME = 't2v_gemm_group'
     _fields_ = [('A', C.c_void_p), ('sAi', C.c_long), ('sAk', C.c_long), ('nb', C.c_int), ('B', C.c_void_p * 3), ('sBj', C.c_long * 3),
                 ('sBk', C.c_long * 3), ('N', C.c_int * 3), ('C', C.c_void_p * 3), ('ldc', C.c_int * 3)]
+
+
+class _AchainDw(C.Structure):
+    C_NAME = 't2v_achain_dw'
+    _fields_ = [('planes', C.c_void_p), ('d_w_ih', C.c_void_p), ('ld_ih', C.c_int), ('d_w_hh', C.c_void_p), ('ld_hh', C.c_int),
+                ('accumulate', C.c_int), ('tile_cap', C.c_int)]
 
 
 class _DecInferBufs(C.Structure):
@@ -76,7 +82,8 @@
            't2v_decoder_train_fwd_persistent', 't2v_decoder_train_persist_supported',
            't2v_decoder_train_persist_scratch_floats', 't2v_decoder_bwd_persist_supported',
            't2v_decoder_bwd_achain_scratch_floats', 't2v_decoder_bwd_achain', 't2v_decoder_bwd_achain_prepare',
-           't2v_decoder_bwd_achain_prepared', 't2v_decoder_bwd_persist_slices', 't2v_decoder_bwd_achain_dq_offset', 't2v_mask_outputs', 't2v_reparam_fwd',
+           't2v_decoder_bwd_achain_prepared', 't2v_decoder_bwd_persist_slices', 't2v_decoder_bwd_achain_dq_offset',
+           't2v_decoder_bwd_achain_dw_offset', 't2v_gemm_f32_grouped_handed', 't2v_gemm_f32_grouped_group_offset', 't2v_mask_outputs', 't2v_reparam_fwd',
            't2v_reparam_bwd', 't2v_gather_words', 't2v_concat2_rows',
            't2v_decoder_train_fwd_persistent16', 't2v_decoder_train_persist16_supported',
            't2v_decoder_train_persist16_scratch_floats', 't2v_decoder_bwd_persistent16', 't2v_decoder_bwd_persist16_supported',
@@ -148,7 +155,13 @@
     lib.t2v_decoder_bwd_persist_supported.argtypes = [C.c_int, C.c_int]
     lib.t2v_decoder_bwd_achain_scratch_floats.argtypes = [C.c_int, C.c_int, C.c_int]
     lib.t2v_decoder_bwd_achain_scratch_floats.restype = C.c_long
-    lib.t2v_decoder_bwd_achain.argtypes = [C.POINTER(_DecTrainPersistWeights), C.c_void_p, C.POINTER(_DecTrainBufs)] + [C.c_void_p] * 8 + [
+    lib.t2v_gemm_f32_grouped_handed.argtypes = [C.POINTER(_GemmGroup), C.c_int, C.c_int, C.c_int, C.c_int, C.c_void_p, C.c_int, C.c_void_p,
+                                                C.c_int, C.c_void_p]
+    lib.t2v_gemm_f32_grouped_group_offset.argtypes = [C.POINTER(_GemmGroup), C.c_int, C.c_int, C.c_int, C.c_int]
+    lib.t2v_gemm_f32_grouped_group_offset.restype = C.c_long
+    lib.t2v_decoder_bwd_achain_dw_offset.argtypes = [C.c_int, C.c_int, C.c_int]
+    lib.t2v_decoder_bwd_achain_dw_offset.restype = C.c_long
+    lib.t2v_decoder_bwd_achain.argtypes = [C.POINTER(_DecTrainPersistWeights), C.POINTER(_AchainDw), C.POINTER(_DecTrainBufs)] + [C.c_void_p] * 8 + [
         C.c_int, C.c_int, C.c_int, C.c_float, C.c_float, C.c_uint64, C.c_void_p]
     lib.t2v_decoder_bwd_persist_slices.argtypes = [C.c_int]
     lib.t2v_decoder_bwd_achain_dq_offset.argtypes = [C.c_int, C.c_int, C.c_int]
@@ -758,7 +771,7 @@
 }
 _STEPS_KERNELS = {'fwd': 'k_lstm_fwd256 + k_attn_fwd', 'bwd': 'k_lstm_bwd256 + k_attn_cell_bwd'}
 _ARENA = tuple(n for n, _ in _DecTrainBufs._fields_)
-ChunkPlan = collections.namedtuple('ChunkPlan', 'b0 b1 fwd bwd prepare')
+ChunkPlan = collections.namedtuple('ChunkPlan', 'b0 b1 fwd bwd prepare dw_epilogue')
 
 
 def _chunk_seed(seed, b0):
@@ -770,9 +783,10 @@
     return _DecTrainPersistWeights(_p(w_ih_att), _p(w_hh_att), _p(w_ih_dec), _p(w_hh_dec), _p(bias_dec), _p(wq), _p(wcomb), _p(vv))
 
 
-def _bwd_launch(lib, eng, prepared, PW, Sb, bufs, dims):
+def _bwd_launch(lib, eng, prepared, PW, Sb, bufs, dims, dw=None):
     name = eng.prepared if prepared else eng.run
-    head = (C.byref(PW), None, C.byref(Sb)) if eng.reserved else (C.byref(PW), C.byref(Sb))
+    assert dw is None or eng.reserved
+    head = (C.byref(PW), None if dw is None else C.byref(dw), C.byref(Sb)) if eng.reserved else (C.byref(PW), C.byref(Sb))
     _check(getattr(lib, name)(*(head + tuple(_p(t) for t in bufs) + tuple(dims) + (_stream(),))), name)
 
 
@@ -802,7 +816,8 @@
                           "DecoderCore.keep_last was off)")
     PW, Sb, bufs, dims, _keep = DecoderCore.last_bwd_persist
     eng = _BWD_ENGINES['persist16' if DecoderCore.last_bwd_kernel == _BWD_ENGINES['persist16'].kernel else 'achain']
-    _bwd_launch(load_library(), eng, False, PW, Sb, bufs, dims)
+    dwh = _keep[-1] if isinstance(_keep[-1], GroupedHandOver) else None
+    _bwd_launch(load_library(), eng, False, PW, Sb, bufs, dims, None if dwh is None else dwh.dw)
     return 1
 
 
@@ -848,6 +863,7 @@
     last_persist = None
     last_bwd = None
     last_bwd_persist = None
+    dw_tile_cap = None
     last_mode = None
     last_bwd_mode = None
     last_kernel = None
@@ -884,7 +900,10 @@
                 bwd.append(None)
         if 'steps' in bwd:
             bwd = ['steps'] * len(bwd)
-        return [ChunkPlan(b0, b1, f, r, f != 'steps' and r in _BWD_ENGINES) for (b0, b1), f, r in zip(chunks, fwd, bwd)]
+        dw_on = (not _BF16 and env('T2V_DW_EPILOGUE', '1') != '0' and env('T2V_DW_GROUPED', '1') != '0' and
+                 env('T2V_F32_GEMM', '') not in ('native', '0'))
+        return [ChunkPlan(b0, b1, f, r, f != 'steps' and r in _BWD_ENGINES, dw_on and r == 'achain')
+                for (b0, b1), f, r in zip(chunks, fwd, bwd)]
 
     @staticmethod
     def _note(fwd=None, bwd=None, **kept):
@@ -899,6 +918,21 @@
             D.chunk_bwd_kernels.append(D.last_bwd_kernel)
         for name, value in kept.items():
             setattr(D, name, value)
+
+    @staticmethod
+    def _wgrad_tensors(ctx, f32):
+        wg = [grad_slot(w) for w in ctx.wrefs]
+        return [torch.empty(w.shape, **f32) if g is None else g for g, w in zip(wg, ctx.wrefs)]
+
+    @staticmethod
+    def _dw_groups(DGA, DGD, XS, wg, pre_c, T, B):
+        TB = T * B
+        x_prev, x_cur = XS[0:T].reshape(TB, XW), XS[1:T + 1].reshape(TB, XW)
+        d_w_ih_att, d_w_hh_att, d_w_ih_dec, d_w_hh_dec = wg
+        att = [(x_prev[:, :H].t(), d_w_hh_att), (x_prev[:, H:KATT].t(), d_w_ih_att[:, PRE:])]
+        if pre_c is not None:
+            att.insert(0, (pre_c.t(), d_w_ih_att[:, :PRE]))
+        return [(DGA.view(TB, G4).t(), att), (DGD.view(TB, G4).t(), [(x_cur[:, :KATT].t(), d_w_ih_dec), (x_cur[:, KATT:].t(), d_w_hh_dec)])]
 
     @staticmethod
     def _bwd_buffers(lib, eng, B, T_in, T, dev):
@@ -1036,6 +1070,7 @@
         tcap = (T_in + 15) // 16 * 16
         acc = bacc = None
         wg = None
+        wg_fresh = False
         dga_l, dmem_l, dpm_l, dpre_l = [], [], [], []
         DecoderCore._note(chunk_bwd_kernels=[])
         for ci, (plan, keep) in enumerate(zip(ctx.plans, ctx.chunks)):
@@ -1050,6 +1085,7 @@
             NS = lib.t2v_attn_bwd_slices(T_in) if eng is None else getattr(lib, eng.slices)(T_in)
             DV = torch.empty(B, NS, A, **f32)
             Sb = _DecTrainBufs(*(_p(t) for t in keep))
+            dwh = None
             if eng is not None:
                 PW = _persist_weights(ctx.raw, bias_dec, wcomb, vv)
                 prep, ctx.prepared[ci] = ctx.prepared[ci], None
@@ -1058,16 +1094,28 @@
                     torch.cuda.current_stream().wait_event(pev)
                 else:
                     DQP, scratch, errw = DecoderCore._bwd_buffers(lib, eng, B, T_in, T, dev)
+                if plan.dw_epilogue and set_f32_gemm_mode(None) and T * B >= 32:
+                    if wg is None:
+                        wg, wg_fresh = DecoderCore._wgrad_tensors(ctx, f32), True
+                    pre_c = None
+                    if ctx.pre2 is not None:
+                        pre_c = ctx.pre2 if B == Bt else ctx.pre2.view(T, Bt, PRE)[:, b0:b0 + B].reshape(T * B, PRE)
+                    groups = DecoderCore._dw_groups(DGA, DGD, XS, wg, pre_c, T, B)
+                    dwh = GroupedHandOver(groups, 1, scratch[lib.t2v_decoder_bwd_achain_dw_offset(B, T_in, T):][:1], not wg_fresh,
+                                          DecoderCore.dw_tile_cap)
+                    if not wg_fresh and overlap() is not None:
+                        overlap().wait('g')
                 stamp('dec_bwd_begin')
                 bufs = (dhc_c, DGA, DGD, DCTX, DV, DQP, scratch, errw)
-                _bwd_launch(lib, eng, prep is not None, PW, Sb, bufs, (B, T_in, T, p_att, p_dec, _chunk_seed(seed, b0)))
+                _bwd_launch(lib, eng, prep is not None, PW, Sb, bufs, (B, T_in, T, p_att, p_dec, _chunk_seed(seed, b0)),
+                            None if dwh is None else dwh.dw)
                 _err_note('decoder backward (persistent kernel hand-off)', errw)
                 dq_off = getattr(lib, eng.dq_offset)(B, T_in, T)
                 rows = eng.dq_rows or B
                 dq_sum = scratch[dq_off:dq_off + T * rows * A].view(T, rows, A)[:, :B].reshape(T * B, A)
                 DecoderCore._note(bwd=plan.bwd)
                 if kept:
-                    DecoderCore._note(last_bwd_persist=(PW, Sb, bufs, (B, T_in, T, p_att, p_dec, seed), keep + (ctx.raw, wcomb, vv, bias_dec)))
+                    DecoderCore._note(last_bwd_persist=(PW, Sb, bufs, (B, T_in, T, p_att, p_dec, seed), keep + (ctx.raw, wcomb, vv, bias_dec, dwh)))
             else:
                 W = _DecWeights(_p(packF_att), _p(packF_dec), _p(packB_att), _p(packB_dec), None, _p(bias_dec),
                                 _p(wqT), _p(wcomb), _p(vv), int(bool(ctx.wbf)))
@@ -1101,12 +1149,12 @@
                 dga2, dgd2 = DGA.view(TB, G4), DGD.view(TB, G4)
                 x_prev = XS[0:T].reshape(TB, XW)
                 x_cur = XS[1:T + 1].reshape(TB, XW)
-                first = wg is None
-                if first:
-                    wg = [grad_slot(w) for w in ctx.wrefs]
-                    wg = [torch.empty(w.shape, **f32) if g is None else g for g, w in zip(wg, ctx.wrefs)]
-                    if ctx.pre2 is None:
-                        wg[0][:, :PRE].zero_()
+                first = wg is None or wg_fresh
+                if wg is None:
+                    wg = DecoderCore._wgrad_tensors(ctx, f32)
+                wg_fresh = False
+                if first and ctx.pre2 is None:
+                    wg[0][:, :PRE].zero_()
                 d_w_ih_att, d_w_hh_att, d_w_ih_dec, d_w_hh_dec = wg
                 grouped = os.environ.get('T2V_DW_GROUPED', '1') != '0'
                 if ctx.pre2 is not None:
@@ -1115,8 +1163,10 @@
                         dpre_l.append(gemm(dga2, ctx.wrefs[0].detach()[:, :PRE].t()).view(T, B, PRE))
                     if not grouped:
                         gemm(dga2.t(), pre_c.t(), out=d_w_ih_att[:, :PRE], accumulate=not first)
-                with side('g', after=fork):
-                    if grouped:
+                with side('g', after=fork, keep=() if dwh is None else (dwh.scr,)):
+                    if dwh is not None:
+                        gemm_grouped(dwh.groups, accumulate=not first, handed=dwh)
+                    elif grouped:
                         att = [(x_prev[:, :H].t(), d_w_hh_att), (x_prev[:, H:KATT].t(), d_w_ih_att[:, PRE:])]
                         if ctx.pre2 is not None:
                             att.insert(0, (pre_c.t(), d_w_ih_att[:, :PRE]))
@@ -1751,9 +1801,43 @@
     return out
 
 
-def gemm_grouped(groups, accumulate=False):
+def _group_array(groups):
+    arr = (_GemmGroup * len(groups))()
+    for g, (A, parts) in zip(arr, groups):
+        g.A, g.sAi, g.sAk, g.nb = A.data_ptr(), A.stride(0), A.stride(1), len(parts)
+        for p, (Bp, out) in enumerate(parts):
+            g.B[p], g.sBj[p], g.sBk[p], g.N[p] = Bp.data_ptr(), Bp.stride(0), Bp.stride(1), Bp.shape[0]
+            g.C[p], g.ldc[p] = out.data_ptr(), out.stride(0)
+    return arr
+
+
+class GroupedHandOver(object):
+
+    def __init__(self, groups, g, counter, accumulate, cap=None):
+        lib = load_library()
+        assert g == 1 and len(groups) == 2 and len(groups[1][1]) == 2
+        M, K = groups[0][0].shape
+        self.groups, self.g, self.counter = groups, g, counter
+        arr = _group_array(groups)
+        off = lib.t2v_gemm_f32_grouped_group_offset(arr, len(groups), M, K, g)
+        if off < 0:
+            raise T2VHipError("GroupedHandOver: these products do not take the grouped plane launch")
+        self.scr = torch.empty(lib.t2v_gemm_f32_grouped_scratch_floats(arr, len(groups), M, K), device=counter.device, dtype=torch.float32)
+        self.cap = -1 if cap is None else int(cap)
+        (_, out_ih), (_, out_hh) = groups[g][1]
+        self.dw = _AchainDw(self.scr.data_ptr() + 4 * off, out_ih.data_ptr(), out_ih.stride(0), out_hh.data_ptr(), out_hh.stride(0),
+                            int(bool(accumulate)), self.cap)
+
+
+def gemm_grouped(groups, accumulate=False, handed=None):
     lib = _require_gpu(groups[0][0])
     M, K = groups[0][0].shape
+    if handed is not None:
+        assert handed.groups is groups and not _BF16
+        cap = handed.cap if handed.cap >= 0 else 2 ** 31 - 1
+        _check(lib.t2v_gemm_f32_grouped_handed(_group_array(groups), len(groups), M, K, int(bool(accumulate)), _p(handed.scr), handed.g,
+                                               _p(handed.counter), cap, _stream()), 't2v_gemm_f32_grouped_handed')
+        return
     ok = 1 <= len(groups) <= 2
     for A, parts in groups:
         ok = ok and A.shape == (M, K) and A.dtype == torch.float32 and 1 <= len(parts) <= 3
@@ -1764,12 +1848,7 @@
             for Bp, out in parts:
                 gemm(A, Bp, out=out, accumulate=accumulate)
         return
-    arr = (_GemmGroup * len(groups))()
-    for g, (A, parts) in zip(arr, groups):
-        g.A, g.sAi, g.sAk, g.nb = A.data_ptr(), A.stride(0), A.stride(1), len(parts)
-        for p, (Bp, out) in enumerate(parts):
-            g.B[p], g.sBj[p], g.sBk[p], g.N[p] = Bp.data_ptr(), Bp.stride(0), Bp.stride(1), Bp.shape[0]
-            g.C[p], g.ldc[p] = out.data_ptr(), out.stride(0)
+    arr = _group_array(groups)
     size_fn, run_fn = ((lib.t2v_gemm_bf16_grouped_scratch_floats, lib.t2v_gemm_bf16_grouped) if _BF16 else
                        (lib.t2v_gemm_f32_grouped_scratch_floats, lib.t2v_gemm_f32_grouped))
     nscr = size_fn(arr, len(groups), M, K)
```

After: 228,100 mel-frames/s (median of 6 runs). 1.03x the previous value.
